# mlee03/FRE-NCtools

Measured on AMD Instinct MI355X. Metric: exchange-cells/s, higher is better.
Workload: dtype f64; 1 GPU; C384 cubed sphere (6 tiles) -> 1440x720 lat-lon, conservative_order2: exchange-grid search + centroid pass + CSR build per step; nxgrid=4160000, parallelism=1 latitude band(s) of the target, one per GPU, world_size=1

## Files before the change

### fre-nctools_amd/_lib.py

```python
import ctypes as C
import os

_HERE = os.path.dirname(os.path.abspath(__file__))
_LIB = None


class FregridHipError(RuntimeError):
    def __init__(self, code, msg):
        super().__init__(f"libfregrid_hip error {code}: {msg}")
        self.code = code


def lib_path():
    return os.environ.get("FREGRID_HIP_LIB") or os.path.join(_HERE, "libfregrid_hip.so")


EXPORTS = [
    "get_maxxgrid", "get_grid_area", "create_xgrid_2dx2d_order1", "create_xgrid_2dx2d_order2", "conserve_interp",
    "clip_2dx2d", "poly_area", "poly_ctrlon", "poly_ctrlat", "fix_lon", "pimod",
    "fg_clip_2dx2d_batch", "fg_poly_op_batch",
    "get_maxxgrid_", "get_grid_area_", "create_xgrid_2dx2d_order1_", "create_xgrid_2dx2d_order2_",
    "fg_last_error", "fg_device_count", "fg_plan_create", "fg_plan_create_dev", "fg_plan_create_empty",
    "fg_plan_destroy", "fg_plan_set_stream", "fg_pool_release", "fg_plan_nxgrid", "fg_plan_ncells_in",
    "fg_plan_cell_sums_dev", "fg_plan_copy_cell_sums", "fg_plan_accumulate_cell_sums", "fg_plan_accumulate_cell_sums_async", "fg_dev_gather_f64", "fg_dev_scatter_f64", "fg_plan_finalize", "fg_plan_get_xgrid", "fg_plan_get_polygons", "fg_plan_create_polylist", "fg_plan_get_cell_struct",
    "fg_plan_get_cell_area", "fg_plan_set_xgrid", "fg_plan_apply", "fg_plan_apply_interleaved", "fg_plan_apply_records", "fg_plan_apply_levels", "fg_plan_apply_records_levels", "fg_plan_levels_capacity", "fg_plan_apply_ex", "fg_plan_mono_begin",
    "fg_plan_mono_minmax_dev", "fg_plan_mono_copy_minmax", "fg_plan_mono_end",
    "fg_plan_create_great_circle", "fg_plan_create_great_circle_dev", "fg_latlon2xyz", "create_xgrid_great_circle",
    "create_xgrid_great_circle_", "get_grid_great_circle_area", "get_grid_great_circle_area_", "clip_2dx2d_great_circle",
    "great_circle_area", "fg_gc_clip_batch", "conserve_interp_great_circle", "fg_sincos_batch",
    "create_xgrid_1dx2d_order1", "create_xgrid_1dx2d_order2", "create_xgrid_2dx1d_order1", "create_xgrid_2dx1d_order2",
    "create_xgrid_1dx2d_order1_", "create_xgrid_1dx2d_order2_", "create_xgrid_2dx1d_order1_", "create_xgrid_2dx1d_order2_",
    "clip", "box_ctrlat", "box_ctrlon", "get_grid_area_no_adjust", "get_grid_area_no_adjust_", "fg_plan_stream", "fg_plan_sync",
    "fg_c2l_create", "fg_c2l_destroy", "fg_c2l_ncells", "fg_c2l_halo_size", "fg_c2l_set_stream", "fg_c2l_sync",
    "fg_c2l_get_centres", "fg_c2l_fill_halo", "fg_c2l_gradient", "fg_c2l_gradient_records", "fg_c2l_records", "fg_c2l_records_levels", "fg_c2l_grid_info", "fg_find_contacts", "fg_halo_map",
    "fg_gnomonic_ed_grid", "fg_tripolar_corners", "fg_remap_write", "fg_remap_write_interp", "fg_remap_read_size", "fg_remap_read", "fg_remap_last_error",
    "fg_plan_trim", "fg_plan_ncells_out", "fg_plan_order", "fg_plan_device", "fg_dev_alloc", "fg_dev_free", "fg_dev_upload", "fg_dev_download",
    "fg_nc_open", "fg_nc_create", "fg_nc_def_dim", "fg_nc_def_var", "fg_nc_put_att_text", "fg_nc_put_att_double", "fg_nc_enddef",
    "fg_nc_inq_ndims", "fg_nc_inq_nvars", "fg_nc_inq_numrecs", "fg_nc_inq_dimid", "fg_nc_inq_dim", "fg_nc_inq_varid", "fg_nc_inq_var",
    "fg_nc_get_att_double", "fg_nc_get_att_text", "fg_nc_get_vara", "fg_nc_get_vara_double", "fg_nc_put_vara", "fg_nc_put_vara_double",
    "fg_nc_close", "fg_nc_last_error", "fg_dev_widen", "fg_dev_narrow", "fg_sweep_create", "fg_sweep_run", "fg_sweep_run_levels", "fg_sweep_destroy", "fg_host_alloc", "fg_host_free",
    "fg_plan_stats", "fg_set_search_mode", "fg_set_search_cull", "fg_set_search_finalize", "fg_set_search_rect", "fg_set_search_frame", "fg_set_apply_xcd", "fg_set_apply_vec", "fg_set_apply_ep", "fg_set_gc_split", "fg_set_profiling", "fg_plan_phase_ms", "fg_gnomonic_ed_corners", "fg_latlon_corners",
    "fg_bilin_create", "fg_bilin_create_from_weights", "fg_bilin_destroy", "fg_bilin_get_index_weight", "fg_bilin_npoints_fine",
    "fg_bilin_nlon_fine", "fg_bilin_nlat_fine", "fg_bilin_nlon", "fg_bilin_nlat", "fg_bilin_ncells", "fg_bilin_set_stream",
    "fg_bilin_sync", "fg_bilin_apply_scalar", "fg_bilin_apply_vector", "fg_bilin_remap_write", "fg_bilin_remap_read",
    "fg_unit_vect_latlon", "fg_bilin_fine_grid", "fg_bilin_ambiguous_ties",
    "fg_extrap_create", "fg_extrap_destroy", "fg_extrap_set_stream", "fg_extrap_stream", "fg_extrap_run_dev", "fg_extrap_run",
    "fg_extrap_last_syncs", "fg_extrap_get_coef", "fg_extrap_coef_host", "fg_set_extrap_batch", "fg_set_extrap_coef",
    "fg_setup_vertical_interp", "fg_dev_vertical_interp",
    "fg_dev_latlon2xyz", "fg_plan_create_great_circle_lonlat", "fg_plan_create_great_circle_lonlat_dev",
    "fg_runoff_create", "fg_runoff_create_from_xgrid", "fg_runoff_destroy", "fg_runoff_nxgrid", "fg_runoff_get_xgrid",
    "fg_runoff_get_maps", "fg_runoff_get_xyz", "fg_runoff_search_stats", "fg_runoff_phase_ms", "fg_runoff_stream", "fg_runoff_apply", "fg_runoff_apply_dev",
    "fg_nearest_unmasked", "fg_set_runoff_prune", "fg_runoff_tile",
    "fg_rland_create", "fg_rland_destroy", "fg_rland_stream", "fg_rland_search", "fg_rland_search_sface", "fg_rland_stats",
    "fg_rland_phase_ms", "fg_set_rland_prune", "fg_rland_tile",
    "fg_river_create", "fg_river_destroy", "fg_river_stream", "fg_river_run", "fg_river_get", "fg_river_get_max_suba",
    "fg_river_stats", "fg_river_phase_ms", "fg_set_river_prune", "fg_river_qsort_index",
    "fg_topog_default_opts", "fg_topog_create", "fg_topog_destroy", "fg_topog_stream", "fg_topog_set_source", "fg_topog_get_source",
    "fg_topog_remap", "fg_topog_filter", "fg_topog_process", "fg_topog_run", "fg_topog_set_depth", "fg_topog_get", "fg_topog_stats",
    "fg_topog_phase_ms", "fg_plan_apply_frac_dev", "fg_set_topog_sweep",
]


class TopogOpts(C.Structure):
    _fields_ = [("scale_factor", C.c_double)] + \
        [(k, C.c_int) for k in ("tripolar_grid", "cyclic_x", "cyclic_y", "fill_first_row", "filter_topog", "num_filter_pass",
                                "smooth_topo_allow_deepening", "round_shallow", "fill_shallow", "deepen_shallow", "full_cell", "flat_bottom",
                                "adjust_topo", "fill_isolated_cells", "dont_change_landmask", "kmt_min")] + \
        [("min_thickness", C.c_double), ("open_very_this_cell", C.c_int), ("fraction_full_cell", C.c_double),
         ("use_great_circle_algorithm", C.c_int), ("on_grid", C.c_int)]


class ApplyOpts(C.Structure):
    _fields_ = [("has_missing", C.c_int), ("missing", C.c_double), ("weight", C.c_void_p),
                ("cell_methods_sum", C.c_int), ("field_area", C.c_void_p), ("area_missing", C.c_double),
                ("cell_area_in", C.c_void_p), ("cell_area_out", C.c_void_p), ("monotonic", C.c_int)]


def lib():
    global _LIB
    if _LIB is not None:
        return _LIB
    path = lib_path()
    if not os.path.exists(path):
        raise ImportError(
            f"{path} not found: build the HIP extension first (make -C fre-nctools_amd/csrc, or "
            "python -c 'import __graft_entry__ as g; g.build()').  There is no CPU fallback.")
    try:
        import torch
    except ImportError:
        pass
    L = C.CDLL(path)
    dp, ip, vp = C.POINTER(C.c_double), C.POINTER(C.c_int), C.c_void_p
    dpp = C.POINTER(dp)
    cip = C.POINTER(C.c_int)

    L.get_maxxgrid.restype = C.c_int
    L.get_grid_area.argtypes = [cip, cip, dp, dp, dp]
    L.get_grid_area.restype = None
    L.create_xgrid_2dx2d_order1.argtypes = [cip] * 4 + [dp] * 5 + [ip] * 4 + [dp]
    L.create_xgrid_2dx2d_order1.restype = C.c_int
    L.create_xgrid_2dx2d_order2.argtypes = [cip] * 4 + [dp] * 5 + [ip] * 4 + [dp] * 3
    L.create_xgrid_2dx2d_order2.restype = C.c_int
    L.conserve_interp.argtypes = [C.c_int] * 4 + [dp] * 7
    L.conserve_interp.restype = None

    L.clip_2dx2d.argtypes = [dp, dp, C.c_int, dp, dp, C.c_int, dp, dp]
    L.clip_2dx2d.restype = C.c_int
    L.poly_area.argtypes = [dp, dp, C.c_int]
    L.poly_area.restype = C.c_double
    L.poly_ctrlon.argtypes = [dp, dp, C.c_int, C.c_double]
    L.poly_ctrlon.restype = C.c_double
    L.poly_ctrlat.argtypes = [dp, dp, C.c_int]
    L.poly_ctrlat.restype = C.c_double
    L.fix_lon.argtypes = [dp, dp, C.c_int, C.c_double]
    L.fix_lon.restype = C.c_int
    L.fg_clip_2dx2d_batch.argtypes = [C.c_int, dp, dp, ip, dp, dp, ip, dp, dp, ip]
    L.fg_clip_2dx2d_batch.restype = C.c_int
    L.fg_poly_op_batch.argtypes = [C.c_int, C.c_int, dp, dp, ip, dp, dp]
    L.fg_poly_op_batch.restype = C.c_int

    L.fg_last_error.restype = C.c_char_p
    L.fg_device_count.restype = C.c_int
    L.fg_plan_create.argtypes = [C.c_int, C.c_int, ip, ip, dpp, dpp, dpp, C.c_int, C.c_int, dp, dp, C.c_int, C.POINTER(vp)]
    L.fg_plan_create.restype = C.c_long
# ... 383 lines not shown
```

### fre-nctools_amd/csrc/plan.hip

```cpp
#include <hip/hip_runtime.h>
#include <math.h>
#include <stdio.h>
#include <stdlib.h>
#include <string.h>
#include <algorithm>
#include <map>
#include <mutex>
#include <string>
#include <type_traits>
#include <vector>
#include "fg_host.h"
#include "xgrid_device.h"

static thread_local std::string g_err;
extern "C" const char *fg_last_error(void) { return g_err.c_str(); }
void fg_set_last_error(const char *msg) { g_err = msg ? msg : ""; }

extern "C" int fg_device_count(void)
{
  int n = 0;
  hipError_t e = hipGetDeviceCount(&n);
  if (e != hipSuccess) { fg_fail(FG_ERR_HIP, "hipGetDeviceCount: %s", hipGetErrorString(e)); return FG_ERR_HIP; }
  return n;
}
// ... 297 lines not shown
    hipEvent_t e = g_handles.get_event(); (void)hipEventRecord(e, st);
    spans.push_back({open_ph, {open_ev, e}}); open_ph = -1;
  }
  void collect(float *ms)
  {
    for (auto &sp : spans) {
      float t = 0; (void)hipEventElapsedTime(&t, sp.second.first, sp.second.second);
      ms[sp.first] += t;
      g_handles.put_event(sp.second.first); g_handles.put_event(sp.second.second);
    }
    spans.clear();
  }
};

struct fg_plan {
  float phase_ms[PH_COUNT] = {0};
  PhaseTimer apply_pt;
  int apply_spans = 0;
  int order = 0, device = 0;
  bool great_circle = false;
  hipStream_t stream = nullptr;
  hipStream_t stream_b = nullptr;
  bool own_stream = true;
  int ntiles = 0;
  std::vector<int> nx_in, ny_in, cell_off;
  std::vector<FgTile> tiles_host;
  int nsrc = 0;
  int nx_out = 0, ny_out = 0, ndst = 0;
  long f_stride = 0;
  bool searched = false, finalized = false, have_geom = false;
  bool fused = false;

  std::vector<void *> owned;
  FgTile *tiles_dev = nullptr;
  double *mask_dev = nullptr;
  FgCells S{}, D{};
  bool rect = false;
  FgRect rect_tab{};
  FgPolyList polys{};
  long nx = 0;
  int *x_src = nullptr, *x_dst = nullptr;
  double *x_area = nullptr, *x_c1 = nullptr, *x_c2 = nullptr;
  int *xoff = nullptr;
  FgRowEnt *perm = nullptr;
  bool rows_built = false;
  bool dist_pending = false;
  double *sums = nullptr;
  FgSrcRec *cen = nullptr;
  FgCsr csr{};
  int *src_idx_f = nullptr;
  double *row_sum = nullptr, *red_partial = nullptr, *red_result = nullptr;
  long row_sum_cap = 0;
  double *il_f = nullptr, *il_out = nullptr, *il_rs = nullptr;
  double *il_m = nullptr;
  unsigned char *lv_bits = nullptr;
  long stats[FG_NSTATS] = {0};
  double *mono_x = nullptr, *mono_b = nullptr;
  int *xerr = nullptr;
  bool mono_open = false;
  unsigned *ll_err = nullptr;

  template <typename T> T *alloc(size_t count)
  {
    void *p = g_pool.get(device, count * sizeof(T));
    if (p) owned.push_back(p);
    return (T *)p;
  }
  void release(void *p)
  {
    if (!p) return;
    for (size_t k = 0; k < owned.size(); k++) if (owned[k] == p) { owned.erase(owned.begin() + k); break; }
    g_pool.put(p);
  }
  void drop_search(size_t keep)
  {
    while (owned.size() > keep) { g_pool.put(owned.back()); owned.pop_back(); }
    tiles_dev = nullptr; mask_dev = nullptr; S = FgCells{}; D = FgCells{};
    x_src = x_dst = nullptr; x_area = x_c1 = x_c2 = nullptr; xoff = nullptr;
    perm = nullptr; csr.row_ptr = nullptr; csr.e1 = nullptr; csr.e2 = nullptr; cen = nullptr; src_idx_f = nullptr; sums = nullptr;
    have_geom = false; rect = false; rect_tab = FgRect{};
  }
};

static bool alloc_cells(fg_plan *pl, FgCells *c, size_t n)
{
  c->lat_min = pl->alloc<double>(n); c->lat_max = pl->alloc<double>(n);
  c->lon_min = pl->alloc<double>(n); c->lon_max = pl->alloc<double>(n);
  c->lon_avg = pl->alloc<double>(n); c->area = pl->alloc<double>(n);
  c->nv = pl->alloc<int>(n);
  c->verts = pl->alloc<double>(n * 16);
  return c->lat_min && c->lat_max && c->lon_min && c->lon_max && c->lon_avg && c->area && c->nv && c->verts;
}

static int plan_base(int order, int ntiles_in, const int *nx_in, const int *ny_in, int nx_out, int ny_out,
                     int device, fg_plan **out)
{
  if (order != FG_CONSERVE_ORDER1 && order != FG_CONSERVE_ORDER2) return fg_fail(FG_ERR_ARG, "order must be 1 or 2");
  if (ntiles_in < 1 || !nx_in || !ny_in || nx_out < 1 || ny_out < 1 || !out) return fg_fail(FG_ERR_ARG, "bad grid sizes");
  if (int rc = fg_use_device("fg_plan", device)) return rc;
  fg_plan *pl = new fg_plan();
  pl->order = order; pl->device = device; pl->ntiles = ntiles_in;
  long off = 0, foff = 0;
  for (int m = 0; m < ntiles_in; m++) {
    if (nx_in[m] < 1 || ny_in[m] < 1) { delete pl; return fg_fail(FG_ERR_ARG, "bad source tile size"); }
    pl->nx_in.push_back(nx_in[m]); pl->ny_in.push_back(ny_in[m]); pl->cell_off.push_back((int)off);
    off += (long)nx_in[m] * ny_in[m];
    foff += (order == 2) ? (long)(nx_in[m] + 2) * (ny_in[m] + 2) : (long)nx_in[m] * ny_in[m];
  }
  if (off > 2000000000L || (long)nx_out * ny_out > 2000000000L) { delete pl; return fg_fail(FG_ERR_ARG, "grid too large for 32-bit cell indices"); }
  pl->nsrc = (int)off; pl->f_stride = foff;
  pl->nx_out = nx_out; pl->ny_out = ny_out; pl->ndst = nx_out * ny_out;
  pl->stream = g_handles.get_stream(device);
  if (!pl->stream) { delete pl; return fg_fail(FG_ERR_HIP, "hipStreamCreate failed"); }
  *out = pl;
  return 0;
}

extern "C" void fg_plan_destroy(fg_plan *pl)
{
  if (!pl) return;
  (void)hipSetDevice(pl->device);
  if (pl->stream || !pl->own_stream) (void)hipStreamSynchronize(pl->stream);
  if (pl->stream && pl->own_stream) g_handles.put_stream(pl->device, pl->stream);
  if (pl->stream_b) { (void)hipStreamSynchronize(pl->stream_b); g_handles.put_stream(pl->device, pl->stream_b); }
  { float junk[PH_COUNT] = {0}; pl->apply_pt.collect(junk); }
  for (void *p : pl->owned) g_pool.put(p);
  delete pl;
}

static void choose_bins(const fg_plan *pl, double mean_dlat, double mean_dlon, FgBins *b)
{
  const double PI = 3.14159265358979323846;
  double h = 1.25 * mean_dlat, w = 1.25 * mean_dlon;
  int nblat = (h > 0) ? (int)ceil(PI / h) : 1;
  int nblon = (w > 0) ? (int)ceil(2.0 * PI / w) : 1;
  if (nblat < 1) nblat = 1; if (nblat > 8192) nblat = 8192;
  if (nblon < 1) nblon = 1; if (nblon > 16384) nblon = 16384;
  (void)pl;
  b->nblat = nblat; b->nblon = nblon;
  b->inv_wlat = nblat / PI;
  b->inv_wlon = nblon / (2.0 * PI);
}

static FgCounters *pinned_counters()
{
  static thread_local FgCounters *h = nullptr;
  if (!h) { if (hipHostMalloc((void **)&h, sizeof(FgCounters), hipHostMallocDefault) != hipSuccess) h = nullptr; }
  return h;
}

struct GcXyz { const double *x, *y, *z; };
struct BoxMode { FgBox box; const double *mask_quad; int no_adjust; };
struct SearchIn {
  const double *const *lon_in = nullptr, *const *lat_in = nullptr, *const *mask_in = nullptr;
  const double *lon_out = nullptr, *lat_out = nullptr;
  const GcXyz *gc_in = nullptr, *gc_out = nullptr;
  const BoxMode *boxm = nullptr;
  double mean_dlat = 0, mean_dlon = 0;
  int rect_hint = 1;
};
struct SearchOpts { bool exact, cull, finalize, rect, dst_frame; int gc_split; bool profile; };
static const char *gc_clip_error(int code)
{
  switch (code) {
    case 3: return "firstIntersect is not in the grid1List";
    case 4: return " not found the next intersection ";
    case 5: return "not return back to the first intersection";
    case 6: return "After clipping, nintersect should be 0";
    case 7: return "inserAfter: point (x,y,z) is not found in the list";
    case 8: return "Error from create_xgrid.c: temp is not in list1";
    default: return "clip_2dx2d_great_circle: more intersections than two convex quadrilaterals can have (list capacity)";
  }
}

// ... 13 lines not shown
  for (int a = 0; a < 3; a++)
    for (int b = 0; b < 3; b++) {
      const long e = (long)js[a] * nxp + is[b];
      if (memcmp(&lon[e], &lon[is[b]], sizeof(double)) || memcmp(&lat[e], &lat[(long)js[a] * nxp], sizeof(double))) return true;
    }
  return false;
}
#define FG_RETRY (-1000L)
struct Carve {
  size_t n = 0;
  size_t operator()(size_t size) { const size_t at = n; n += size; return at; }
};
struct SearchBlocks {
  fg_plan *pl;
  bool ok = true;
  std::vector<void *> scratch;
  template <typename T> T *keep(size_t count) { T *p = pl->alloc<T>(count); ok = ok && p; return p; }
  template <typename T> T *get(size_t count) { T *p = keep<T>(count); if (p) scratch.push_back(p); return p; }
  void release() { for (void *p : scratch) pl->release(p); scratch.clear(); }
};
static long plan_search_core(fg_plan *pl, const SearchIn &in, const SearchOpts &opt, SearchCaps *caps)
{
  const bool gc = in.gc_in != nullptr;
  const BoxMode *const boxm = in.boxm;
  pl->great_circle = gc;
  hipStream_t st = pl->stream;
  const int nsrc = pl->nsrc, ndst = pl->ndst, order = pl->order;
  FgCounters *hc = pinned_counters();
  if (!hc) return fg_fail(FG_ERR_HIP, "hipHostMalloc failed");

  std::vector<FgTile> &th = pl->tiles_host;
  th.resize(pl->ntiles + 1);
  for (int m = 0; m < pl->ntiles; m++) th[m] = FgTile{gc ? nullptr : in.lon_in[m], gc ? nullptr : in.lat_in[m], pl->nx_in[m], pl->ny_in[m], pl->cell_off[m]};
  th[pl->ntiles] = FgTile{in.lon_out, in.lat_out, pl->nx_out, pl->ny_out, 0};
  pl->tiles_dev = pl->alloc<FgTile>(pl->ntiles + 1);
  if (!pl->tiles_dev) return fg_fail(FG_ERR_HIP, "out of device memory");
  FgTileSet ts; ts.n = 0;
  const bool by_value = !gc && pl->ntiles + 1 <= FG_TILESET_MAX;
  if (by_value) { ts.n = pl->ntiles + 1; for (int m = 0; m <= pl->ntiles; m++) ts.t[m] = th[m]; }
  else FGCHK(hipMemcpyAsync(pl->tiles_dev, th.data(), sizeof(FgTile) * th.size(), hipMemcpyHostToDevice, st));
  FgTileXyz *gct_dev = nullptr;
  std::vector<FgTileXyz> gct;
  if (gc) {
    gct.resize(pl->ntiles + 1);
    for (int m = 0; m < pl->ntiles; m++) gct[m] = FgTileXyz{in.gc_in[m].x, in.gc_in[m].y, in.gc_in[m].z, pl->nx_in[m], pl->ny_in[m], pl->cell_off[m]};
    gct[pl->ntiles] = FgTileXyz{in.gc_out->x, in.gc_out->y, in.gc_out->z, pl->nx_out, pl->ny_out, 0};
    gct_dev = pl->alloc<FgTileXyz>(pl->ntiles + 1);
    if (!gct_dev) return fg_fail(FG_ERR_HIP, "out of device memory");
    FGCHK(hipMemcpyAsync(gct_dev, gct.data(), sizeof(FgTileXyz) * gct.size(), hipMemcpyHostToDevice, st));
  }

  bool any_mask = false;
  if (in.mask_in) for (int m = 0; m < pl->ntiles; m++) if (in.mask_in[m]) any_mask = true;
  if (any_mask) {
    pl->mask_dev = pl->alloc<double>(nsrc);
    if (!pl->mask_dev) return fg_fail(FG_ERR_HIP, "out of device memory");
    std::vector<double> ones;
    for (int m = 0; m < pl->ntiles; m++) {
      size_t nc = (size_t)pl->nx_in[m] * pl->ny_in[m];
      if (in.mask_in[m]) FGCHK(hipMemcpyAsync(pl->mask_dev + pl->cell_off[m], in.mask_in[m], nc * sizeof(double), hipMemcpyDeviceToDevice, st));
      else {
        ones.assign(nc, 1.0);
        FGCHK(hipMemcpyAsync(pl->mask_dev + pl->cell_off[m], ones.data(), nc * sizeof(double), hipMemcpyHostToDevice, st));
        FGCHK(hipStreamSynchronize(st));
      }
    }
  }

  const bool rect = caps->rect && !gc && !boxm;
  pl->rect = rect;
  const double dst_tlon = opt.dst_frame ? (double)NAN : 3.14159265358979323846;
  FgBins bins;
  choose_bins(pl, in.mean_dlat, in.mean_dlon, &bins);
  if (rect) { bins.nblat = 0; bins.nblon = 0; }
  const long nbins = (long)bins.nblat * bins.nblon;
  const long nslots = nbins + bins.nblat;
  const unsigned long long nentries = rect ? 0ull : caps->entries;
  const int ecap = (int)std::min<unsigned long long>(nentries, 2147483647ull);
  FgPairSpace ps{};
  ps.nreg = caps->nreg; ps.regcap = caps->regcap;
  const long npairs = fgd_pairs_total(ps);
  const long nx_alloc = npairs;

  if (!alloc_cells(pl, &pl->S, nsrc)) return fg_fail(FG_ERR_HIP, "out of device memory");
  SearchBlocks blk{pl};
  struct { double *hdr, *lat_ax, *lon_ax, *col, *row, *col_min, *col_max, *col_avg; } rt{};
  if (rect) {
    pl->D = FgCells{};
    pl->D.area = blk.keep<double>(ndst);
    Carve at;
    const size_t o_hdr = at(8), o_lat = at((size_t)pl->ny_out + 1), o_lon = at((size_t)pl->nx_out + 1), o_col = at(8 * (size_t)pl->nx_out),
                 o_row = at(4 * ((size_t)pl->ny_out + 1)), o_cmin = at((size_t)pl->nx_out), o_cmax = at((size_t)pl->nx_out), o_cavg = at((size_t)pl->nx_out);
    double *rect_blk = blk.keep<double>(at.n);
    if (!blk.ok) return fg_fail(FG_ERR_HIP, "out of device memory");
    rt = {rect_blk + o_hdr, rect_blk + o_lat, rect_blk + o_lon, rect_blk + o_col, rect_blk + o_row, rect_blk + o_cmin, rect_blk + o_cmax, rect_blk + o_cavg};
  } else if (!alloc_cells(pl, &pl->D, ndst)) return fg_fail(FG_ERR_HIP, "out of device memory");
  const long t_bins = fgd_scan_tiles(nslots), t_rows = fgd_scan_tiles(ndst), t_comp = fgd_scan_tiles(nsrc);
  const size_t zreg = (size_t)FG_NREG * FG_FILL_STRIDE * sizeof(unsigned);
  Carve z;
  const size_t z_dc = z((sizeof(FgCounters) + 127) / 128 * 128), z_fill = z(zreg), z_tick = z(128);
  const size_t z_lb_bins = z(t_bins * sizeof(unsigned long long)), z_lb_rows = z(t_rows * sizeof(unsigned long long)),
               z_lb_comp = z(t_comp * sizeof(unsigned long long));
  const size_t z_bin_cnt = z((size_t)(nslots + 1) * sizeof(int)), z_bin_fill = z((size_t)(nslots + 1) * sizeof(int)),
               z_row_cnt = z((size_t)(ndst + 1) * sizeof(int)), z_nacc = z((size_t)(nsrc + 1) * sizeof(int));
  z((16 - (z.n - z_bin_cnt) % 16) % 16);
  const size_t z_gc_ntask = z(gc ? zreg : 0), z_gc_ocnt = z(gc ? zreg : 0);
  const size_t zbytes = z.n;
  char *zero_blk = blk.get<char>(zbytes);
  int *bin_start = blk.get<int>(nslots + 1);
  int *heavy_list = blk.get<int>(nsrc + 1);
  int *rare_list = blk.get<int>(rect ? nsrc + 1 : 1);
  int *big_list = blk.get<int>(nsrc + 1);
  int *pair_beg = blk.get<int>(nsrc + 1), *pair_cnt = blk.get<int>(nsrc + 1);
  FgBinEntry *bin_entries = blk.get<FgBinEntry>(nentries ? nentries : 1);
  ps.src = blk.get<int>(npairs + 1); ps.dst = blk.get<int>(npairs + 1);
  double *tmp_area = blk.get<double>(npairs + 1);
  double *tmp_clon = (order == 2) ? blk.get<double>(npairs + 1) : nullptr;
  double *tmp_clat = (order == 2) ? blk.get<double>(npairs + 1) : nullptr;
  int *defer_list = blk.get<int>(npairs + 1);
  const bool early_rows = !gc && !boxm;
  int *tmp_rowpos = early_rows ? blk.get<int>(npairs + 1) : nullptr;
  const bool gc_split = gc && opt.gc_split && npairs < (1L << 28);
  const long tcap_want = (opt.gc_split == 2) ? npairs / 64 : 3 * npairs;
  const long tcap_reg = gc_split ? std::min<long>((tcap_want / FG_NREG + 255) / 256 * 256, 0x7ffffff0L / FG_NREG) : 0;
  const long tcap_all = tcap_reg * FG_NREG;
  unsigned *gc_meta = gc_split ? blk.get<unsigned>(npairs + 1) : nullptr;
  int *gc_tbase = gc_split ? blk.get<int>(npairs + 1) : nullptr;
  int *gc_order = gc_split ? blk.get<int>(npairs + 1) : nullptr;
  unsigned *gc_task = gc_split ? blk.get<unsigned>(tcap_all + 1) : nullptr;
  double *gc_res = gc_split ? blk.get<double>(2 * (size_t)tcap_all + 2) : nullptr;
  pl->xoff = blk.keep<int>(nsrc + 1);
  pl->x_src = blk.keep<int>(nx_alloc + 1); pl->x_dst = blk.keep<int>(nx_alloc + 1);
  pl->x_area = blk.keep<double>(nx_alloc + 1);
  if (order == 2) { pl->x_c1 = blk.keep<double>(nx_alloc + 1); pl->x_c2 = blk.keep<double>(nx_alloc + 1); pl->sums = blk.keep<double>(3 * (size_t)nsrc); }
  int *x_rowpos = blk.get<int>(nx_alloc + 1);
  pl->perm = blk.keep<FgRowEnt>(nx_alloc + 1);
  pl->csr.row_ptr = blk.keep<int>(ndst + 1);
  if (!pl->src_idx_f) pl->src_idx_f = blk.keep<int>(nsrc + 1);
  if (!blk.ok) return fg_fail(FG_ERR_HIP, "out of device memory");
  FgCounters *dc = (FgCounters *)(zero_blk + z_dc);
  ps.fill = (unsigned *)(zero_blk + z_fill);
  unsigned *tickets = (unsigned *)(zero_blk + z_tick);
  unsigned long long *lb_bins = (unsigned long long *)(zero_blk + z_lb_bins), *lb_rows = (unsigned long long *)(zero_blk + z_lb_rows),
                     *lb_comp = (unsigned long long *)(zero_blk + z_lb_comp);
  int *bin_cnt = (int *)(zero_blk + z_bin_cnt), *bin_fill = (int *)(zero_blk + z_bin_fill), *row_cnt = (int *)(zero_blk + z_row_cnt);
  int *nacc = (int *)(zero_blk + z_nacc);
  FGCHK(hipMemsetAsync(zero_blk, 0, zbytes, st));
  if (pl->ll_err) FGCHK(hipMemcpyAsync(&dc->err[2], pl->ll_err, sizeof(unsigned), hipMemcpyDeviceToDevice, st));

  PhaseTimer pt, ptot;
  pt.start(opt.profile, st); ptot.start(opt.profile, st);
  for (int k = 0; k < PH_COUNT; k++) pl->phase_ms[k] = 0;
  ptot.begin(PH_SEARCH_TOTAL);
  pt.begin(PH_CELL_STRUCT);
  if (gc) {
    fgd_gc_cell_struct(gct_dev + pl->ntiles, 1, ndst, pl->D, st, opt.cull ? dc->band_keys : nullptr, 1);
    fgd_gc_cell_struct(gct_dev, pl->ntiles, nsrc, pl->S, st, opt.cull ? dc->band_keys : nullptr, 2);
    fgd_src_field_index(order, pl->tiles_dev, pl->ntiles, nsrc, pl->src_idx_f, st);
  } else if (rect) {
    FgRect &R = pl->rect_tab;
    R.hdr = rt.hdr; R.lat_ax = rt.lat_ax; R.lon_ax = rt.lon_ax; R.col = rt.col; R.row = rt.row;
    R.col_min = rt.col_min; R.col_max = rt.col_max; R.col_avg = rt.col_avg;
    R.bad = &dc->rect_bad; R.nx = pl->nx_out; R.ny = pl->ny_out;
    fgd_rect_tables(in.lon_out, in.lat_out, pl->nx_out, pl->ny_out, rt.hdr, rt.lat_ax, rt.lon_ax, rt.col, rt.col_min, rt.col_max, rt.col_avg, rt.row,
                    &dc->rect_bad, dc->err, st, dst_tlon);
    if (pl->polys.npoly) fgd_polylist_records(pl->polys, pl->S, pl->src_idx_f, pl->sums, &R, heavy_list, &dc->heavy_cnt, dc->err, st);
    fgd_cell_struct2r(ts, pl->tiles_dev, pl->tiles_dev, pl->ntiles, pl->polys.npoly ? 0 : nsrc, ndst, pl->S, pl->D.area, R, pl->mask_dev, order,
                      pl->src_idx_f, pl->sums, dc->err, st, dc->band_keys, (opt.cull && !pl->polys.npoly) ? 2 : 0, heavy_list, &dc->heavy_cnt,
                      rare_list, &dc->rare_cnt, ps, pair_beg, pair_cnt, big_list, &dc->big_cnt);
  } else if (opt.cull && !boxm && !pl->polys.npoly) {
    fgd_band_keys(in.lat_out, (long)(pl->nx_out + 1) * (pl->ny_out + 1), dc->band_keys, st);
    fgd_cell_struct2(ts, pl->tiles_dev, pl->tiles_dev, pl->ntiles, nsrc, ndst, pl->S, pl->D, bins, bin_cnt, order, pl->src_idx_f, pl->sums, dc->err, st, dc->band_keys, 2, dst_tlon);
  } else if (pl->polys.npoly) {
    fgd_polylist_records(pl->polys, pl->S, pl->src_idx_f, pl->sums, nullptr, nullptr, nullptr, dc->err, st);
    fgd_cell_struct2(ts, pl->tiles_dev, pl->tiles_dev, pl->ntiles, 0, ndst, pl->S, pl->D, bins, bin_cnt, order, pl->src_idx_f, pl->sums, dc->err, st, nullptr, 0, dst_tlon);
  } else
    fgd_cell_struct2(ts, pl->tiles_dev, pl->tiles_dev, pl->ntiles, nsrc, ndst, pl->S, pl->D, bins, bin_cnt, order, pl->src_idx_f, pl->sums, dc->err, st, nullptr, 0, dst_tlon);
  if (boxm) fgd_box_cell_boxes(boxm->box, pl->S, st);
  if (boxm && boxm->no_adjust) fgd_box_area_no_adjust(boxm->box, pl->S.area, st);
  pt.end();
  pl->have_geom = true;

  if (!rect) {
    pt.begin(PH_BINS);
    if (gc) fgd_bin_count(ndst, pl->D, bins, bin_cnt, st);
    fgd_exclusive_scan1(bin_cnt, nslots, bin_start, lb_bins, &tickets[0], &dc->total[0], dc->err, st);
    fgd_bin_fill(ndst, pl->D, bins, bin_fill, bin_start, bin_entries, ecap, nsrc, pl->S, pl->mask_dev, heavy_list, &dc->heavy_cnt, st);
    pt.end();
  }

  pt.begin(PH_CANDIDATES);
  if (rect)
    fgd_candidates_rect(nsrc, pl->S, pl->mask_dev, pl->rect_tab, ps, pair_beg, pair_cnt, heavy_list, &dc->heavy_cnt, big_list, &dc->big_cnt, st,
                        pl->polys.npoly ? 0 : 1,
                        rare_list, &dc->rare_cnt, dc->err);
  else
    fgd_candidates1(nsrc, pl->S, pl->mask_dev, bins, bin_start, bin_entries, ecap, ps, pair_beg, pair_cnt, heavy_list, &dc->heavy_cnt, big_list,
                    &dc->big_cnt, st);
  pt.end();
  hipEvent_t gc_e1 = nullptr, gc_e2 = nullptr;
  struct EvReturn {
    hipEvent_t &a, &b;
    ~EvReturn() { g_handles.put_sync_event(a); g_handles.put_sync_event(b); a = b = nullptr; }
  } ev_return{gc_e1, gc_e2};
  if (boxm) {
    pt.begin(PH_CLIP_GENERAL);
    fgd_clip_box(order, ps, boxm->box, th[pl->ntiles], pl->S, pl->D, pl->mask_dev, boxm->mask_quad, tmp_area, tmp_clon, tmp_clat, nacc, dc->stats, dc->err, st);
    pt.end();
  } else if (gc) {
    pt.begin(PH_CLIP_GENERAL);
    if (gc_split) {
      if (!pl->stream_b) pl->stream_b = g_handles.get_stream(pl->device);
      gc_e1 = g_handles.get_sync_event(); gc_e2 = g_handles.get_sync_event();
      GcSplit g{gc_meta, gc_tbase, gc_task, gc_res, (unsigned)tcap_reg, (unsigned *)(zero_blk + z_gc_ntask), defer_list, &dc->defer_cnt,
                &dc->gc_list2_cnt, npairs, gc_order, (unsigned *)(zero_blk + z_gc_ocnt)};
      fgd_gc_clip_split(ps, pl->S, pl->mask_dev, pl->D, tmp_area, nacc, g, dc->stats, dc->err, st, pl->stream_b, gc_e1, gc_e2);
    } else
      fgd_gc_clip(ps, pl->S, pl->mask_dev, pl->D, tmp_area, nacc, defer_list, &dc->defer_cnt, dc->stats, dc->err, st);
    pt.end();
  } else {
    pt.begin(PH_CLIP_QUAD);
    fgd_clip_quad(order, ps, pl->S, pl->mask_dev, pl->D, tmp_area, tmp_clon, tmp_clat, nacc, defer_list, &dc->defer_cnt, dc->stats, dc->err, st,
                  rect ? &pl->rect_tab : nullptr, row_cnt, tmp_rowpos);
    pt.end();
    pt.begin(PH_CLIP_GENERAL);
    fgd_clip_general(order, ps, pl->S, pl->mask_dev, pl->D, tmp_area, tmp_clon, tmp_clat, nacc, defer_list, &dc->defer_cnt, dc->stats, dc->err, st,
                     rect ? &pl->rect_tab : nullptr, row_cnt, tmp_rowpos);
    pt.end();
  }
  pt.begin(PH_COMPACT);
  FgCompactIo io{};
  io.pair_beg = pair_beg; io.pair_cnt = pair_cnt;
  io.tmp_area = tmp_area; io.tmp_clon = tmp_clon; io.tmp_clat = tmp_clat;
  io.xoff = pl->xoff; io.x_src = pl->x_src; io.x_dst = pl->x_dst; io.x_area = pl->x_area; io.x_c1 = pl->x_c1; io.x_c2 = pl->x_c2;
  io.row_cnt = row_cnt; io.x_rowpos = x_rowpos; io.sums = pl->sums; io.big_list = big_list; io.big_cnt = &dc->big_cnt;
  io.tmp_rowpos = tmp_rowpos; io.row_ptr = pl->csr.row_ptr; io.perm = pl->perm;
  io.dc = dc; io.xcap = nx_alloc;
  if (early_rows)
    fgd_exclusive_scan2(nacc, nsrc, pl->xoff, lb_comp, &tickets[2], &dc->xtot, row_cnt, ndst, pl->csr.row_ptr, lb_rows, &tickets[1], &dc->rows_total, dc->err, st);
  else
    fgd_exclusive_scan1(nacc, nsrc, pl->xoff, lb_comp, &tickets[2], &dc->xtot, dc->err, st);
  fgd_compact(order, nsrc, ps, io, st);
  pt.end();
  if (!early_rows) {
    pt.begin(PH_ROWS);
    fgd_exclusive_scan1(row_cnt, ndst, pl->csr.row_ptr, lb_rows, &tickets[1], &dc->rows_total, dc->err, st);
    fgd_csr_fill_pos(nx_alloc, &dc->xtot, pl->x_src, pl->x_dst, pl->csr.row_ptr, x_rowpos, pl->perm, st);
    pt.end();
  }
  ptot.end();
  const bool fuse = opt.finalize && early_rows && !pl->polys.npoly;
  int *fused_tmp = nullptr;
  if (fuse) {
    pt.begin(PH_FINALIZE);
    if (order == 2) {
      pl->cen = pl->alloc<FgSrcRec>((size_t)nsrc + 1);
      if (!pl->cen) return fg_fail(FG_ERR_HIP, "out of device memory");
      fgd_centroids(nsrc, pl->S, pl->sums, pl->cen, st);
      pl->csr.e2 = pl->alloc<FgCsrEntry2>(nx_alloc + 1);
    } else pl->csr.e1 = pl->alloc<FgCsrEntry1>(nx_alloc + 1);
    if (!pl->csr.e1 && !pl->csr.e2) return fg_fail(FG_ERR_HIP, "out of device memory");
    int *sg_tmp = pl->alloc<int>(3 * (size_t)(nx_alloc + 1));
    fgd_csr_sortgather(order, ndst, (long)nsrc + ndst, pl->perm, pl->x_area, pl->x_c1, pl->x_c2, pl->src_idx_f,
                       order == 2 ? pl->cen : nullptr, pl->csr, st, sg_tmp, nx_alloc + 1);
    fused_tmp = sg_tmp;
    pt.end();
  }
  FGCHK(hipMemcpyAsync(hc, dc, sizeof(FgCounters), hipMemcpyDeviceToHost, st));
  FGCHK(hipStreamSynchronize(st));
  pt.collect(pl->phase_ms); ptot.collect(pl->phase_ms);
  FGCHK(hipGetLastError());
  if (rect && hc->rect_bad) { caps->rect = false; return FG_RETRY; }
  if (hc->total[0] > nentries) { caps->entries = hc->total[0]; return FG_RETRY; }
  if (hc->total[0] > 2000000000ull) return fg_fail(FG_ERR_ARG, "bin table too large");
  if (hc->total[3] > (unsigned long long)ps.regcap) {
    if (hc->total[3] > 2000000000ull / (unsigned long long)ps.nreg) return fg_fail(FG_ERR_CAPACITY, "candidate pair list exceeds 2^31 entries");
    caps->regcap = (int)((hc->total[3] + FG_REG_ALIGN - 1) / FG_REG_ALIGN * FG_REG_ALIGN);
    return FG_RETRY;
  }
  if (hc->err[2] & G_ERRBIT_LL2X) return fg_fail(FG_ERR_ARG, "latlon2xyz: a grid corner is not finite, or its latitude (|lat| >= 2.4262) or longitude "
                                                          "(|lon| > 1024) lies outside the range of the device trig (radians expected)");
  if (hc->err[0] & 8u) return fg_fail(FG_ERR_ARG, "a grid corner latitude lies outside [-pi/2, pi/2] (radians expected)");
  if (hc->err[0] & 1u) return fg_fail(FG_ERR_MAXV, "create_xgrid.c: n2_in is greater than MAX_V");
  if (hc->err[0] & 2u) return fg_fail(FG_ERR_PARALLEL, "the line between <x1_0,y1_0> and  <x1_1,y1_1> should not parallel to "
                                                    "the line between <x2_0,y2_0> and  <x2_1,y2_1>");
  if (hc->err[0] & 4u) return fg_fail(FG_ERR_MAXV, "clipped polygon exceeds 16 vertices");
  if (hc->err[0] & G_ERRBIT_GC_CONVEX1) return fg_fail(FG_ERR_GEOM, "create_xgrid.c(clip_2dx2d_great_circle): grid box 1 is not convex");
  if (hc->err[0] & G_ERRBIT_GC_CONVEX2) return fg_fail(FG_ERR_GEOM, "create_xgrid.c(clip_2dx2d_great_circle): grid box 2 is not convex");
  if (hc->err[0] & G_ERRBIT_GC_CLIP) return fg_fail(FG_ERR_GEOM, "%s", gc_clip_error((int)hc->err[1]));
  if (hc->err[0] & G_ERRBIT_LOOKBACK) return fg_fail(FG_ERR_HIP, "single-pass scan: a tile waited too long for its predecessor");
  pl->nx = (long)hc->xtot;
  pl->stats[FG_STAT_PAIRS] = (long)hc->total[1];
  pl->stats[FG_STAT_NONEMPTY] = (long)(hc->xtot + hc->stats[FG_STAT_BELOW]);
  pl->stats[FG_STAT_NXGRID] = pl->nx;
  pl->stats[FG_STAT_BORDERLINE] = (long)hc->stats[FG_STAT_BORDERLINE];
  pl->stats[FG_STAT_BINS] = nbins;
  pl->stats[FG_STAT_BIN_ENTRIES] = (long)hc->total[0];
  pl->stats[FG_STAT_DEFERRED] = hc->defer_cnt + hc->gc_list2_cnt;
  pl->stats[FG_STAT_HEAVY] = hc->heavy_cnt;
  pl->stats[FG_STAT_RARE] = hc->rare_cnt;
  pl->stats[FG_STAT_BELOW] = (long)hc->stats[FG_STAT_BELOW];

  pl->rect_tab.bad = nullptr;
  blk.release();
  pl->rows_built = true;
  pl->searched = true;
  if (fuse) {
    pl->release(pl->perm); pl->perm = nullptr; pl->release(fused_tmp);
    if (!pl->red_partial) { pl->red_partial = pl->alloc<double>(1024); pl->red_result = pl->alloc<double>(260); }
    if (!pl->red_partial || !pl->red_result) return fg_fail(FG_ERR_HIP, "out of device memory");
    pl->dist_pending = (order == 2);
    pl->finalized = true; pl->fused = true;
  }
  return pl->nx;
}

static int g_search_exact = 0;
extern "C" void fg_set_search_mode(int exact) { g_search_exact = exact; }
extern "C" void fg_set_search_cull(int on) { g_search_cull = on ? 1 : 0; }
extern "C" void fg_set_search_finalize(int on) { g_search_finalize = on ? 1 : 0; }
static long plan_search(fg_plan *pl, const SearchIn &in)
{
  static const bool env_exact = getenv("FREGRID_HIP_EXACT_SEARCH") && atoi(getenv("FREGRID_HIP_EXACT_SEARCH")) != 0;
  const SearchOpts opt{.exact = g_search_exact || env_exact, .cull = g_search_cull != 0, .finalize = g_search_finalize != 0,
                       .rect = g_search_rect != 0, .dst_frame = g_dst_frame != 0, .gc_split = g_gc_split, .profile = g_profiling != 0};
  const long big = std::max((long)pl->nsrc, (long)pl->ndst);
  if (big > (1L << 28)) return fg_fail(FG_ERR_CAPACITY, "grid of %ld cells: more than 2^28 cells per search are not supported", big);
  SearchCaps caps;
  caps.entries = opt.exact ? 0ull : 3ull * (unsigned long long)pl->ndst + 4096ull;
  const unsigned long long cap_pairs = std::min<unsigned long long>(8ull * (unsigned long long)big + 65536ull, 2000000000ull);
  caps.nreg = (int)std::max(1L, std::min((long)FG_NREG, ((long)pl->nsrc + 1023) / 1024));
  caps.regcap = opt.exact ? 0 : (int)((cap_pairs / caps.nreg + FG_REG_ALIGN - 1) / FG_REG_ALIGN * FG_REG_ALIGN);
  caps.rect = opt.rect && in.rect_hint && !in.gc_in && !in.boxm && pl->nx_out <= 8192 && pl->nx_out >= 2;
  const size_t keep = pl->owned.size();
  long rc = FG_RETRY;
  int attempts = 0;
  for (; attempts < 4 && rc == FG_RETRY; attempts++) {
    if (attempts) {
      (void)hipStreamSynchronize(pl->stream);
      pl->drop_search(keep);
    }
    rc = plan_search_core(pl, in, opt, &caps);
  }
  if (rc == FG_RETRY) return fg_fail(FG_ERR_CAPACITY, "exchange-grid search: capacities did not settle");
  if (rc >= 0) pl->stats[FG_STAT_EXACT] = (attempts > 1) ? 1 : 0;
  return rc;
}

struct CornerSample {
  int nsamp = 0;
  std::vector<double> q;
  const double *corners(int a, int k) const { return &q[((size_t)a * nsamp + k) * 4]; }
};
static long sample_step(int nx, int ny, int *nsamp)
{
// ... 584 lines not shown
  }
  if (area) jobs.push_back(XferJob{area, pl->x_area, (size_t)nx * sizeof(double), true});
  if (pl->order == 2) {
    if (c1) jobs.push_back(XferJob{c1, pl->x_c1, (size_t)nx * sizeof(double), true});
    if (c2) jobs.push_back(XferJob{c2, pl->x_c2, (size_t)nx * sizeof(double), true});
  }
  if (!xfer_pool().run(pl->device, jobs)) return fg_fail(FG_ERR_HIP, "fg_plan_get_xgrid: device -> host copy failed");
  return 0;
}

extern "C" int fg_plan_get_polygons(const fg_plan *pl, int maxv, int *n_out, double *v0, double *v1, double *v2)
{
  if (!pl || !n_out || !v0 || !v1) return fg_fail(FG_ERR_ARG, "null argument");
  if (!pl->searched || !pl->have_geom || !pl->x_src) return fg_fail(FG_ERR_STATE, "fg_plan_get_polygons: needs a plan from a search (cell records)");
  if (pl->great_circle && !v2) return fg_fail(FG_ERR_ARG, "fg_plan_get_polygons: a great-circle plan returns x, y, z");
  if (maxv < 3 || maxv > 64) return fg_fail(FG_ERR_ARG, "fg_plan_get_polygons: maxv must be 3..64");
  FGCHK(hipSetDevice(pl->device));
  FGCHK(hipStreamSynchronize(pl->stream));
  const long nx = pl->nx, CH = 1L << 20;
  const int dev = pl->device;
  for (long k0 = 0; k0 < nx; k0 += CH) {
    const long n = std::min(CH, nx - k0);
    const size_t nv = (size_t)n * maxv;
    int *d_n = (int *)g_pool.get(dev, n * sizeof(int));
    double *d_v = (double *)g_pool.get(dev, 3 * nv * sizeof(double));
    struct Put { void *a, *b; ~Put() { g_pool.put(a); g_pool.put(b); } } put{d_n, d_v};
    if (!d_n || !d_v) return fg_fail(FG_ERR_HIP, "out of device memory");
    std::vector<XferJob> jobs;
    if (pl->great_circle) {
      double *a = (double *)g_pool.get(dev, (size_t)n * 12 * 8), *b = (double *)g_pool.get(dev, (size_t)n * 12 * 8);
      double *o = (double *)g_pool.get(dev, (size_t)n * FG_GC_POLY_CAP * 3 * 8), *ar = (double *)g_pool.get(dev, (size_t)n * 8);
      struct Put4 { void *p[4]; ~Put4() { for (void *q : p) g_pool.put(q); } } put4{{a, b, o, ar}};
      if (!a || !b || !o || !ar) return fg_fail(FG_ERR_HIP, "out of device memory");
      fgd_xgrid_gather_gc(n, pl->x_src + k0, pl->x_dst + k0, pl->S, pl->D, a, b, pl->stream);
      fgd_gc_clip_batch((int)n, a, b, o, d_n, ar, pl->stream);
      fgd_split_xyz(n, maxv, o, d_v, d_v + nv, d_v + 2 * nv, pl->stream);
      FGCHK(hipStreamSynchronize(pl->stream));
      jobs.push_back(XferJob{v2 + (size_t)k0 * maxv, d_v + 2 * nv, nv * sizeof(double), true});
    } else {
      fgd_xgrid_polygons(n, pl->x_src + k0, pl->x_dst + k0, pl->S, pl->D, pl->rect ? &pl->rect_tab : nullptr, maxv, d_n, d_v, d_v + nv, pl->stream);
      FGCHK(hipStreamSynchronize(pl->stream));
    }
    FGCHK(hipGetLastError());
    jobs.push_back(XferJob{n_out + k0, d_n, (size_t)n * sizeof(int), true});
    jobs.push_back(XferJob{v0 + (size_t)k0 * maxv, d_v, nv * sizeof(double), true});
    jobs.push_back(XferJob{v1 + (size_t)k0 * maxv, d_v + nv, nv * sizeof(double), true});
    if (!xfer_pool().run(dev, jobs)) return fg_fail(FG_ERR_HIP, "fg_plan_get_polygons: device -> host copy failed");
  }
  return 0;
}

extern "C" int fg_plan_get_cell_area(const fg_plan *pl, double *area_in, double *area_out)
{
  if (!pl) return fg_fail(FG_ERR_ARG, "null plan");
  if (!pl->have_geom) return fg_fail(FG_ERR_STATE, "plan holds no cell records");
  FGCHK(hipSetDevice(pl->device));
  FGCHK(hipStreamSynchronize(pl->stream));
  if (area_in) FGCHK(hipMemcpy(area_in, pl->S.area, (size_t)pl->nsrc * sizeof(double), hipMemcpyDeviceToHost));
  if (area_out) FGCHK(hipMemcpy(area_out, pl->D.area, (size_t)pl->ndst * sizeof(double), hipMemcpyDeviceToHost));
  return 0;
}

extern "C" int fg_plan_get_cell_struct(const fg_plan *pl, int which, double *lat_min, double *lat_max, double *lon_min,
                                       double *lon_max, double *lon_avg, int *nvert, double *vlon, double *vlat)
{
  if (!pl) return fg_fail(FG_ERR_ARG, "null plan");
  if (!pl->have_geom) return fg_fail(FG_ERR_STATE, "plan holds no cell records");
  FGCHK(hipSetDevice(pl->device));
  FGCHK(hipStreamSynchronize(pl->stream));
  FgCells tmp{};
  std::vector<void *> tmp_blocks;
  struct Free { std::vector<void *> &v; ~Free() { for (void *p : v) g_pool.put(p); } } free_tmp{tmp_blocks};
  if (which && pl->rect) {
    const size_t nd = (size_t)pl->ndst;
    auto get = [&](size_t bytes) { void *p = g_pool.get(pl->device, bytes); if (p) tmp_blocks.push_back(p); return p; };
    tmp.lat_min = (double *)get(nd * 8); tmp.lat_max = (double *)get(nd * 8); tmp.lon_min = (double *)get(nd * 8);
    tmp.lon_max = (double *)get(nd * 8); tmp.lon_avg = (double *)get(nd * 8); tmp.nv = (int *)get(nd * 4); tmp.verts = (double *)get(nd * 128);
    tmp.area = pl->D.area;
    if (tmp_blocks.size() != 7) return fg_fail(FG_ERR_HIP, "out of device memory");
    FgRect R = pl->rect_tab;
    fgd_rect_materialize(pl->ndst, R, tmp, pl->stream);
    FGCHK(hipStreamSynchronize(pl->stream));
  }
  const FgCells &c = which ? (pl->rect ? tmp : pl->D) : pl->S;
  size_t n = which ? pl->ndst : pl->nsrc;
  if (lat_min) FGCHK(hipMemcpy(lat_min, c.lat_min, n * sizeof(double), hipMemcpyDeviceToHost));
  if (lat_max) FGCHK(hipMemcpy(lat_max, c.lat_max, n * sizeof(double), hipMemcpyDeviceToHost));
  if (lon_min) FGCHK(hipMemcpy(lon_min, c.lon_min, n * sizeof(double), hipMemcpyDeviceToHost));
  if (lon_max) FGCHK(hipMemcpy(lon_max, c.lon_max, n * sizeof(double), hipMemcpyDeviceToHost));
  if (lon_avg) FGCHK(hipMemcpy(lon_avg, c.lon_avg, n * sizeof(double), hipMemcpyDeviceToHost));
  if (nvert) FGCHK(hipMemcpy(nvert, c.nv, n * sizeof(int), hipMemcpyDeviceToHost));
  if (vlon || vlat) {
    std::vector<double> v(n * 16);
    FGCHK(hipMemcpy(v.data(), c.verts, n * 16 * sizeof(double), hipMemcpyDeviceToHost));
    for (size_t k = 0; k < n; k++)
      for (int l = 0; l < 8; l++) {
        if (vlon) vlon[k * 8 + l] = v[k * 16 + l];
        if (vlat) vlat[k * 8 + l] = v[k * 16 + 8 + l];
      }
  }
  return 0;
}

extern "C" int fg_plan_set_xgrid(fg_plan *pl, long nxgrid, const int *t_in, const int *i_in, const int *j_in,
                                 const int *i_out, const int *j_out, const double *area,
                                 const double *di_in, const double *dj_in)
{
  if (!pl) return fg_fail(FG_ERR_ARG, "null plan");
  if (nxgrid < 0 || (nxgrid > 0 && (!t_in || !i_in || !j_in || !i_out || !j_out || !area))) return fg_fail(FG_ERR_ARG, "null exchange-cell array");
  if (pl->order == 2 && nxgrid > 0 && (!di_in || !dj_in)) return fg_fail(FG_ERR_ARG, "order 2 needs di_in/dj_in");
  if (pl->finalized || pl->searched) return fg_fail(FG_ERR_STATE, "fg_plan_set_xgrid needs a plan from fg_plan_create_empty");
  FGCHK(hipSetDevice(pl->device));
  std::vector<int> s(nxgrid), d(nxgrid);
  for (long k = 0; k < nxgrid; k++) {
    int m = t_in[k];
    if (m < 0 || m >= pl->ntiles || i_in[k] < 0 || i_in[k] >= pl->nx_in[m] || j_in[k] < 0 || j_in[k] >= pl->ny_in[m] ||
        i_out[k] < 0 || i_out[k] >= pl->nx_out || j_out[k] < 0 || j_out[k] >= pl->ny_out)
      return fg_fail(FG_ERR_ARG, "exchange cell %ld has an index outside its grid", k);
    s[k] = pl->cell_off[m] + j_in[k] * pl->nx_in[m] + i_in[k];
    d[k] = j_out[k] * pl->nx_out + i_out[k];
  }
  pl->nx = nxgrid;
  pl->x_src = pl->alloc<int>(nxgrid + 1); pl->x_dst = pl->alloc<int>(nxgrid + 1);
  pl->x_area = pl->alloc<double>(nxgrid + 1);
  if (pl->order == 2) { pl->x_c1 = pl->alloc<double>(nxgrid + 1); pl->x_c2 = pl->alloc<double>(nxgrid + 1); }
  if (!pl->x_src || !pl->x_dst || !pl->x_area || (pl->order == 2 && (!pl->x_c1 || !pl->x_c2))) return fg_fail(FG_ERR_HIP, "out of device memory");
  if (nxgrid > 0) {
    FGCHK(hipMemcpy(pl->x_src, s.data(), nxgrid * sizeof(int), hipMemcpyHostToDevice));
    FGCHK(hipMemcpy(pl->x_dst, d.data(), nxgrid * sizeof(int), hipMemcpyHostToDevice));
    FGCHK(hipMemcpy(pl->x_area, area, nxgrid * sizeof(double), hipMemcpyHostToDevice));
    if (pl->order == 2) {
      FGCHK(hipMemcpy(pl->x_c1, di_in, nxgrid * sizeof(double), hipMemcpyHostToDevice));
      FGCHK(hipMemcpy(pl->x_c2, dj_in, nxgrid * sizeof(double), hipMemcpyHostToDevice));
    }
  }
  pl->searched = true;
  int rc = build_csr(pl, nullptr);
  if (rc) return rc;
  pl->finalized = true;
  return 0;
}

extern int g_apply_vec, g_apply_ep;
extern "C" void fg_set_apply_ep(int on) { g_apply_ep = on ? 1 : 0; }

extern int g_apply_xcd;
extern "C" void fg_set_apply_xcd(int on) { g_apply_xcd = on < 0 ? 0 : on; }
extern "C" void fg_set_apply_vec(int v) { g_apply_vec = (v >= 4) ? 4 : (v >= 2 ? 2 : (v == 1 ? 1 : 0)); }

static void apply_span_begin(fg_plan *pl, hipStream_t st)
{
  pl->apply_pt.start(g_profiling != 0 && pl->apply_spans < 256, st);
  pl->apply_pt.begin(PH_APPLY);
}
static void apply_span_end(fg_plan *pl)
{
  pl->apply_pt.end();
  if (pl->apply_pt.on) pl->apply_spans++;
}

static int levels_pad(int nz) { return nz > 4 ? 8 : (nz > 2 ? 4 : 2); }

static int ensure_il_rs(fg_plan *pl)
{
  if (!pl->il_rs) {
    pl->il_rs = pl->alloc<double>((size_t)pl->ndst * 16);
    if (!pl->il_rs) return fg_fail(FG_ERR_HIP, "out of device memory");
// ... 1042 lines not shown
```

### fre-nctools_amd/csrc/poly_kernels.hip

```cpp
#include "xgrid_device.h"
#include "geom.hip.h"

#define PB_IN   12
#define PB_CAP  24

__device__ inline int d_clip_private(const double *lon1, const double *lat1, int n1,
                                     const double *lon2, const double *lat2, int n2,
                                     double *lon_out, double *lat_out)
{
  double cx[PB_CAP], cy[PB_CAP], ex[PB_IN], ey[PB_IN];
  bool wrap = false;
  for (int k = 0; k < n1; k++) { cx[k] = lon1[k]; cy[k] = lat1[k]; if (cx[k] > G_TPI || cx[k] < 0.0) wrap = true; }
  for (int k = 0; k < n2; k++) { ex[k] = lon2[k]; ey[k] = lat2[k]; }
  if (wrap) {
    for (int k = 0; k < n1; k++) cx[k] = d_pimod1(cx[k]);
    for (int k = 0; k < n2; k++) ex[k] = d_pimod1(ex[k]);
  }
  int n_cur = n1;
  double x2_0 = ex[n2 - 1], y2_0 = ey[n2 - 1];
  for (int e = 0; e < n2; e++) {
    double x2_1 = ex[e], y2_1 = ey[e];
    double x1_0 = cx[n_cur - 1], y1_0 = cy[n_cur - 1];
    int inside_last = d_inside_edge(x2_0, y2_0, x2_1, y2_1, x1_0, y1_0);
    int n_new = 0;
// ... 22 lines not shown
    n_cur = n_new;
    if (!n_cur) return 0;
    for (int k = 0; k < n_cur; k++) { cx[k] = lon_out[k]; cy[k] = lat_out[k]; }
    x2_0 = x2_1; y2_0 = y2_1;
  }
  return n_cur;
}

__global__ __launch_bounds__(64) void k_poly_clip(int npoly, const double *lon1, const double *lat1, const int *n1,
                                                   const double *lon2, const double *lat2, const int *n2,
                                                   double *lon_out, double *lat_out, int *n_out)
{
  int p = blockIdx.x * blockDim.x + threadIdx.x;
  if (p >= npoly) return;
  double a[PB_IN], b[PB_IN], c[PB_IN], d[PB_IN], xo[PB_CAP], yo[PB_CAP];
  int m1 = n1[p], m2 = n2[p];
  if (m1 < 1 || m1 > PB_IN || m2 < 1 || m2 > PB_IN) { n_out[p] = -2; return; }
  for (int k = 0; k < m1; k++) { a[k] = lon1[(size_t)p * PB_CAP + k]; b[k] = lat1[(size_t)p * PB_CAP + k]; }
  for (int k = 0; k < m2; k++) { c[k] = lon2[(size_t)p * PB_CAP + k]; d[k] = lat2[(size_t)p * PB_CAP + k]; }
  int n = d_clip_private(a, b, m1, c, d, m2, xo, yo);
  n_out[p] = n;
  for (int k = 0; k < PB_CAP; k++) {
    lon_out[(size_t)p * PB_CAP + k] = (k < n) ? xo[k] : 0.0;
    lat_out[(size_t)p * PB_CAP + k] = (k < n) ? yo[k] : 0.0;
  }
}

__global__ __launch_bounds__(64) void k_poly_op(int op, int npoly, double *lon, double *lat, int *n, const double *clon,
                                                 double *result)
{
  int p = blockIdx.x * blockDim.x + threadIdx.x;
  if (p >= npoly) return;
  double x[PB_CAP], y[PB_CAP];
  int m = n[p];
  if (m < 1 || m > PB_CAP || (op == 3 && m > G_FIXCAP - 4)) { if (result) result[p] = 0; if (op == 3) n[p] = -2; return; }
  for (int k = 0; k < m; k++) { x[k] = lon[(size_t)p * PB_CAP + k]; y[k] = lat[(size_t)p * PB_CAP + k]; }
  if (op == 0) result[p] = d_poly_area<1>(x, y, m);
  else if (op == 1) result[p] = d_poly_ctrlon<1>(x, y, m, clon[p]);
  else if (op == 2) result[p] = d_poly_ctrlat<1>(x, y, m);
  else if (op >= 4) {
    double pa, pclon, pclat;
    d_poly_area_ctr<1>(x, y, m, op == 5 ? clon[p] : 0.0, &pa, &pclon, &pclat);
    result[p] = (op == 4) ? pa : (op == 5) ? pclon : pclat;
  } else {
    int mm = d_fix_lon(x, y, m, clon[p]);
    n[p] = mm;
    for (int k = 0; k < PB_CAP; k++) {
      lon[(size_t)p * PB_CAP + k] = (k < mm) ? x[k] : 0.0;
      lat[(size_t)p * PB_CAP + k] = (k < mm) ? y[k] : 0.0;
    }
  }
}

void fgd_poly_clip(int npoly, const double *lon1, const double *lat1, const int *n1, const double *lon2, const double *lat2,
                   const int *n2, double *lon_out, double *lat_out, int *n_out, hipStream_t st)
{
  if (npoly > 0) k_poly_clip<<<(npoly + 63) / 64, 64, 0, st>>>(npoly, lon1, lat1, n1, lon2, lat2, n2, lon_out, lat_out, n_out);
}
void fgd_poly_op(int op, int npoly, double *lon, double *lat, int *n, const double *clon, double *result, hipStream_t st)
{
  if (npoly > 0) k_poly_op<<<(npoly + 63) / 64, 64, 0, st>>>(op, npoly, lon, lat, n, clon, result);
}

__global__ __launch_bounds__(256) void k_sincos_probe(long n, const double *x, double *s, double *c)
{
  long i = (long)blockIdx.x * blockDim.x + threadIdx.x;
  if (i >= n) return;
  s[i] = d_sin_lat(x[i]); c[i] = d_cos_lat(x[i]);
}
void fgd_sincos_probe(long n, const double *x, double *s, double *c, hipStream_t st)
{
  if (n > 0) k_sincos_probe<<<(int)((n + 255) / 256), 256, 0, st>>>(n, x, s, c);
}

__global__ __launch_bounds__(64) void k_xgrid_polygons(long n, const int *x_src, const int *x_dst, FgCells S, FgCells D, FgRect R, int rect,
                                                        int maxv, int *n_out, double *lon_out, double *lat_out)
{
  const long k = (long)blockIdx.x * blockDim.x + threadIdx.x;
  if (k >= n) return;
  const int s = x_src[k], d = x_dst[k];
  double a[PB_IN], b[PB_IN], c[PB_IN], e[PB_IN], xo[PB_CAP], yo[PB_CAP];
  const int n1 = S.nv[s];
  int n2;
  const double *sv = S.verts + (size_t)s * 16;
  for (int q = 0; q < 8; q++) { a[q] = sv[q]; b[q] = sv[8 + q]; }
  double lon_out_avg;
  if (rect) {
    const int j = d / R.nx, i = d - j * R.nx;
    const double *cr = R.col + (size_t)i * RECT_COLW;
    const double ya = R.lat_ax[j], yb = R.lat_ax[j + 1];
    c[0] = cr[0]; c[1] = cr[1]; c[2] = cr[2]; c[3] = cr[3]; lon_out_avg = cr[6];
    e[0] = ya; e[1] = ya; e[2] = yb; e[3] = yb;
    n2 = 4;
  } else {
    const double *dv = D.verts + (size_t)d * 16;
    for (int q = 0; q < 8; q++) { c[q] = dv[q]; e[q] = dv[8 + q]; }
    lon_out_avg = D.lon_avg[d];
    n2 = D.nv[d];
  }
  const double dx = lon_out_avg - S.lon_avg[s];
  const double shift = (dx < -G_PI) ? G_TPI : ((dx > G_PI) ? -G_TPI : 0.0);
  if (shift != 0.0) for (int q = 0; q < n2; q++) c[q] += shift;
  int m = (n1 < 1 || n2 < 1) ? 0 : d_clip_private(a, b, n1, c, e, n2, xo, yo);
  n_out[k] = m;
  for (int q = 0; q < maxv; q++) {
    lon_out[(size_t)k * maxv + q] = (q < m && q < PB_CAP) ? xo[q] : 0.0;
    lat_out[(size_t)k * maxv + q] = (q < m && q < PB_CAP) ? yo[q] : 0.0;
  }
}
void fgd_xgrid_polygons(long n, const int *x_src, const int *x_dst, FgCells S, FgCells D, const FgRect *rect, int maxv,
                        int *n_out, double *lon_out, double *lat_out, hipStream_t st)
{
  if (n > 0) k_xgrid_polygons<<<(unsigned)((n + 63) / 64), 64, 0, st>>>(n, x_src, x_dst, S, D, rect ? *rect : FgRect{}, rect ? 1 : 0, maxv,
                                                                      n_out, lon_out, lat_out);
}
__global__ __launch_bounds__(256) void k_xgrid_gather_gc(long n, const int *x_src, const int *x_dst, FgCells S, FgCells D, double *a, double *b)
{
  const long t = (long)blockIdx.x * blockDim.x + threadIdx.x;
  if (t >= n * 12) return;
  const long k = t / 12; const int q = (int)(t - k * 12);
  a[t] = S.verts[(size_t)x_src[k] * 16 + q];
  b[t] = D.verts[(size_t)x_dst[k] * 16 + q];
}
void fgd_xgrid_gather_gc(long n, const int *x_src, const int *x_dst, FgCells S, FgCells D, double *a, double *b, hipStream_t st)
{
  if (n > 0) k_xgrid_gather_gc<<<(unsigned)((n * 12 + 255) / 256), 256, 0, st>>>(n, x_src, x_dst, S, D, a, b);
}
__global__ __launch_bounds__(256) void k_split_xyz(long n, int maxv, const double *xyz, double *x, double *y, double *z)
{
  const long t = (long)blockIdx.x * blockDim.x + threadIdx.x;
  if (t >= n * maxv) return;
  const long k = t / maxv; const int q = (int)(t - k * maxv);
  const bool in = q < FG_GC_POLY_CAP;
  x[t] = in ? xyz[((size_t)k * FG_GC_POLY_CAP + q) * 3] : 0.0;
  y[t] = in ? xyz[((size_t)k * FG_GC_POLY_CAP + q) * 3 + 1] : 0.0;
  z[t] = in ? xyz[((size_t)k * FG_GC_POLY_CAP + q) * 3 + 2] : 0.0;
}
void fgd_split_xyz(long n, int maxv, const double *xyz, double *x, double *y, double *z, hipStream_t st)
{
  if (n > 0) k_split_xyz<<<(unsigned)((n * maxv + 255) / 256), 256, 0, st>>>(n, maxv, xyz, x, y, z);
}
```

### fre-nctools_amd/csrc/xgrid_device.h

```cpp
#pragma once
#include <hip/hip_runtime.h>

struct FgTile {
  const double *lon;
  const double *lat;
  int nx, ny;
  int cell_off;
};

struct FgTileXyz {
  const double *x, *y, *z;
  int nx, ny;
  int cell_off;
};
#define G_ERRBIT_GC_CONVEX1 16u
#define G_ERRBIT_GC_CONVEX2 32u
#define G_ERRBIT_GC_CLIP    64u

struct FgCells {
  double *lat_min, *lat_max, *lon_min, *lon_max, *lon_avg, *area;
  int *nv;
  double *verts;
};

struct FgBins {
  int nblat, nblon;
  double inv_wlat, inv_wlon;
};

struct FgBinEntry {
  double lat_min, lat_max, lon_min, lon_max, lon_avg;
  int d;
  int row0;
};

enum {
  FG_STAT_PAIRS = 0,
  FG_STAT_NONEMPTY = 1,
  FG_STAT_NXGRID = 2,
  FG_STAT_BORDERLINE = 3,
  FG_STAT_BINS = 4,
  FG_STAT_BIN_ENTRIES = 5,
  FG_STAT_DEFERRED = 6,
  FG_STAT_HEAVY = 7,
  FG_STAT_BELOW = 8,
  FG_STAT_EXACT = 9,
  FG_STAT_RARE = 10,
  FG_NSTATS = 11
};

#define FG_REG_ALIGN 512
#define FG_NREG 64
#define FG_FILL_STRIDE 32
struct FgPairSpace {
  int *src, *dst;
  unsigned *fill;
  int regcap, nreg;
};
#ifdef __HIPCC__
__device__ __forceinline__ bool d_pair_live(const FgPairSpace &ps, int p)
{
  const unsigned first = blockIdx.x * blockDim.x;
  const unsigned r = first / (unsigned)ps.regcap;
  const unsigned f = ps.fill[r * FG_FILL_STRIDE];
  return (unsigned)p - r * (unsigned)ps.regcap < (f < (unsigned)ps.regcap ? f : (unsigned)ps.regcap);
}
#endif
static inline long fgd_pairs_total(const FgPairSpace &ps) { return (long)ps.regcap * ps.nreg; }
#ifdef __HIPCC__
__device__ __forceinline__ unsigned long long d_ord_key(double v)
{
  const unsigned long long b = (unsigned long long)__double_as_longlong(v);
  return (b >> 63) ? ~b : (b | 0x8000000000000000ull);
}
__device__ __forceinline__ double d_ord_val(unsigned long long k)
{
  const unsigned long long b = (k >> 63) ? (k & 0x7fffffffffffffffull) : ~k;
  return __longlong_as_double((long long)b);
}
#endif

#define FG_TILESET_MAX 8
struct FgTileSet { FgTile t[FG_TILESET_MAX]; int n; };

struct FgLl2xGrid { const double *lon, *lat; double *x, *y, *z; long n; };
struct FgLl2xSet { FgLl2xGrid g[FG_TILESET_MAX]; int n; };
#define G_ERRBIT_LL2X 256u
void fgd_latlon2xyz(const FgLl2xGrid *grids, int ngrids, unsigned *err, hipStream_t st);

struct FgCounters {
  unsigned long long total[4];
  unsigned long long rows_total;
  unsigned long long band_keys[2];
  unsigned long long xtot;
  unsigned err[4];
  int heavy_cnt;
  unsigned rect_bad;
  int defer_cnt, big_cnt;
  int gc_list2_cnt;
  int rare_cnt;
  unsigned long long stats[FG_NSTATS];
};
#define G_ERRBIT_LOOKBACK 128u

long fgd_scan_tiles(long n);
void fgd_exclusive_scan1(const int *in, long n, int *out, unsigned long long *status, unsigned *ticket,
                         unsigned long long *total_dev, unsigned *err, hipStream_t st);

void fgd_exclusive_scan2(const int *in_a, long n_a, int *out_a, unsigned long long *status_a, unsigned *ticket_a, unsigned long long *total_a,
                         const int *in_b, long n_b, int *out_b, unsigned long long *status_b, unsigned *ticket_b, unsigned long long *total_b,
                         unsigned *err, hipStream_t st);

void fgd_cell_struct2(const FgTileSet &ts, const FgTile *tiles_in, FgTile *tiles_out, int ntiles, int nsrc, int ndst, FgCells S, FgCells D,
                      FgBins b, int *slot_cnt, int order, int *src_idx_f, double *sums, unsigned *err, hipStream_t st,
                      unsigned long long *band_keys = nullptr, int cull = 0, double dst_tlon = 3.14159265358979323846);
void fgd_cell_struct(const FgTile *tiles_dev, int ntiles, int ncells, FgCells c, unsigned *err, hipStream_t st);
void fgd_band_keys(const double *lat, long n, unsigned long long *band_keys, hipStream_t st);
void fgd_bin_count(int ncells, FgCells c, FgBins b, int *slot_cnt, hipStream_t st);
void fgd_bin_fill(int ndst, FgCells D, FgBins b, int *slot_fill, const int *slot_start, FgBinEntry *entries, int cap,
                  int nsrc, FgCells S, const double *mask, int *heavy_list, int *heavy_cnt, hipStream_t st);
void fgd_candidates1(int nsrc, FgCells S, const double *mask, FgBins b, const int *slot_start, const FgBinEntry *entries, int ecap,
                     FgPairSpace ps, int *pair_beg, int *pair_cnt, const int *heavy_list, const int *heavy_cnt, int *big_list, int *big_cnt,
                     hipStream_t st);
#define RECT_COLW 8
struct FgRect {
  const double *lon_ax;
  const double *lat_ax;
  const double *col;
  const double *col_min, *col_max, *col_avg;
  const double *hdr;
  const double *row;
  const unsigned *bad;
  int nx, ny;
};
void fgd_rect_tables(const double *lon, const double *lat, int nx, int ny, double *hdr, double *lat_ax, double *lon_ax, double *col,
                     double *col_min, double *col_max, double *col_avg, double *row, unsigned *bad, unsigned *err, hipStream_t st,
                     double dst_tlon = 3.14159265358979323846);
void fgd_cell_struct2r(const FgTileSet &ts, const FgTile *tiles_in, FgTile *tiles_out, int ntiles, int nsrc, int ndst, FgCells S, double *area_out,
                       FgRect R, const double *mask, int order, int *src_idx_f, double *sums, unsigned *err, hipStream_t st,
                       unsigned long long *band_keys, int cull, int *heavy_list, int *heavy_cnt, int *rare_list, int *rare_cnt, FgPairSpace ps,
                       int *pair_beg, int *pair_cnt, int *big_list, int *big_cnt);
void fgd_rect_materialize(int ndst, FgRect R, FgCells D, hipStream_t st);
struct FgPolyList { const int *n; const double *lon, *lat; const double *lon_avg, *area; int npoly; };
void fgd_polylist_records(FgPolyList P, FgCells S, int *src_idx_f, double *sums, const FgRect *rect, int *heavy_list, int *heavy_cnt,
                          unsigned *err, hipStream_t st);
void fgd_candidates_rect(int nsrc, FgCells S, const double *mask, FgRect R, FgPairSpace ps, int *pair_beg, int *pair_cnt,
                         const int *heavy_list, const int *heavy_cnt, int *big_list, int *big_cnt, hipStream_t st, int listed_only,
                         const int *rare_list = nullptr, const int *rare_cnt = nullptr, unsigned *err = nullptr);
void fgd_clip_general(int order, FgPairSpace ps, FgCells S, const double *mask, FgCells D,
              double *tmp_area, double *tmp_clon, double *tmp_clat, int *nacc, int *defer_list, int *defer_cnt,
              unsigned long long *stats, unsigned *err, hipStream_t st, const FgRect *rect = nullptr, int *row_cnt = nullptr,
              int *tmp_rowpos = nullptr);
void fgd_clip_quad(int order, FgPairSpace ps, FgCells S, const double *mask, FgCells D,
              double *tmp_area, double *tmp_clon, double *tmp_clat, int *nacc, int *defer_list, int *defer_cnt,
              unsigned long long *stats, unsigned *err, hipStream_t st, const FgRect *rect = nullptr, int *row_cnt = nullptr,
              int *tmp_rowpos = nullptr);
struct alignas(8) FgRowEnt { int n, s; };
struct alignas(16) FgSrcRec { double cen_lon, cen_lat; };
struct FgCompactIo {
  const int *pair_beg, *pair_cnt;
  const double *tmp_area, *tmp_clon, *tmp_clat;
  const int *xoff;
  int *x_src, *x_dst;
  double *x_area, *x_c1, *x_c2;
  int *row_cnt, *x_rowpos;
  const int *tmp_rowpos;
  const int *row_ptr; FgRowEnt *perm;
  double *sums;
  const int *big_list;
  const int *big_cnt;
  FgCounters *dc;
  long xcap;
};
void fgd_compact(int order, int nsrc, FgPairSpace ps, const FgCompactIo &io, hipStream_t st);
void fgd_centroids(int nsrc, FgCells S, const double *sums, FgSrcRec *cen, hipStream_t st);
void fgd_distances(long nx, const int *x_src, const double *x_area, const FgSrcRec *cen, double *x_c1, double *x_c2, hipStream_t st);

struct FgCsrEntry1 { int idx_f; int pad; double area; };
struct FgCsrEntry2 { int idx_f; int idx_g; double area, di, dj; };
struct FgCsr {
  int *row_ptr;
  FgCsrEntry1 *e1;
  FgCsrEntry2 *e2;
};
void fgd_csr_count(long nx, const int *x_dst, int *row_cnt, hipStream_t st);
void fgd_csr_fill(long nx, const int *x_src, const int *x_dst, const int *row_ptr, int *row_fill, FgRowEnt *perm, hipStream_t st);
void fgd_csr_fill_pos(long nx_cap, const unsigned long long *nx_dev, const int *x_src, const int *x_dst, const int *row_ptr, const int *x_rowpos,
                      FgRowEnt *perm, hipStream_t st);
void fgd_csr_sortgather(int order, int ndst, long nx, const FgRowEnt *perm, const double *x_area, const double *x_c1, const double *x_c2,
                        const int *src_idx_f, const FgSrcRec *cen, FgCsr csr, hipStream_t st, int *tmp = nullptr, long ntmp = 0,
                        int long_rows = 0);
void fgd_src_field_index(int order, const FgTile *tiles_dev, int ntiles, int nsrc, int *src_idx_f, hipStream_t st);
void fgd_apply1(int order, int ndst, FgCsr csr, const double *f, const double *gx, const double *gy, const int *gmask,
                int has_missing, double missing, double *out, double *row_sum, hipStream_t st, long nx = -1);
void fgd_apply_il(int order, int nb, int ndst, FgCsr csr, const double *f, const double *gx, const double *gy, double missing,
                  double *out, double *row_sum, long out_ld, int nb_valid, hipStream_t st, long nx = -1);
void fgd_interleave(int nb_pad, long n, const double *in, long ld, int nb_valid, double *out, hipStream_t st);
void fgd_apply_il_merged(int nb, int ndst, long nx, FgCsr csr, const double *rec, double missing, double *out, double *row_sum, long out_ld,
                         int nb_valid, hipStream_t st);
void fgd_merge3(int nb_pad, long n, const int *src_idx_f, const double *f, long ld_f, const double *gx, const double *gy, long ld_g,
                int nb_valid, double *out, hipStream_t st);
void fgd_interleave3(int nb_pad, int narr, const double *const *in, const long *ld, const long *n, double *const *out, int nb_valid,
                     hipStream_t st);
void fgd_deinterleave(int nb_pad, long n, const double *in, long ld, int nb_valid, double *out, hipStream_t st);
#define FG_LEVELS_CAP 256
void fgd_apply_levels8(int order, int ndst, long nx, FgCsr csr, const double *rec, const unsigned char *gbits, double missing, double *out,
                       double *row_sum, long ld, int nb_valid, hipStream_t st);
void fgd_gmask_bits(long n, const int *gmask, long ld, int nb, unsigned char *bits, hipStream_t st);
void fgd_apply_frac(int ndst, FgCsr csr, const double *data, double *out, hipStream_t st);
void fgd_reduce_sum(const double *v, long n, double *partial, double *result, hipStream_t st);
void fgd_xgrid_indices(long nx, const int *x_src, const int *x_dst, const FgTile *tiles_dev, int ntiles, int nx_out,
                       int *t_in, int *i_in, int *j_in, int *i_out, int *j_out, hipStream_t st);

struct FgApplyEx {
  const double *weight;
  const double *cell_area;
  const double *field_area;
  const double *cell_area_out;
  const int *gmask;
  const double *xdata;
  double area_missing, missing;
  int has_missing, sum;
};
#define FG_XERR_AREA_MISSING 1
#define FG_XERR_ABOVE 2
#define FG_XERR_BELOW 4
void fgd_apply_ex(int order, int ndst, FgCsr csr, const double *f, const double *gx, const double *gy, FgApplyEx o,
                  double *out, double *row_sum, int *err, hipStream_t st, long nx = -1);
void fgd_mono_bounds(const FgTile *tiles_dev, int ntiles, int nsrc, const int *src_idx_f, const double *f, double missing,
                     double *fbmax, double *fbmin, double *fmax, double *fmin, hipStream_t st);
void fgd_mono_xdata(long nx, FgCsr csr, const double *f, const double *gx, const double *gy, const int *gmask, double missing,
// ... 65 lines not shown
```

### fre-nctools_amd/csrc/xgrid_kernels.hip

```cpp
#include <algorithm>
#include "xgrid_device.h"
#ifndef FG_EXP
#define FG_EXP 0
#endif
static __shared__ double fgs_lds_tab[112 * 4];
#define FGS_TAB(k, j) fgs_lds_tab[(k) * 4 + (j)]
#include "geom.hip.h"
__device__ __forceinline__ void d_load_trig_table()
{
  for (int i = threadIdx.x; i < 112 * 4; i += blockDim.x) fgs_lds_tab[i] = FG_SINCOS_TAB[i >> 2][i & 3];
  __syncthreads();
}

#define SCAN_THREADS 256
#define SCAN_ITEMS   8
#define SCAN_CHUNK   (SCAN_THREADS * SCAN_ITEMS)
#define LB_AGG   (1ull << 62)
#define LB_INC   (2ull << 62)
#define LB_MASK  ((1ull << 62) - 1ull)
#define LB_SPIN_LIMIT (1u << 22)

__device__ __forceinline__ unsigned wave_incl_scan(unsigned v, int lane)
{
#pragma unroll
// ... 134 lines not shown
  unsigned run = (unsigned)excl + inc - s;
#pragma unroll
  for (int k = 0; k < SCAN_ITEMS; k++) { tile[threadIdx.x * SCAN_ITEMS + k] = run; run += loc[k]; }
  __syncthreads();
#pragma unroll
  for (int k = 0; k < SCAN_ITEMS; k++) {
    const int li = k * SCAN_THREADS + threadIdx.x;
    const long idx = base + li;
    if (idx <= j.n) j.out[idx] = (int)tile[li];
  }
  if (threadIdx.x == 0 && j.n >= base && j.n < base + SCAN_CHUNK) *j.total = excl + tot;
}

long fgd_scan_tiles(long n) { if (n < 0) n = 0; return (n + 1 + SCAN_CHUNK - 1) / SCAN_CHUNK; }
void fgd_exclusive_scan2(const int *in_a, long n_a, int *out_a, unsigned long long *status_a, unsigned *ticket_a, unsigned long long *total_a,
                         const int *in_b, long n_b, int *out_b, unsigned long long *status_b, unsigned *ticket_b, unsigned long long *total_b,
                         unsigned *err, hipStream_t st)
{
  if (n_a < 0) n_a = 0;
  if (n_b < 0) n_b = 0;
  const long nt = std::max(fgd_scan_tiles(n_a), fgd_scan_tiles(n_b));
  k_scan2<<<dim3((unsigned)nt, 2), SCAN_THREADS, 0, st>>>(FgScanJob{in_a, n_a, out_a, status_a, ticket_a, total_a},
                                                         FgScanJob{in_b, n_b, out_b, status_b, ticket_b, total_b}, err, 2 * nt > 1024 ? 1 : 0);
}

void fgd_exclusive_scan1(const int *in, long n, int *out, unsigned long long *status, unsigned *ticket,
                         unsigned long long *total_dev, unsigned *err, hipStream_t st)
{
  if (n < 0) n = 0;
  const int nt = (int)fgd_scan_tiles(n);
  k_scan1<<<nt, SCAN_THREADS, 0, st>>>(in, n, out, status, nt <= 1024 ? nullptr : ticket, total_dev, err);
}


template <bool QUADS_ONLY = false>
__device__ __forceinline__ int d_cell_record(const FgTile *tiles, int ntiles, int ncells, const FgCells &c, unsigned *err, int s0,
                                             double *vtile, double *box , int *tile_of,
                                             const unsigned long long *cull = nullptr, double tlon = G_PI, bool *rare = nullptr)
{
  constexpr int VS = QUADS_ONLY ? 9 : 17, NLIVE = QUADS_ONLY ? 8 : 16, CAP = QUADS_ONLY ? 4 : G_FIXCAP;
  const int s = s0 + threadIdx.x;
  double *row = vtile + threadIdx.x * VS;
#pragma unroll
  for (int k = 0; k < NLIVE; k++) row[k] = 0.0;
  int nvert = 0;
  bool listed = false;
  if (s < ncells) {
    int t = 0;
    while (t + 1 < ntiles && s >= tiles[t + 1].cell_off) t++;
    *tile_of = t;
    const FgTile T = tiles[t];
    int loc = s - T.cell_off;
    int i = loc % T.nx, j = loc / T.nx;
    int nxp = T.nx + 1;
    int n0 = j * nxp + i, n1 = n0 + 1, n3 = n0 + nxp, n2 = n3 + 1;
    double x[CAP], y[CAP];
    x[0] = T.lon[n0]; y[0] = T.lat[n0];
    x[1] = T.lon[n1]; y[1] = T.lat[n1];
    x[2] = T.lon[n2]; y[2] = T.lat[n2];
    x[3] = T.lon[n3]; y[3] = T.lat[n3];
    double lmin = y[0], lmax = y[0];
#pragma unroll
    for (int k = 1; k < 4; k++) { if (y[k] < lmin) lmin = y[k]; if (y[k] > lmax) lmax = y[k]; }
    c.lat_min[s] = lmin; c.lat_max[s] = lmax;
    box[0] = lmin; box[1] = lmax;
    if (!(lmin >= -G_HPI - 1.e-6) || !(lmax <= G_HPI + 1.e-6)) atomicOr(err, G_ERRBIT_BADLAT);
    bool out_of_band = false;
    if (cull && cull[0]) {
      const double bmax = d_ord_val(cull[0]), bmin = d_ord_val(~cull[1]);
      out_of_band = (lmax <= bmin) || (lmin >= bmax);
    }
    int n = out_of_band ? 0 : d_fix_lon_quad_fast(x, y, tlon);
    if constexpr (!QUADS_ONLY) {
      if (n < 0) n = d_fix_lon(x, y, 4, tlon);
    }
    if (out_of_band) { c.nv[s] = 0; c.area[s] = 0; }
    else if (QUADS_ONLY && n < 0) {
      listed = true;
#pragma unroll
      for (int k = 0; k < 4; k++) { row[k] = x[k]; row[4 + k] = y[k]; }
    }
    else if (n < 0 || n > G_MAXV) {
      atomicOr(err, G_ERRBIT_MAXV);
      c.nv[s] = 0; c.lon_min[s] = 0; c.lon_max[s] = 0; c.lon_avg[s] = 0; c.area[s] = 0;
    } else if constexpr (QUADS_ONLY) {
      double xmin = x[0], xmax = x[0], xs = 0;
#pragma unroll
      for (int k = 1; k < 4; k++) { if (x[k] < xmin) xmin = x[k]; if (x[k] > xmax) xmax = x[k]; }
#pragma unroll
      for (int k = 0; k < 4; k++) xs += x[k];
      xs /= 4;
      c.lon_min[s] = xmin; c.lon_max[s] = xmax; c.lon_avg[s] = xs;
      box[2] = xmin; box[3] = xmax; box[4] = xs;
      c.nv[s] = 4;
      nvert = 4;
#pragma unroll
      for (int k = 0; k < 4; k++) { row[k] = x[k]; row[4 + k] = y[k]; }
      c.area[s] = d_poly_area<1>(x, y, 4);
    } else {
      double xmin = x[0], xmax = x[0], xs = 0;
      for (int k = 1; k < n; k++) { if (x[k] < xmin) xmin = x[k]; if (x[k] > xmax) xmax = x[k]; }
      for (int k = 0; k < n; k++) xs += x[k];
      xs /= n;
      c.lon_min[s] = xmin; c.lon_max[s] = xmax; c.lon_avg[s] = xs;
      box[2] = xmin; box[3] = xmax; box[4] = xs;
      c.nv[s] = n;
      nvert = n;
      for (int k = 0; k < G_MAXV; k++) {
        row[k] = (k < n) ? x[k] : 0.0;
        row[8 + k] = (k < n) ? y[k] : 0.0;
      }
      c.area[s] = d_poly_area<1>(x, y, n);
    }
  }
  if (QUADS_ONLY) *rare = listed;
  if (!__syncthreads_or(nvert != 0 || listed) && cull) return 0;
  const long cnt = (long)min(256, ncells - s0) * 16;
  double *out = c.verts + (size_t)s0 * 16;
#pragma unroll
  for (int q = 0; q < 16; q++) {
    const long e = (long)q * 256 + threadIdx.x;
    if constexpr (QUADS_ONLY) {
      const int k = (int)e & 15;
      if (e < cnt) out[e] = (k & 4) ? 0.0 : vtile[(e >> 4) * VS + ((k >> 3) << 2) + (k & 3)];
    } else if (e < cnt) out[e] = vtile[(e >> 4) * VS + (e & 15)];
  }
  return nvert;
}

__device__ __forceinline__ int d_finish_rare_cell(const FgCells &c, unsigned *err, int s, int lane, double *box)
{
  double *v = c.verts + (size_t)s * 16;
  double x[G_FIXCAP], y[G_FIXCAP];
#pragma unroll
  for (int k = 0; k < 4; k++) { x[k] = v[k]; y[k] = v[8 + k]; }
  double lmin = y[0], lmax = y[0];
#pragma unroll
  for (int k = 1; k < 4; k++) { if (y[k] < lmin) lmin = y[k]; if (y[k] > lmax) lmax = y[k]; }
  box[0] = lmin; box[1] = lmax;
  const int n = d_fix_lon(x, y, 4, G_PI);
  if (n < 0 || n > G_MAXV) {
    if (lane == 0) {
      atomicOr(err, G_ERRBIT_MAXV);
      c.nv[s] = 0; c.lon_min[s] = 0; c.lon_max[s] = 0; c.lon_avg[s] = 0; c.area[s] = 0;
      for (int k = 0; k < 16; k++) v[k] = 0.0;
    }
    return 0;
  }
  double xmin = x[0], xmax = x[0], xs = 0;
  for (int k = 1; k < n; k++) { if (x[k] < xmin) xmin = x[k]; if (x[k] > xmax) xmax = x[k]; }
  for (int k = 0; k < n; k++) xs += x[k];
  xs /= n;
  box[2] = xmin; box[3] = xmax; box[4] = xs;
  const double area = d_poly_area<1>(x, y, n);
  if (lane == 0) {
    c.lon_min[s] = xmin; c.lon_max[s] = xmax; c.lon_avg[s] = xs;
    c.nv[s] = n;
    for (int k = 0; k < G_MAXV; k++) {
      v[k] = (k < n) ? x[k] : 0.0;
      v[8 + k] = (k < n) ? y[k] : 0.0;
    }
    c.area[s] = area;
  }
  return n;
}

__global__ __launch_bounds__(256) void k_cell_struct(const FgTile *tiles, int ntiles, int ncells, FgCells c, unsigned *err)
{
  __shared__ double vtile[256 * 17];
  d_load_trig_table();
  double box[5]; int tl = 0;
  (void)d_cell_record(tiles, ntiles, ncells, c, err, blockIdx.x * 256, vtile, box, &tl);
}

__device__ __forceinline__ void d_cell_box(double lat_min, double lat_max, double lon_min, double lon_max, FgBins b,
                                           int *r0, int *r1, long long *l0, long long *l1)
{
  const double eps = 1.e-9;
  int a0 = (int)floor((lat_min - eps + G_HPI) * b.inv_wlat);
  int a1 = (int)floor((lat_max + eps + G_HPI) * b.inv_wlat);
  *r0 = max(0, min(b.nblat - 1, a0));
  *r1 = max(0, min(b.nblat - 1, a1));
  *l0 = (long long)floor((lon_min - eps) * b.inv_wlon);
  *l1 = (long long)floor((lon_max + eps) * b.inv_wlon);
}
__device__ __forceinline__ int d_colmod(long long l, int nb) { return (int)(((l % nb) + nb) % nb); }

__device__ __forceinline__ int d_slot_position(int *slot_cnt, int key)
{
  const int lane = threadIdx.x & 63;
  const int prev = __shfl_up(key, 1);
  const bool head = (lane == 0) || (key != prev);
  const unsigned long long heads = __ballot(head);
  const int start = 63 - __clzll((long long)(heads & ((2ull << lane) - 1ull)));
  const unsigned long long above = (start == 63) ? 0ull : (heads & ~((2ull << start) - 1ull));
  const int end = above ? (__ffsll((long long)above) - 1) : 64;
  int base = 0;
  if (lane == start && key >= 0) base = atomicAdd(&slot_cnt[key], end - start);
  base = __shfl(base, start);
  return base + (lane - start);
}

#define BIN_COPIES 16
#define BIN_ROW_COPIES 4
static_assert(BIN_COPIES >= 1 && BIN_COPIES <= 16, "a bin record keeps the copy number and copies - 1 in four bits each");

__device__ __forceinline__ bool d_copy_first(int word, int c_start, int nblon, bool first_row)
{
  const int col = word & 0xffff, o = (word >> 16) & 15, flen = ((word >> 20) & 15) + 1;
  if (((word >> 24) & 1) && !first_row) return false;
  int p = col - c_start;
  if (p < 0) p += nblon;
  return p == 0 || (o == 0 && p + flen <= nblon);
}

template <bool FILL>
__device__ __forceinline__ void d_bin_insert(bool live, int d, double lat_min, double lat_max, double lon_min, double lon_max, double lon_avg,
                                             FgBins b, int *slot_cnt, const int *slot_start, FgBinEntry *entries, int cap)
{
  FgBinEntry E;
  int r0 = 0, r1 = 0; long long l0 = 0, l1 = 0;
  if (live) {
    E.lat_min = lat_min; E.lat_max = lat_max; E.lon_min = lon_min; E.lon_max = lon_max; E.lon_avg = lon_avg;
    E.d = d;
    d_cell_box(lat_min, lat_max, lon_min, lon_max, b, &r0, &r1, &l0, &l1);
    E.row0 = r0;
  }
  const int nbins = b.nblat * b.nblon;
  const int maxcopies = (b.nblon <= 0xffff) ? min(BIN_COPIES, b.nblon) : 1, maxrows_c = (b.nblon <= 0xffff) ? BIN_ROW_COPIES : 1;
  const bool regular = live && r1 - r0 <= maxrows_c && l1 - l0 <= maxcopies;
  const int ccopies = regular ? max(1, (int)(l1 - l0)) : 0, rcopies = regular ? max(1, r1 - r0) : 0;
  const int ncopies = ccopies * rcopies;
  int maxc = ncopies;
#pragma unroll
  for (int o = 32; o; o >>= 1) maxc = max(maxc, __shfl_xor(maxc, o));
  for (int k = 0; k < maxc; k++) {
    const bool on = k < ncopies;
    const int kr = on ? k / ccopies : 0, kc = on ? k - kr * ccopies : 0;
    const int col = on ? d_colmod(l0 + kc, b.nblon) : 0;
    const int slot = on ? (r0 + kr) * b.nblon + col : -1;
    if (FILL) {
      const int pos = d_slot_position(slot_cnt, slot);
      if (on) {
        const int at = slot_start[slot] + pos;
// ... 289 lines not shown
{
  const int lane = threadIdx.x;
  if ((int)blockIdx.x < H) {
    const int nheavy = *heavy_cnt;
    for (int h = blockIdx.x; h < nheavy; h += H) {
      const int s = heavy_list[h];
      const double lat_in_min = S.lat_min[s], lat_in_max = S.lat_max[s];
      const double lon_in_min = S.lon_min[s], lon_in_max = S.lon_max[s], lon_in_avg = S.lon_avg[s];
      const SrcQuery q = d_src_query(lat_in_min, lat_in_max, lon_in_min, lon_in_max, b);
      const int cnt = d_heavy_scan<false>(q, b, slot_start, entries, ecap, lat_in_min, lat_in_max, lon_in_min, lon_in_max, lon_in_avg,
                                          s, nullptr, nullptr, 0, 0);
      const int r = (int)(((unsigned)s * 2654435761u >> 12) % (unsigned)ps.nreg);
      unsigned base = 0;
      if (lane == 0 && cnt) base = atomicAdd(&ps.fill[r * FG_FILL_STRIDE], (unsigned)cnt);
      base = __shfl(base, 0);
      const int loc0 = (int)min(base, (unsigned)ps.regcap), n_ok = min(cnt, ps.regcap - loc0);
      const int wbase = r * ps.regcap + loc0;
      if (n_ok > 0)
        (void)d_heavy_scan<true>(q, b, slot_start, entries, ecap, lat_in_min, lat_in_max, lon_in_min, lon_in_max, lon_in_avg,
                                 s, ps.src, ps.dst, wbase, n_ok);
      if (lane == 0) { pair_beg[s] = wbase; pair_cnt[s] = n_ok; if (n_ok > CP_SMALL) big_list[atomicAdd(big_cnt, 1)] = s; }
    }
    return;
  }
  const int bR = (int)blockIdx.x - H;
  const long t = (long)bR * 64 + lane;
  const int s = (int)(t / CAND_G), sub = (int)(t % CAND_G);
  int cnt = 0;
  int ids[4] = {-1, -1, -1, -1};
  bool heavy = false;
  double lat_in_min = 0, lat_in_max = 0, lon_in_min = 0, lon_in_max = 0, lon_in_avg = 0;
  SrcQuery q{};
  if (s < nsrc && d_src_active(S, mask, s)) {
    lat_in_min = S.lat_min[s]; lat_in_max = S.lat_max[s];
    lon_in_min = S.lon_min[s]; lon_in_max = S.lon_max[s]; lon_in_avg = S.lon_avg[s];
    q = d_src_query(lat_in_min, lat_in_max, lon_in_min, lon_in_max, b);
    heavy = d_query_size(q, b, slot_start) > HEAVY_ENTRIES;
    if (!heavy)
      cnt = d_lane_scan<false>(q, sub, b, slot_start, entries, ecap, lat_in_min, lat_in_max, lon_in_min, lon_in_max, lon_in_avg,
                               ids, s, nullptr, nullptr, 0u, 0u);
  }
  const unsigned incl = wave_incl_scan((unsigned)cnt, lane);
  const unsigned total = __shfl(incl, 63);
  const unsigned excl = incl - (unsigned)cnt;
  const int r = (int)((((unsigned)(bR / CAND_CHUNK)) * 2654435761u >> 12) % (unsigned)ps.nreg);
  unsigned base = 0;
  if (lane == 0 && total) base = atomicAdd(&ps.fill[r * FG_FILL_STRIDE], total);
  base = __shfl(base, 0);
  int c4 = cnt;
  c4 += __shfl_xor(c4, 1); c4 += __shfl_xor(c4, 2);
  const unsigned excl0 = __shfl(excl, lane & ~(CAND_G - 1));
  if (sub == 0 && s < nsrc && !heavy) {
    const unsigned first = base + excl0;
    const int loc0 = (int)min(first, (unsigned)ps.regcap);
    pair_beg[s] = r * ps.regcap + loc0;
    pair_cnt[s] = min(c4, ps.regcap - loc0);
  }
  {
    const bool bigc = sub == 0 && s < nsrc && !heavy && min(c4, ps.regcap - (int)min(base + excl0, (unsigned)ps.regcap)) > CP_SMALL;
    const unsigned long long bm = __ballot(bigc);
    if (bm) {
      int q = 0;
      if (lane == 0) q = atomicAdd(big_cnt, __popcll(bm));
      q = __shfl(q, 0);
      if (bigc) big_list[q + __popcll(bm & ((1ull << lane) - 1ull))] = s;
    }
  }
  if (cnt == 0) return;
  const unsigned wloc = base + excl;
  int *psrc = ps.src + (size_t)r * ps.regcap, *pdst = ps.dst + (size_t)r * ps.regcap;
  if (cnt <= 4) {
#pragma unroll
    for (int k = 0; k < 4; k++)
      if (k < cnt && wloc + k < (unsigned)ps.regcap) { psrc[wloc + k] = s; pdst[wloc + k] = ids[k]; }
    return;
  }
  (void)d_lane_scan<true>(q, sub, b, slot_start, entries, ecap, lat_in_min, lat_in_max, lon_in_min, lon_in_max, lon_in_avg,
                          ids, s, psrc, pdst, wloc, (unsigned)ps.regcap);
}


#define RECT_HDR 8
#define RECT_EPS 1.e-9
#define RECT_HEAVY 48

__global__ __launch_bounds__(256) void k_rect_tables(const double *lon, const double *lat, int nx, int ny, double *hdr, double *lat_ax,
                                                      double *lon_ax, double *col, double *col_min, double *col_max, double *col_avg, double *row,
                                                      unsigned *bad, unsigned *err, double dst_tlon)
{
  d_load_trig_table();
  const long np = (long)(nx + 1) * (ny + 1);
  const long gid = (long)blockIdx.x * 256 + threadIdx.x, gsz = (long)gridDim.x * 256;
  bool b = false;
  for (long e = gid; e < np; e += gsz) {
    const long j = e / (nx + 1); const int i = (int)(e - j * (nx + 1));
    if (__double_as_longlong(lon[e]) != __double_as_longlong(lon[i]) ||
        __double_as_longlong(lat[e]) != __double_as_longlong(lat[j * (nx + 1)])) b = true;
  }
  if (gid <= ny) {
    const double y = lat[gid * (nx + 1)];
    lat_ax[gid] = y;
    if (!(y >= -G_HPI - 1.e-6) || !(y <= G_HPI + 1.e-6)) atomicOr(err, G_ERRBIT_BADLAT);
    if (gid < ny && !(lat[(gid + 1) * (nx + 1)] > y)) b = true;
    if (gid > 0 && gid < ny && d_is_pole(y)) b = true;
    double *r = row + (size_t)gid * 4;
    r[0] = d_sin_lat(0.5 * (y + y));
    if (gid < ny) {
      const double yb = lat[(gid + 1) * (nx + 1)];
      const bool flat = fabs(yb - y) < G_SMALL;
      const double dy = 0.5 * (yb - y);
      r[1] = d_sin_lat(0.5 * (yb + y)); r[2] = flat ? 1.0 : d_sin_lat(dy) / dy; r[3] = flat ? 1.0 : 0.0;
    } else { r[1] = 0.0; r[2] = 1.0; r[3] = 1.0; }
  }
  if (gid <= nx) lon_ax[gid] = lon[gid];
  if (gid < nx) {
    const double x0 = lon[gid], x1 = lon[gid + 1];
    if (!(x1 > x0) || !(x1 - x0 < G_PI - 1.e-6)) b = true;
    double x[G_FIXCAP], y[G_FIXCAP];
    x[0] = x0; x[1] = x1; x[2] = x1; x[3] = x0;
    y[0] = 0.0; y[1] = 0.0; y[2] = 0.1; y[3] = 0.1;
    const int n = d_fix_lon(x, y, 4, dst_tlon);
    double *c = col + (size_t)gid * RECT_COLW;
    if (n != 4) { b = true; for (int k = 0; k < RECT_COLW; k++) c[k] = 0.0; col_min[gid] = 0.0; col_max[gid] = 0.0; col_avg[gid] = 0.0; }
    else {
      double xmin = x[0], xmax = x[0], xs = 0;
      for (int k = 1; k < 4; k++) { if (x[k] < xmin) xmin = x[k]; if (x[k] > xmax) xmax = x[k]; }
      for (int k = 0; k < 4; k++) xs += x[k];
      xs /= 4;
      c[0] = x[0]; c[1] = x[1]; c[2] = x[2]; c[3] = x[3]; c[4] = xmin; c[5] = xmax; c[6] = xs; c[7] = x1 - x0;
      col_min[gid] = xmin; col_max[gid] = xmax; col_avg[gid] = xs;
    }
  }
  if (gid == 0) {
    if (!(lon[nx] - lon[0] <= G_TPI + 1.e-9)) b = true;
    hdr[0] = lon[0]; hdr[1] = nx / (lon[nx] - lon[0]); hdr[2] = lat[0]; hdr[3] = ny / (lat[(long)ny * (nx + 1)] - lat[0]);
  }
  if (__ballot(b) && (threadIdx.x & 63) == 0) atomicOr(bad, 1u);
}

template <bool STRICT>
__device__ __forceinline__ int d_axis_first(const double *ax, int n, double v, double x0, double inv)
{
  const double t = fmin(fmax(floor((v - x0) * inv), -1.0), (double)(n - 1));
  const int g = (int)t;
  auto above = [&](double a) { return STRICT ? a > v : a >= v; };
  const bool lo_ok = (g < 0) || !above(ax[g]);
  const bool hi_ok = (g + 1 >= n) || above(ax[g + 1]);
  if (lo_ok && hi_ok) return g + 1;
  int lo = 0, hi = n;
  while (lo < hi) { const int mid = (lo + hi) >> 1; if (above(ax[mid])) hi = mid; else lo = mid + 1; }
  return lo;
}

struct RectQuery { int j0, j1; int nw; int wa[3], wb[3]; };

__device__ __forceinline__ RectQuery d_rect_query(const FgRect &R, double lat_in_min, double lat_in_max, double lon_in_min, double lon_in_max)
{
  RectQuery q{};
  const double lon0 = R.hdr[0], inv_lon = R.hdr[1], lat0 = R.hdr[2], inv_lat = R.hdr[3];
  q.j0 = max(d_axis_first<true>(R.lat_ax, R.ny + 1, lat_in_min, lat0, inv_lat) - 1, 0);
  q.j1 = min(d_axis_first<false>(R.lat_ax, R.ny + 1, lat_in_max, lat0, inv_lat) - 1, R.ny - 1);
  q.nw = 0;
  if (lon_in_max - lon_in_min > G_PI) { q.nw = 1; q.wa[0] = 0; q.wb[0] = R.nx - 1; return q; }
  const double axl = R.lon_ax[0], axh = R.lon_ax[R.nx];
#pragma unroll
  for (int t = 2; t >= -2; t--) {
    const double T = t * G_TPI;
    const double lo = lon_in_min - RECT_EPS - T, hi = lon_in_max + RECT_EPS - T;
    if (!(axh > lo) || !(axl < hi)) continue;
    const int a = max(d_axis_first<true>(R.lon_ax, R.nx + 1, lo, lon0, inv_lon) - 1, 0);
    const int b = min(d_axis_first<false>(R.lon_ax, R.nx + 1, hi, lon0, inv_lon) - 1, R.nx - 1);
    if (a <= b && q.nw < 3) {
      if (q.nw == 0) { q.wa[0] = a; q.wb[0] = b; } else if (q.nw == 1) { q.wa[1] = a; q.wb[1] = b; } else { q.wa[2] = a; q.wb[2] = b; }
      q.nw++;
    }
  }
  return q;
}
__device__ __forceinline__ int d_rect_ncols(const RectQuery &q)
{
  int n = 0;
#pragma unroll
  for (int w = 0; w < 3; w++) if (w < q.nw) n += q.wb[w] - q.wa[w] + 1;
  return n;
}
__device__ __forceinline__ bool d_rect_heavy(const FgRect &R, double lat_in_min, double lat_in_max, double lon_in_min, double lon_in_max)
{
  const double nr = (lat_in_max - lat_in_min) * R.hdr[3] + 2.0;
  const double nc = (lon_in_max - lon_in_min > G_PI) ? (double)R.nx : (lon_in_max - lon_in_min) * R.hdr[1] + 2.0;
  return nr * nc > (double)RECT_HEAVY;
}
__device__ __forceinline__ int d_rect_col(const RectQuery &q, int k)
{
  int i = q.wa[0] + k;
  const int l0 = q.wb[0] - q.wa[0] + 1;
  if (q.nw > 1 && k >= l0) { i = q.wa[1] + (k - l0); const int l1 = q.wb[1] - q.wa[1] + 1; if (q.nw > 2 && k - l0 >= l1) i = q.wa[2] + (k - l0 - l1); }
  return i;
}
__device__ __forceinline__ bool d_rect_col_pass(const FgRect &R, int i, double lon_in_min, double lon_in_max, double lon_in_avg)
{
  double lon_out_min = R.col_min[i], lon_out_max = R.col_max[i];
  const double dx = R.col_avg[i] - lon_in_avg;
  if (dx < -G_PI)     { lon_out_min += G_TPI; lon_out_max += G_TPI; }
  else if (dx > G_PI) { lon_out_min -= G_TPI; lon_out_max -= G_TPI; }
  return !(lon_out_min >= lon_in_max || lon_out_max <= lon_in_min);
}

__device__ __forceinline__ double d_rect_area(const double *c, const double *r)
{
  const double s_lo = r[0], s_hi = r[4], s_mid = r[1], dat = r[2];
  const bool flat_m = r[3] != 0.0;
  double area = 0.0;
#pragma unroll
  for (int k = 0; k < 4; k++) {
    double dx = c[(k + 1) & 3] - c[k];
    if (dx > G_PI)  dx = dx - 2.0 * G_PI;
    if (dx < -G_PI) dx = dx + 2.0 * G_PI;
    if (fabs(dx + G_PI) < G_SMALL || fabs(dx - G_PI) < G_SMALL) { area += G_PI; continue; }
    if (k == 0) area -= dx * s_lo;
    else if (k == 2) area -= dx * s_hi;
    else if (flat_m) area -= dx * s_mid;
    else area -= dx * s_mid * dat;
  }
  if (area < 0) return -area * G_RADIUS * G_RADIUS;
  return area * G_RADIUS * G_RADIUS;
}

__device__ __forceinline__ int d_kth_set_bit(unsigned long long m, unsigned k)
{
  int pos = 0;
#pragma unroll
  for (int w = 32; w; w >>= 1) {
    const unsigned c = (unsigned)__popcll(m & ((1ull << w) - 1ull));
    if (k >= c) { k -= c; m >>= w; pos += w; }
  }
  return pos;
}

#define RECT_WL_WORDS 10
template <bool ONE = false>
__device__ __forceinline__ bool d_rect_wave_candidates(const FgRect &R, const FgPairSpace &ps, bool active, int s, int nsrc, unsigned wave_no,
                                                       double lat_in_min, double lat_in_max, double lon_in_min, double lon_in_max,
                                                       double lon_in_avg, int *pair_beg, int *pair_cnt, int *big_list, int *big_cnt,
                                                       unsigned *wl )
{
  const int lane = threadIdx.x & 63;
  int cnt = 0, nr = 0, nwc = 0, nc = 0;
  unsigned long long cmask = 0ull;
  RectQuery q{};
  bool heavy = false;
  if (active) {
    heavy = d_rect_heavy(R, lat_in_min, lat_in_max, lon_in_min, lon_in_max);
    if (!heavy) {
      q = d_rect_query(R, lat_in_min, lat_in_max, lon_in_min, lon_in_max);
      nr = max(q.j1 - q.j0 + 1, 0);
      nwc = d_rect_ncols(q);
      if (nr > 0) {
        for (int k = 0; k < nwc; k++)
          if (d_rect_col_pass(R, d_rect_col(q, k), lon_in_min, lon_in_max, lon_in_avg)) { nc++; if (k < 64) cmask |= 1ull << k; }
      }
      cnt = (int)min((long)nr * nc, 0x3fffffffL);
    }
  }
  const unsigned incl = wave_incl_scan((unsigned)cnt, lane);
  const unsigned total = __shfl(incl, 63);
  const unsigned excl = incl - (unsigned)cnt;
  const int r = (int)((wave_no * 2654435761u >> 12) % (unsigned)ps.nreg);
  unsigned base = 0;
  if (lane == 0 && total) base = atomicAdd(&ps.fill[r * FG_FILL_STRIDE], total);
  base = __shfl(base, 0);
  int n_ok = 0;
  const unsigned first = base + excl;
  if (s < nsrc && !heavy && (!ONE || lane == 0)) {
    const int loc0 = (int)min(first, (unsigned)ps.regcap);
    n_ok = min(cnt, ps.regcap - loc0);
    pair_beg[s] = r * ps.regcap + loc0;
    pair_cnt[s] = n_ok;
  }
  {
    const bool bigc = n_ok > CP_SMALL;
    const unsigned long long bm = __ballot(bigc);
    if (bm) {
      int qq = 0;
      if (lane == 0) qq = atomicAdd(big_cnt, __popcll(bm));
      qq = __shfl(qq, 0);
      if (bigc) big_list[qq + __popcll(bm & ((1ull << lane) - 1ull))] = s;
    }
  }
  const bool wide = nwc > 64;
  const int l0 = q.nw > 1 ? q.wb[0] - q.wa[0] + 1 : 64, l1 = q.nw > 2 ? q.wb[1] - q.wa[1] + 1 : 64;
  __syncthreads();
  wl[lane] = excl;
  wl[64 + lane] = wide ? 0u : (unsigned)nc;
  wl[2 * 64 + lane] = (unsigned)cmask; wl[3 * 64 + lane] = (unsigned)(cmask >> 32);
  wl[4 * 64 + lane] = (unsigned)q.j0;
  wl[5 * 64 + lane] = (unsigned)q.wa[0]; wl[6 * 64 + lane] = (unsigned)l0;
  wl[7 * 64 + lane] = (unsigned)(q.wa[1] - l0); wl[8 * 64 + lane] = (unsigned)(l0 + l1);
  wl[9 * 64 + lane] = (unsigned)(q.wa[2] - l0 - l1);
  __syncthreads();
  const unsigned lim = min(total, (unsigned)ps.regcap - min(base, (unsigned)ps.regcap));
  int *wsrc = ps.src + (size_t)r * ps.regcap + base, *wdst = ps.dst + (size_t)r * ps.regcap + base;
  const int s_first = ONE ? s : s - lane;
  for (unsigned ob = 0; ob < lim; ob += 64) {
    const unsigned o = ob + lane;
    if (o >= lim || base + o >= (unsigned)ps.regcap) continue;
    int L = 0;
#pragma unroll
    for (int st = 32; st; st >>= 1) if (wl[L + st] <= o) L += st;
    const unsigned ncL = wl[64 + L];
    if (!ncL) continue;
    const unsigned t = o - wl[L], jr = t / ncL, kc = t - jr * ncL;
    const int k = d_kth_set_bit((unsigned long long)wl[2 * 64 + L] | ((unsigned long long)wl[3 * 64 + L] << 32), kc);
    const int i = k + (k < (int)wl[6 * 64 + L] ? (int)wl[5 * 64 + L] : k < (int)wl[8 * 64 + L] ? (int)wl[7 * 64 + L] : (int)wl[9 * 64 + L]);
    wsrc[o] = s_first + L;
    wdst[o] = ((int)wl[4 * 64 + L] + (int)jr) * R.nx + i;
  }
  if (wide && n_ok > 0) {
    int *psrc = ps.src + (size_t)r * ps.regcap + first, *pdst = ps.dst + (size_t)r * ps.regcap + first;
    int w = 0;
    for (int j = q.j0; j <= q.j1 && w < n_ok; j++)
      for (int k = 0; k < nwc && w < n_ok; k++) {
        const int i = d_rect_col(q, k);
        if (d_rect_col_pass(R, i, lon_in_min, lon_in_max, lon_in_avg)) { psrc[w] = s; pdst[w] = j * R.nx + i; w++; }
      }
  }
  return heavy;
}

#define RECORD_WAVES 7
__global__ __launch_bounds__(256, RECORD_WAVES) void k_cell_struct2r(FgTileSet ts, const FgTile *tiles_in, FgTile *tiles_out, int ntiles, int nsrc, int ndst,
                                                        int nbS, FgCells S, double *area_out, FgRect R, const double *mask, int order, int *src_idx_f,
                                                        double *sums, unsigned *err, unsigned long long *band_keys, int cull,
                                                        int *heavy_list, int *heavy_cnt, int *rare_list, int *rare_cnt, FgPairSpace ps,
                                                        int *pair_beg, int *pair_cnt, int *big_list, int *big_cnt)
{
  __shared__ double vtile[256 * 9];
  __shared__ FgTile sh_tiles[FG_TILESET_MAX];
  static_assert(64 * RECT_WL_WORDS * sizeof(unsigned) <= 64 * 9 * sizeof(double), "a wave's share of vtile holds its candidate words");
  if (*R.bad) return;
  if (ts.n && (int)threadIdx.x < ts.n) sh_tiles[threadIdx.x] = ts.t[threadIdx.x];
  const bool isD = (int)blockIdx.x >= nbS;
  __shared__ unsigned long long sh_band[2];
  if (cull) {
    if (threadIdx.x == 0) { sh_band[0] = d_ord_key(R.lat_ax[R.ny]); sh_band[1] = ~d_ord_key(R.lat_ax[0]); }
    __syncthreads();
    band_keys = sh_band;
  }
  if (cull && !isD && band_keys[0]) {
    __syncthreads();
    const FgTile *tl0 = ts.n ? sh_tiles : tiles_in;
    const int s = blockIdx.x * 256 + threadIdx.x;
    bool keep = false;
    int idx_f = s;
    if (s < nsrc) {
      int t = 0;
      while (t + 1 < ntiles && s >= tl0[t + 1].cell_off) t++;
      const int loc = s - tl0[t].cell_off, i = loc % tl0[t].nx, j = loc / tl0[t].nx, nxp = tl0[t].nx + 1;
      if (order == 2) {
        int foff = 0;
        for (int m = 0; m < t; m++) foff += (tl0[m].nx + 2) * (tl0[m].ny + 2);
        idx_f = foff + (j + 1) * (tl0[t].nx + 2) + i + 1;
      }
      const int n0 = j * nxp + i;
      const double y0 = tl0[t].lat[n0], y1 = tl0[t].lat[n0 + 1], y2 = tl0[t].lat[n0 + nxp + 1], y3 = tl0[t].lat[n0 + nxp];
      const double lmin = fmin(fmin(y0, y1), fmin(y2, y3)), lmax = fmax(fmax(y0, y1), fmax(y2, y3));
      const double bmax = d_ord_val(band_keys[0]), bmin = d_ord_val(~band_keys[1]);
      keep = !((lmax <= bmin) || (lmin >= bmax)) || !(lmin == lmin);
    }
    if (!__syncthreads_or(keep)) {
      if (s < nsrc) {
        S.nv[s] = 0; S.area[s] = 0;
        pair_beg[s] = 0; pair_cnt[s] = 0;
        if (src_idx_f) src_idx_f[s] = idx_f;
        if (sums) { sums[s] = 0.0; sums[nsrc + s] = 0.0; sums[2 * (size_t)nsrc + s] = 0.0; }
      }
      if (ts.n && blockIdx.x == 0 && (int)threadIdx.x < ts.n) tiles_out[threadIdx.x] = sh_tiles[threadIdx.x];
      return;
    }
  }
  d_load_trig_table();
  const FgTile *tiles = ts.n ? sh_tiles : tiles_in;
  if (ts.n && blockIdx.x == 0 && (int)threadIdx.x < ts.n) tiles_out[threadIdx.x] = sh_tiles[threadIdx.x];
  if (!isD) {
    double box[5] = {0, 0, 0, 0, 0};
    int tl = 0;
    const int s0 = blockIdx.x * 256, s = s0 + threadIdx.x, lane = threadIdx.x & 63;
    bool rare = false;
    const int nv = d_cell_record<true>(tiles, ntiles, nsrc, S, err, s0, vtile, box, &tl, cull ? band_keys : nullptr, G_PI, &rare);
    {
      const unsigned long long m = __ballot(rare);
      if (m) {
        int base = 0;
        if (lane == 0) base = atomicAdd(rare_cnt, __popcll(m));
        base = __shfl(base, 0);
        if (rare) rare_list[base + __popcll(m & ((1ull << lane) - 1ull))] = s;
      }
    }
    if (s < nsrc && sums) { sums[s] = 0.0; sums[nsrc + s] = 0.0; sums[2 * (size_t)nsrc + s] = 0.0; }
    if (s < nsrc && src_idx_f) {
      if (order != 2) src_idx_f[s] = s;
      else {
        int foff = 0;
        for (int t = 0; t < tl; t++) foff += (tiles[t].nx + 2) * (tiles[t].ny + 2);
        const int loc = s - tiles[tl].cell_off, i = loc % tiles[tl].nx, j = loc / tiles[tl].nx;
        src_idx_f[s] = foff + (j + 1) * (tiles[tl].nx + 2) + i + 1;
      }
    }
    const bool active = s < nsrc && nv > 0 && (!mask || mask[s] > 0.5);
    const bool heavy = d_rect_wave_candidates(R, ps, active, s, nsrc, (unsigned)(s >> 6), box[0], box[1], box[2], box[3], box[4], pair_beg, pair_cnt,
                                              big_list, big_cnt, (unsigned *)(vtile + (threadIdx.x >> 6) * (64 * 9)));
    const unsigned long long m = __ballot(heavy);
    if (m) {
      int base = 0;
      if (lane == 0) base = atomicAdd(heavy_cnt, __popcll(m));
      base = __shfl(base, 0);
      if (heavy) heavy_list[base + __popcll(m & ((1ull << lane) - 1ull))] = s;
    }
  } else {
    const int d = ((int)blockIdx.x - nbS) * 256 + threadIdx.x;
    if (d < ndst) {
      const int j = d / R.nx, i = d - j * R.nx;
      area_out[d] = d_rect_area(R.col + (size_t)i * RECT_COLW, R.row + (size_t)j * 4);
    }
  }
}

__global__ __launch_bounds__(256) void k_polylist_records(FgPolyList P, FgCells S, int *src_idx_f, double *sums, FgRect R, int rect,
                                                           int *heavy_list, int *heavy_cnt, unsigned *err)
{
  if (rect && *R.bad) return;
  const int s = blockIdx.x * 256 + threadIdx.x, lane = threadIdx.x & 63;
  bool heavy = false;
  if (s < P.npoly) {
    const int n = P.n[s];
    double *v = S.verts + (size_t)s * 16;
    if (n < 3 || n > G_MAXV) {
      if (n > G_MAXV) atomicOr(err, G_ERRBIT_MAXV);
      S.nv[s] = 0; S.area[s] = 0; S.lat_min[s] = 0; S.lat_max[s] = 0; S.lon_min[s] = 0; S.lon_max[s] = 0; S.lon_avg[s] = 0;
      for (int k = 0; k < 16; k++) v[k] = 0.0;
    } else {
      double xmin = 0, xmax = 0, ymin = 0, ymax = 0;
      for (int k = 0; k < G_MAXV; k++) {
        const double x = (k < n) ? P.lon[(size_t)s * G_MAXV + k] : 0.0, y = (k < n) ? P.lat[(size_t)s * G_MAXV + k] : 0.0;
        v[k] = x; v[8 + k] = y;
        if (k == 0) { xmin = xmax = x; ymin = ymax = y; }
        else if (k < n) { xmin = fmin(xmin, x); xmax = fmax(xmax, x); ymin = fmin(ymin, y); ymax = fmax(ymax, y); }
      }
      if (!(ymin >= -G_HPI - 1.e-6) || !(ymax <= G_HPI + 1.e-6)) atomicOr(err, G_ERRBIT_BADLAT);
      S.nv[s] = n; S.area[s] = P.area[s]; S.lon_avg[s] = P.lon_avg[s];
      S.lat_min[s] = ymin; S.lat_max[s] = ymax; S.lon_min[s] = xmin; S.lon_max[s] = xmax;
      if (rect) heavy = d_rect_heavy(R, ymin, ymax, xmin, xmax);
    }
    if (src_idx_f) src_idx_f[s] = s;
    if (sums) { sums[s] = 0.0; sums[P.npoly + s] = 0.0; sums[2 * (size_t)P.npoly + s] = 0.0; }
  }
  if (rect) {
    const unsigned long long m = __ballot(heavy);
    if (m) {
      int base = 0;
      if (lane == 0) base = atomicAdd(heavy_cnt, __popcll(m));
      base = __shfl(base, 0);
      if (heavy) heavy_list[base + __popcll(m & ((1ull << lane) - 1ull))] = s;
    }
  }
}

__global__ __launch_bounds__(256) void k_rect_materialize(int ndst, FgRect R, FgCells D)
{
  const int d = blockIdx.x * 256 + threadIdx.x;
  if (d >= ndst) return;
  const int j = d / R.nx, i = d - j * R.nx;
  const double *c = R.col + (size_t)i * RECT_COLW;
  const double ya = R.lat_ax[j], yb = R.lat_ax[j + 1];
  D.lat_min[d] = ya; D.lat_max[d] = yb; D.lon_min[d] = c[4]; D.lon_max[d] = c[5]; D.lon_avg[d] = c[6]; D.nv[d] = 4;
  double *v = D.verts + (size_t)d * 16;
  for (int k = 0; k < 16; k++) v[k] = 0.0;
  v[0] = c[0]; v[1] = c[1]; v[2] = c[2]; v[3] = c[3];
  v[8] = ya; v[9] = ya; v[10] = yb; v[11] = yb;
}

__device__ __forceinline__ void d_rect_cell_candidates(const FgRect &R, const FgPairSpace &ps, int s, int lane, double lat_in_min, double lat_in_max,
                                                       double lon_in_min, double lon_in_max, double lon_in_avg, int *pair_beg, int *pair_cnt,
                                                       int *big_list, int *big_cnt)
{
  const RectQuery q = d_rect_query(R, lat_in_min, lat_in_max, lon_in_min, lon_in_max);
  const int nwc = d_rect_ncols(q), nr = q.j1 - q.j0 + 1;
  int nc = 0;
  for (int kb = 0; kb < nwc; kb += 64) {
    const int k = kb + lane;
    const bool pass = k < nwc && d_rect_col_pass(R, d_rect_col(q, k), lon_in_min, lon_in_max, lon_in_avg);
    nc += __popcll(__ballot(pass));
  }
  const long cnt_l = (long)nr * nc;
  const int cnt = (int)min(cnt_l, 0x7fffffffL);
  const int r = (int)(((unsigned)s * 2654435761u >> 12) % (unsigned)ps.nreg);
  unsigned base = 0;
  if (lane == 0 && cnt) base = atomicAdd(&ps.fill[r * FG_FILL_STRIDE], (unsigned)cnt);
  base = __shfl(base, 0);
  const int loc0 = (int)min(base, (unsigned)ps.regcap), n_ok = min(cnt, ps.regcap - loc0);
  const int wbase = r * ps.regcap + loc0;
  int cbase = 0;
  for (int kb = 0; kb < nwc && n_ok > 0; kb += 64) {
    const int k = kb + lane;
    int i = 0; bool pass = false;
    if (k < nwc) { i = d_rect_col(q, k); pass = d_rect_col_pass(R, i, lon_in_min, lon_in_max, lon_in_avg); }
    const unsigned long long m = __ballot(pass);
    const int at = cbase + __popcll(m & ((1ull << lane) - 1ull));
    if (pass)
      for (int jr = 0; jr < nr; jr++) {
        const long kk = (long)jr * nc + at;
        if (kk < n_ok) { ps.src[wbase + kk] = s; ps.dst[wbase + kk] = (q.j0 + jr) * R.nx + i; }
      }
    cbase += __popcll(m);
  }
  if (lane == 0) { pair_beg[s] = wbase; pair_cnt[s] = n_ok; if (n_ok > CP_SMALL) big_list[atomicAdd(big_cnt, 1)] = s; }
}

#define RARE_BLOCKS 64
template <bool FINISH>
__global__ __launch_bounds__(64) void k_candidates_rect(int nsrc, int H, FgCells S, const double *mask, FgRect R, FgPairSpace ps,
                                                         int *pair_beg, int *pair_cnt, const int *heavy_list, const int *heavy_cnt,
                                                         int *big_list, int *big_cnt, const int *rare_list, const int *rare_cnt, unsigned *err)
{
  const int lane = threadIdx.x;
  __shared__ unsigned wl[64 * RECT_WL_WORDS];
  if (FINISH && (int)blockIdx.x < RARE_BLOCKS) d_load_trig_table();
  const unsigned bad = *R.bad;
  const int nrare = FINISH ? *rare_cnt : 0;
  if (bad) return;
  const int hb = FINISH ? (int)blockIdx.x - RARE_BLOCKS : (int)blockIdx.x;
  if (hb >= 0 && hb < H) {
    const int nheavy = *heavy_cnt;
    for (int h = hb; h < nheavy; h += H) {
      const int s = heavy_list[h];
      d_rect_cell_candidates(R, ps, s, lane, S.lat_min[s], S.lat_max[s], S.lon_min[s], S.lon_max[s], S.lon_avg[s], pair_beg, pair_cnt, big_list, big_cnt);
    }
    return;
  }
  if constexpr (FINISH) {
    for (int h = blockIdx.x; h < nrare; h += RARE_BLOCKS) {
      const int s = rare_list[h];
      const double mk = mask ? mask[s] : 1.0;
      double b[5] = {0, 0, 0, 0, 0};
      const int nv = d_finish_rare_cell(S, err, s, lane, b);
      if (!(nv > 0 && mk > 0.5)) continue;
      if (d_rect_heavy(R, b[0], b[1], b[2], b[3])) d_rect_cell_candidates(R, ps, s, lane, b[0], b[1], b[2], b[3], b[4], pair_beg, pair_cnt, big_list, big_cnt);
      else (void)d_rect_wave_candidates<true>(R, ps, lane == 0, s, nsrc, (unsigned)(s >> 6), b[0], b[1], b[2], b[3], b[4], pair_beg, pair_cnt, big_list, big_cnt, wl);
    }
  } else {
    const int bR = (int)blockIdx.x - H;
    const int s = bR * 64 + lane;
    const bool active = s < nsrc && d_src_active(S, mask, s);
    double b[5] = {0, 0, 0, 0, 0};
    if (active) { b[0] = S.lat_min[s]; b[1] = S.lat_max[s]; b[2] = S.lon_min[s]; b[3] = S.lon_max[s]; b[4] = S.lon_avg[s]; }
    (void)d_rect_wave_candidates(R, ps, active, s, nsrc, (unsigned)bR, b[0], b[1], b[2], b[3], b[4], pair_beg, pair_cnt, big_list, big_cnt, wl);
  }
}

struct ClipOut { double area, clon, clat; };

template <int ORDER, int S>
__device__ __forceinline__ void d_finish_pair(const double *px, const double *py, int n_out, double maskv,
                                              double area_in, double area_out, double lon_in_avg,
                                              ClipOut *o, unsigned long long *stats)
{
  double pa, clon = 0, clat = 0;
  if (ORDER == 2) d_poly_area_ctr<S>(px, py, n_out, lon_in_avg, &pa, &clon, &clat);
  else pa = d_poly_area<S>(px, py, n_out);
  double xarea = pa * maskv;
  double min_area = (area_in < area_out) ? area_in : area_out;
  double ratio = xarea / min_area;
  if (fabs(ratio - 1.e-6) < 1.e-15) atomicAdd(&stats[FG_STAT_BORDERLINE], 1ull);
  if (ratio > 1.e-6) { o->area = xarea; o->clon = clon; o->clat = clat; }
  else o->area = -2.0;
}

#ifndef CLIP_THREADS
#define CLIP_THREADS 256
#endif
#ifndef CLIP_SLOTS
#define CLIP_SLOTS 8
#endif
#ifndef CLIP_WAVES
#define CLIP_WAVES 4
#endif
#ifndef CLIP_PAD_LDS
#define CLIP_PAD_LDS 0
#endif

template <bool RECT, int T>
__device__ __forceinline__ int d_clip_quad_sh(double2 (*sh_poly)[T], const int tid, const int s, const int d,
                                              const FgCells &S, const FgCells &D, const FgRect &R, unsigned *err)
{
  constexpr int NV1 = RECT ? CLIP_SLOTS : 4;
  const double *sv = S.verts + (size_t)s * 16;
  double x1[NV1], y1[NV1], x2[4], y2[4];
  double lon_out_avg;
  int n1 = S.nv[s], n2 = RECT ? 4 : D.nv[d];
  double lon_in_avg = S.lon_avg[s];
#pragma unroll
  for (int k = 0; k < NV1; k++) { x1[k] = sv[k]; y1[k] = sv[8 + k]; }
  if (RECT) {
    const int j = d / R.nx, i = d - j * R.nx;
    const double *c = R.col + (size_t)i * RECT_COLW;
    double ya = R.lat_ax[j], yb = R.lat_ax[j + 1];
    x2[0] = c[0]; x2[1] = c[1]; x2[2] = c[2]; x2[3] = c[3]; lon_out_avg = c[6];
    asm volatile("" : "+v"(ya), "+v"(yb));
    y2[0] = ya; y2[1] = ya; y2[2] = yb; y2[3] = yb;
  } else {
    const double *dv = D.verts + (size_t)d * 16;
#pragma unroll
    for (int k = 0; k < 4; k++) { x2[k] = dv[k]; y2[k] = dv[8 + k]; }
    lon_out_avg = D.lon_avg[d];
#pragma unroll
    for (int k = 0; k < 4; k++) asm volatile("" : "+v"(y2[k]));
    asm volatile("" : "+v"(n2));
  }
#pragma unroll
  for (int k = 0; k < NV1; k++) asm volatile("" : "+v"(x1[k]), "+v"(y1[k]));
#pragma unroll
  for (int k = 0; k < 4; k++) asm volatile("" : "+v"(x2[k]));
  asm volatile("" : "+v"(n1), "+v"(lon_in_avg), "+v"(lon_out_avg));
  if (n1 > NV1 || n2 > 4) return -1;
  double shift = 0.0;
  {
    double dx = lon_out_avg - lon_in_avg;
    if (dx < -G_PI) shift = G_TPI; else if (dx > G_PI) shift = -G_TPI;
  }
  bool wrap = false;
#pragma unroll
  for (int k = 0; k < NV1; k++) {
    if (!(k < 4 || k < n1)) { x1[k] = 0.0; y1[k] = 0.0; }
    if (k < n1 && (x1[k] > G_TPI || x1[k] < 0.0)) wrap = true;
  }
#pragma unroll
  for (int k = 0; k < 4; k++) if (shift != 0.0) x2[k] += shift;
  if (wrap) {
#pragma unroll
    for (int k = 0; k < NV1; k++) x1[k] = d_pimod1(x1[k]);
#pragma unroll
    for (int k = 0; k < 4; k++) x2[k] = d_pimod1(x2[k]);
  }
#pragma unroll
  for (int k = 0; k < NV1; k++) if (k < 4 || k < n1) sh_poly[k][tid] = make_double2(x1[k], y1[k]);
  const long long b0x = __double_as_longlong(x2[0]), b1x = __double_as_longlong(x2[1]);
  const long long b2x = __double_as_longlong(x2[2]), b3x = __double_as_longlong(x2[3]);
  const long long b0y = __double_as_longlong(y2[0]), b1y = __double_as_longlong(y2[1]);
  const long long b2y = __double_as_longlong(y2[2]), b3y = __double_as_longlong(y2[3]);
  auto cut = [=](int e) -> double2 {
    const long long m0 = -(long long)(e == 0), m1 = -(long long)(e == 1), m2 = -(long long)(e == 2), m3 = -(long long)(e == 3);
    return make_double2(__longlong_as_double((b0x & m0) | (b1x & m1) | (b2x & m2) | (b3x & m3)),
                        __longlong_as_double((b0y & m0) | (b1y & m1) | (b2y & m2) | (b3y & m3)));
  };
  int n_cur = n1;
  bool overflow = false, parallel = false;
  double2 e0 = cut(n2 - 1);
#if FG_EXP == 2
  for (int e = 0; e < 0; e++) {
#else
#pragma unroll
  for (int e = 0; e < 4; e++) {
    if ((!RECT && e >= n2) || n_cur <= 0) break;
#endif
    double2 e1 = cut(e);
    const double x2_0 = e0.x, y2_0 = e0.y, x2_1 = e1.x, y2_1 = e1.y;
    double2 c[CLIP_SLOTS];
    unsigned inmask = 0u;
#pragma unroll
    for (int k = 0; k < CLIP_SLOTS; k++) c[k] = sh_poly[k][tid];
#pragma unroll
    for (int k = 0; k < CLIP_SLOTS; k++)
      if (k < n_cur) inmask |= (unsigned)d_inside_edge(x2_0, y2_0, x2_1, y2_1, c[k].x, c[k].y) << k;
    const unsigned full = (1u << n_cur) - 1u;
    const unsigned prevmask = ((inmask << 1) | (inmask >> (n_cur - 1))) & full;
    const unsigned tmask = inmask ^ prevmask;
    const int ncross = __popc(tmask);
    if (ncross > 2 || ncross + __popc(inmask) > CLIP_SLOTS) { overflow = true; break; }
    if (tmask) {
      const int ka = __ffs((int)tmask) - 1, kb = 31 - __clz((int)tmask);
      double2 I[2];
#pragma unroll
      for (int j = 0; j < 2; j++) {
        const int k = j ? kb : ka;
        const double2 p0 = sh_poly[k ? k - 1 : n_cur - 1][tid], p1 = sh_poly[k][tid];
        const double x1_0 = p0.x, y1_0 = p0.y, x1_1 = p1.x, y1_1 = p1.y;
        double dy1 = y1_1 - y1_0;
        double dy2 = y2_1 - y2_0;
        double dx1 = x1_1 - x1_0;
        double dx2 = x2_1 - x2_0;
        double ds1 = y1_0 * x1_1 - y1_1 * x1_0;
        double ds2 = y2_0 * x2_1 - y2_1 * x2_0;
        double determ = dy2 * dx1 - dy1 * dx2;
        if (fabs(determ) < 1.0e-30) parallel = true;
        I[j] = make_double2((dx2 * ds1 - dx1 * ds2) / determ, (dy2 * ds1 - dy1 * ds2) / determ);
      }
#pragma unroll
      for (int k = 0; k < CLIP_SLOTS; k++)
        if (k < n_cur && ((inmask >> k) & 1u))
          sh_poly[__popc(inmask & ((1u << k) - 1u)) + __popc(tmask & ((2u << k) - 1u))][tid] = c[k];
      sh_poly[__popc(inmask & ((1u << ka) - 1u))][tid] = I[0];
      sh_poly[__popc(inmask & ((1u << kb) - 1u)) + 1][tid] = I[1];
    }
    n_cur = ncross + __popc(inmask);
    e0 = e1;
  }
  if (overflow) return -1;
  if (parallel) atomicOr(err, G_ERRBIT_PARALLEL);
  return n_cur;
}

#ifndef CLIP_COMPACT
#define CLIP_COMPACT 0
#endif
__device__ __forceinline__ int d_row_slot(int *row_cnt, bool take, int d, int lane);
template <int ORDER, bool RECT>
__global__ __launch_bounds__(CLIP_THREADS) __attribute__((amdgpu_waves_per_eu(CLIP_WAVES, CLIP_WAVES))) void k_clip_quad(FgPairSpace ps, FgCells S, const double *mask, FgCells D, FgRect R,
                                                 double *tmp_area, double *tmp_clon, double *tmp_clat, int *nacc,
                                                 int *defer_list, int *defer_cnt,
                                                 unsigned long long *stats, unsigned *err, int *row_cnt, int *tmp_rowpos)
{
  constexpr int T = CLIP_THREADS;
  __shared__ double2 sh_poly[CLIP_SLOTS][T];
#if CLIP_PAD_LDS
  __shared__ char sh_pad[CLIP_PAD_LDS];
  if (nacc == (int *)16) sh_pad[threadIdx.x * 7 % CLIP_PAD_LDS] = 1;
#endif
#if CLIP_COMPACT
  __shared__ unsigned short sh_perm[T];
  __shared__ unsigned char sh_n[T];
  __shared__ int sh_wtot[T / 64];
#endif
  const int tid = threadIdx.x, lane = tid & 63;
  const int p0 = blockIdx.x * T;
  const unsigned first = blockIdx.x * T, reg = first / (unsigned)ps.regcap;
  const unsigned fill = ps.fill[reg * FG_FILL_STRIDE];
  const unsigned bad = RECT ? *R.bad : 0u;
  if ((RECT && bad != 0u) | (first - reg * (unsigned)ps.regcap >= fill)) return;
  static_assert(2 * T >= 112 * 4, "at most two table values per lane");
  const int t0 = min(tid, 112 * 4 - 1), t1 = min(tid + T, 112 * 4 - 1);
  int s_in = ps.src[p0 + tid], d_in = ps.dst[p0 + tid];
  double tab0 = FG_SINCOS_TAB[t0 >> 2][t0 & 3], tab1 = FG_SINCOS_TAB[t1 >> 2][t1 & 3];
  asm volatile("" : "+v"(s_in), "+v"(d_in), "+v"(tab0), "+v"(tab1));
  fgs_lds_tab[t0] = tab0; fgs_lds_tab[t1] = tab1;
  __syncthreads();
  bool defer = false;
  int n_cur = 0;
  if ((unsigned)(p0 + tid) - reg * (unsigned)ps.regcap < min(fill, (unsigned)ps.regcap)) {
    n_cur = d_clip_quad_sh<RECT, T>(sh_poly, tid, s_in, d_in, S, D, R, err);
    if (n_cur < 0) { defer = true; n_cur = 0; }
    else if (n_cur == 0) ps.dst[p0 + tid] = -1;
  }
  int src = tid;
#if CLIP_COMPACT
  {
    const int wave = tid >> 6;
    const unsigned long long hm = __ballot(n_cur > 0);
    if (lane == 0) sh_wtot[wave] = __popcll(hm);
    sh_n[tid] = (unsigned char)n_cur;
    __syncthreads();
    int base = 0, total = 0;
#pragma unroll
    for (int w = 0; w < T / 64; w++) { const int c = sh_wtot[w]; if (w < wave) base += c; total += c; }
    if (n_cur > 0) sh_perm[base + __popcll(hm & ((1ull << lane) - 1ull))] = (unsigned short)tid;
    __syncthreads();
    if (tid < total) { src = sh_perm[tid]; n_cur = sh_n[src]; } else n_cur = 0;
  }
#endif
  bool below = false, acc = false;
  int s = -1, d_acc = -1;
  if (n_cur > 0) {
    const int p = p0 + src;
    s = CLIP_COMPACT ? ps.src[p] : s_in;
    const int d = CLIP_COMPACT ? ps.dst[p] : d_in;
    ClipOut o; o.area = -1.0; o.clon = 0; o.clat = 0;
    const double *px = (const double *)&sh_poly[0][src];
#if FG_EXP == 1
    o.area = n_cur + px[0] + px[1];
#else
    d_finish_pair<ORDER, 2 * T>(px, px + 1, n_cur, mask ? mask[s] : 1.0, S.area[s], D.area[d], S.lon_avg[s], &o, stats);
#endif
    if (o.area >= 0) {
      acc = true;
      tmp_area[p] = o.area;
      if (ORDER == 2) { tmp_clon[p] = o.clon; tmp_clat[p] = o.clat; }
      d_acc = d;
    } else {
      ps.dst[p] = -1;
      below = (o.area == -2.0);
    }
  }
  if (row_cnt) {
    const int slot = d_row_slot(row_cnt, acc, d_acc, lane);
    if (acc) tmp_rowpos[p0 + src] = slot;
  }
  if (__ballot(s >= 0)) {
    const int s_prev = __shfl_up(s, 1, 64);
    const bool head = (lane == 0) || (s != s_prev);
    const unsigned long long hm = __ballot(head), am = __ballot(acc);
    if (head && s >= 0) {
      const unsigned long long above = (lane == 63) ? 0ull : (hm >> (lane + 1)) << (lane + 1);
      const int end = above ? (__ffsll((long long)above) - 1) : 64;
      const unsigned long long upto = (end == 64) ? ~0ull : ((1ull << end) - 1ull);
      const int cnt = __popcll(am & upto & ~((1ull << lane) - 1ull));
      if (cnt) atomicAdd(&nacc[s], cnt);
    }
  }
  const unsigned long long dm = __ballot(defer), bm = __ballot(below);
  if (dm) {
    int q = 0;
    if (lane == 0) q = atomicAdd(defer_cnt, __popcll(dm));
    q = __shfl(q, 0);
    if (defer) defer_list[q + __popcll(dm & ((1ull << lane) - 1ull))] = p0 + tid;
  }
  if (bm && lane == 0) atomicAdd(&stats[FG_STAT_BELOW], (unsigned long long)__popcll(bm));
}

#define GEN_THREADS 64
#define GEN_CAP 16
template <int ORDER, bool RECT>
__global__ __launch_bounds__(GEN_THREADS) void k_clip_general(const int *defer_list, const int *defer_cnt,
                                                              const int *pair_src, int *pair_dst,
                                                              FgCells S, const double *mask, FgCells D, FgRect R,
                                                              double *tmp_area, double *tmp_clon, double *tmp_clat, int *nacc,
                                                              unsigned long long *stats, unsigned *err, int *row_cnt, int *tmp_rowpos)
{
  __shared__ double2 sh_a[GEN_CAP][GEN_THREADS];
  __shared__ double2 sh_b[GEN_CAP][GEN_THREADS];
  __shared__ double2 sh_cut[G_MAXV][GEN_THREADS];
  if (RECT && *R.bad) return;
  d_load_trig_table();
  const int tid = threadIdx.x;
  const int ndefer = *defer_cnt;
  for (int q = blockIdx.x * GEN_THREADS + tid; q < ndefer; q += gridDim.x * GEN_THREADS) {
    const int p = defer_list[q];
    const int s = pair_src[p], d = pair_dst[p];
    const int n1 = S.nv[s], n2 = RECT ? 4 : D.nv[d];
    const double *sv = S.verts + (size_t)s * 16;
    const double lon_in_avg = S.lon_avg[s];
    double dvx[G_MAXV], dvy[G_MAXV], lon_out_avg;
    if (RECT) {
      const int j = d / R.nx, i = d - j * R.nx;
      const double *c = R.col + (size_t)i * RECT_COLW;
      const double ya = R.lat_ax[j], yb = R.lat_ax[j + 1];
      dvx[0] = c[0]; dvx[1] = c[1]; dvx[2] = c[2]; dvx[3] = c[3]; lon_out_avg = c[6];
      dvy[0] = ya; dvy[1] = ya; dvy[2] = yb; dvy[3] = yb;
#pragma unroll
      for (int k = 4; k < G_MAXV; k++) { dvx[k] = 0.0; dvy[k] = 0.0; }
    } else {
      const double *dv = D.verts + (size_t)d * 16;
#pragma unroll
      for (int k = 0; k < G_MAXV; k++) { dvx[k] = dv[k]; dvy[k] = dv[8 + k]; }
      lon_out_avg = D.lon_avg[d];
    }
    double shift = 0.0;
    {
      double dx = lon_out_avg - lon_in_avg;
      if (dx < -G_PI) shift = G_TPI; else if (dx > G_PI) shift = -G_TPI;
    }
    bool wrap = false;
    for (int k = 0; k < n1; k++) { double xv = sv[k]; if (xv > G_TPI || xv < 0.0) wrap = true; }
    for (int k = 0; k < n1; k++) {
      double xv = sv[k]; if (wrap) xv = d_pimod1(xv);
      sh_a[k][tid] = make_double2(xv, sv[8 + k]);
    }
#pragma unroll
    for (int k = 0; k < G_MAXV; k++)
      if (k < n2) {
        double xv = dvx[k]; if (shift != 0.0) xv += shift; if (wrap) xv = d_pimod1(xv);
        sh_cut[k][tid] = make_double2(xv, dvy[k]);
      }
    double2 (*cur)[GEN_THREADS] = sh_a;
    double2 (*nxt)[GEN_THREADS] = sh_b;
    int n_cur = n1;
    bool overflow = false, parallel = false;
    double2 e0 = sh_cut[n2 - 1][tid];
    for (int e = 0; e < n2 && n_cur > 0 && !overflow; e++) {
      double2 e1 = sh_cut[e][tid];
      const double x2_0 = e0.x, y2_0 = e0.y, x2_1 = e1.x, y2_1 = e1.y;
      double2 lastv = cur[n_cur - 1][tid];
      double x1_0 = lastv.x, y1_0 = lastv.y;
      int inside_last = d_inside_edge(x2_0, y2_0, x2_1, y2_1, x1_0, y1_0);
      int n_new = 0;
      for (int k = 0; k < n_cur; k++) {
        double2 cv = cur[k][tid];
        double x1_1 = cv.x, y1_1 = cv.y;
        int inside = d_inside_edge(x2_0, y2_0, x2_1, y2_1, x1_1, y1_1);
        if (inside != inside_last) {
          double dy1 = y1_1 - y1_0;
          double dy2 = y2_1 - y2_0;
          double dx1 = x1_1 - x1_0;
          double dx2 = x2_1 - x2_0;
          double ds1 = y1_0 * x1_1 - y1_1 * x1_0;
          double ds2 = y2_0 * x2_1 - y2_1 * x2_0;
          double determ = dy2 * dx1 - dy1 * dx2;
          if (fabs(determ) < 1.0e-30) parallel = true;
          if (n_new < GEN_CAP) nxt[n_new][tid] = make_double2((dx2 * ds1 - dx1 * ds2) / determ,
                                                              (dy2 * ds1 - dy1 * ds2) / determ);
          else overflow = true;
          n_new++;
        }
        if (inside) {
          if (n_new < GEN_CAP) nxt[n_new][tid] = make_double2(x1_1, y1_1);
          else overflow = true;
          n_new++;
        }
        x1_0 = x1_1; y1_0 = y1_1; inside_last = inside;
      }
      n_cur = n_new;
      double2 (*t)[GEN_THREADS] = cur; cur = nxt; nxt = t;
      e0 = e1;
    }
    if (overflow) { atomicOr(err, G_ERRBIT_OVERFLOW); pair_dst[p] = -1; continue; }
    if (parallel) atomicOr(err, G_ERRBIT_PARALLEL);
    ClipOut o; o.area = -1.0; o.clon = 0; o.clat = 0;
    if (n_cur > 0) {
      const double *px = (const double *)&cur[0][tid];
      d_finish_pair<ORDER, 2 * GEN_THREADS>(px, px + 1, n_cur, mask ? mask[s] : 1.0, S.area[s], D.area[d],
                                            lon_in_avg, &o, stats);
    }
    if (o.area >= 0) {
      tmp_area[p] = o.area;
      if (ORDER == 2) { tmp_clon[p] = o.clon; tmp_clat[p] = o.clat; }
      atomicAdd(&nacc[s], 1);
      if (row_cnt) tmp_rowpos[p] = atomicAdd(&row_cnt[d], 1);
    } else {
      pair_dst[p] = -1;
      if (o.area == -2.0) atomicAdd(&stats[FG_STAT_BELOW], 1ull);
    }
  }
}

#define CP_SPAN (256 + CP_SMALL)
static_assert(CP_SMALL % 64 == 0 && CP_SMALL <= 256, "the halo lanes of k_compact are whole waves of its 256-lane block");

struct CpPair { int s, d, beg, cnt, row; long x0; int na; double a, l, t; bool mine; };

__device__ __forceinline__ int d_row_slot(int *row_cnt, bool take, int d, int lane)
{
  const int key = take ? d : -1 - lane;
  const int prev = __shfl_up(key, 1, 64);
  const bool head = (lane == 0) || (key != prev);
  const unsigned long long hm = __ballot(head), am = __ballot(take);
  int slot = 0;
  if (!am) return 0;
  if (4 * __popcll(hm & am) > 3 * __popcll(am)) {
    if (take) slot = atomicAdd(&row_cnt[d], 1);
// ... 149 lines not shown
          sval[rank - c0] = a; sval[stage + rank - c0] = l; sval[2 * stage + rank - c0] = t;
        }
        if (io.tmp_rowpos) io.perm[row] = FgRowEnt{(int)pos, s};
        else io.x_rowpos[pos] = atomicAdd(&io.row_cnt[d], 1);
      }
      __syncthreads();
      if (ORDER == 2 && threadIdx.x < 3 && x0 + na <= io.xcap) {
        const double *v = sval + threadIdx.x * stage;
        const int n = min(stage, na - c0);
        int k = 0;
        for (; k + 8 <= n; k += 8) {
          double t[8];
#pragma unroll
          for (int u = 0; u < 8; u++) t[u] = v[k + u];
#pragma unroll
          for (int u = 0; u < 8; u++) acc += t[u];
        }
        for (; k < n; k++) acc += v[k];
      }
      __syncthreads();
    }
    if (ORDER == 2 && io.sums && threadIdx.x < 3) io.sums[(size_t)threadIdx.x * nsrc + s] = acc;
  }
}

template <int ORDER>
__global__ __launch_bounds__(256, 8) void k_compact(int nsrc, FgPairSpace ps, FgCompactIo io)
{
  __shared__ double lds[CP_LDS_DOUBLES];
  if ((int)blockIdx.x < BIG_BLOCKS) { d_compact_big<ORDER>(nsrc, ps, io, lds); return; }
  int *sh_d = (int *)lds;
  double (*sh_v)[CP_SPAN] = (double (*)[CP_SPAN])(lds + CP_SPAN / 2 + 8);
  const int tid = threadIdx.x;
  const int p0 = ((int)blockIdx.x - BIG_BLOCKS) * 256;
  const unsigned r = (unsigned)p0 / (unsigned)ps.regcap;
  const unsigned rfill = ps.fill[r * FG_FILL_STRIDE];
  const unsigned live_end = r * (unsigned)ps.regcap + (rfill < (unsigned)ps.regcap ? rfill : (unsigned)ps.regcap);
  if ((unsigned)p0 >= live_end) return;
  CpPair c, h; h.mine = false; h.d = -1;
  if (tid < CP_SMALL) { d_cp_load<ORDER, true>(ps, io, p0, tid, live_end, c, h); sh_d[256 + tid] = h.d; }
  else d_cp_load<ORDER, false>(ps, io, p0, tid, live_end, c, h);
  sh_d[tid] = c.d;
  __syncthreads();
  const bool first = (unsigned)(p0 + tid) < live_end && p0 + tid == c.beg;
  {
    const long pos = d_cp_place<ORDER>(io, c, p0, sh_d, sh_v);
    if (!io.tmp_rowpos) { const int slot = d_row_slot(io.row_cnt, pos >= 0, c.d, tid & 63); if (pos >= 0) io.x_rowpos[pos] = slot; }
  }
  if (tid < CP_SMALL) {
    const long pos = d_cp_place<ORDER>(io, h, p0, sh_d, sh_v);
    if (!io.tmp_rowpos) { const int slot = d_row_slot(io.row_cnt, pos >= 0, h.d, tid & 63); if (pos >= 0) io.x_rowpos[pos] = slot; }
  }
  if (ORDER != 2 || !io.sums) return;
  __syncthreads();
  if (!first || !c.mine || c.x0 + c.na > io.xcap) return;
  double sa = 0, sl = 0, st = 0;
  const int lb = c.beg - p0;
  for (int k = 0; k < c.na; k++) { sa += sh_v[0][lb + k]; sl += sh_v[1][lb + k]; st += sh_v[2][lb + k]; }
  io.sums[c.s] = sa; io.sums[nsrc + c.s] = sl; io.sums[2 * (size_t)nsrc + c.s] = st;
}

__global__ __launch_bounds__(256) void k_centroids(int nsrc, FgCells S, const double *sums, FgSrcRec *cen)
{
  const int s = blockIdx.x * blockDim.x + threadIdx.x;
  double a = 0, ca = 1, cl = 0, ct = 0;
  int nv = 0;
  bool whole = false;
  if (s < nsrc && (a = sums[s]) > 0) {
    const double sl = sums[nsrc + s], st = sums[2 * (size_t)nsrc + s], sa = S.area[s];
    nv = S.nv[s];
    if (nv > 0) {
      ca = sa;
      if (fabs(a - ca) / ca < 1.e-3) {
        cl = sl / a;
        ct = st / a;
      } else whole = true;
    }
  }
  if (__syncthreads_or(whole)) {
    d_load_trig_table();
    if (whole) {
      double x[G_MAXV], y[G_MAXV];
      int n = nv;
      const double *vp = S.verts + (size_t)s * 16;
      for (int k = 0; k < G_MAXV; k++) { x[k] = vp[k]; y[k] = vp[8 + k]; }
      cl = d_poly_ctrlon<1>(x, y, n, S.lon_avg[s]) / ca;
      ct = d_poly_ctrlat<1>(x, y, n) / ca;
    }
  }
  if (s < nsrc) cen[s] = FgSrcRec{cl, ct};
}

__global__ __launch_bounds__(256) void k_distances(long nx, const int *x_src, const double *x_area, const FgSrcRec *cen, double *x_c1,
                                                    double *x_c2)
{
  long n = (long)blockIdx.x * blockDim.x + threadIdx.x;
  if (n >= nx) return;
  int s = x_src[n];
  double a = x_area[n];
  double di = x_c1[n] / a, dj = x_c2[n] / a;
  di -= cen[s].cen_lon; dj -= cen[s].cen_lat;
  x_c1[n] = di; x_c2[n] = dj;
}

static inline int nblk(long n, int t) { return (int)((n + t - 1) / t); }

void fgd_cell_struct(const FgTile *tiles_dev, int ntiles, int ncells, FgCells c, unsigned *err, hipStream_t st)
{
  if (ncells > 0) k_cell_struct<<<nblk(ncells, 256), 256, 0, st>>>(tiles_dev, ntiles, ncells, c, err);
}

void fgd_cell_struct2(const FgTileSet &ts, const FgTile *tiles_in, FgTile *tiles_out, int ntiles, int nsrc, int ndst, FgCells S, FgCells D,
                      FgBins b, int *slot_cnt, int order, int *src_idx_f, double *sums, unsigned *err, hipStream_t st,
                      unsigned long long *band_keys, int cull, double dst_tlon)
{
  const int nbS = nblk(nsrc, 256), nbD = nblk(ndst, 256);
  if (nbS + nbD > 0)
    k_cell_struct2<<<nbS + nbD, 256, 0, st>>>(ts, tiles_in, tiles_out, ntiles, nsrc, ndst, nbS, S, D, b, slot_cnt, order, src_idx_f, sums, err,
                                              band_keys, cull, dst_tlon);
}

void fgd_bin_count(int ncells, FgCells c, FgBins b, int *slot_cnt, hipStream_t st)
{
  if (ncells > 0) k_bin_count<<<nblk(ncells, 256), 256, 0, st>>>(ncells, c, b, slot_cnt);
}

void fgd_bin_fill(int ndst, FgCells D, FgBins b, int *slot_fill, const int *slot_start, FgBinEntry *entries, int cap,
                  int nsrc, FgCells S, const double *mask, int *heavy_list, int *heavy_cnt, hipStream_t st)
{
  const int nbD = nblk(ndst, 256), nbS = nblk(nsrc, 256);
  if (nbD + nbS > 0)
    k_bin_fill<<<nbD + nbS, 256, 0, st>>>(ndst, nbD, D, b, slot_fill, slot_start, entries, cap, nsrc, S, mask, heavy_list, heavy_cnt);
}

void fgd_candidates1(int nsrc, FgCells S, const double *mask, FgBins b, const int *slot_start, const FgBinEntry *entries, int ecap,
                     FgPairSpace ps, int *pair_beg, int *pair_cnt, const int *heavy_list, const int *heavy_cnt, int *big_list, int *big_cnt,
                     hipStream_t st)
{
  if (nsrc <= 0) return;
  const int nbR = nblk((long)nsrc * CAND_G, 64);
  const int H = min(8 * HEAVY_BLOCKS, max(64, nblk(nsrc, 8)));
  k_candidates1<<<nbR + H, 64, 0, st>>>(nsrc, H, S, mask, b, slot_start, entries, ecap, ps, pair_beg, pair_cnt, heavy_list, heavy_cnt, big_list, big_cnt);
}

void fgd_clip_quad(int order, FgPairSpace ps, FgCells S, const double *mask, FgCells D,
                   double *tmp_area, double *tmp_clon, double *tmp_clat, int *nacc, int *defer_list, int *defer_cnt,
                   unsigned long long *stats, unsigned *err, hipStream_t st, const FgRect *rect, int *row_cnt, int *tmp_rowpos)
{
  const long np = fgd_pairs_total(ps);
  if (np <= 0) return;
  const FgRect R = rect ? *rect : FgRect{};
  const int g = nblk(np, CLIP_THREADS);
#define FG_LAUNCH_QUAD(O, RC) k_clip_quad<O, RC><<<g, CLIP_THREADS, 0, st>>>(ps, S, mask, D, R, tmp_area, tmp_clon, tmp_clat, nacc, defer_list, defer_cnt, stats, err, row_cnt, tmp_rowpos)
  if (order == 2) { if (rect) FG_LAUNCH_QUAD(2, true); else FG_LAUNCH_QUAD(2, false); }
  else            { if (rect) FG_LAUNCH_QUAD(1, true); else FG_LAUNCH_QUAD(1, false); }
#undef FG_LAUNCH_QUAD
}

void fgd_clip_general(int order, FgPairSpace ps, FgCells S, const double *mask, FgCells D,
                      double *tmp_area, double *tmp_clon, double *tmp_clat, int *nacc, int *defer_list, int *defer_cnt,
                      unsigned long long *stats, unsigned *err, hipStream_t st, const FgRect *rect, int *row_cnt, int *tmp_rowpos)
{
  const long np = fgd_pairs_total(ps);
  if (np <= 0) return;
  int grid = nblk(np, GEN_THREADS); if (grid > 1024) grid = 1024;
  const FgRect R = rect ? *rect : FgRect{};
#define FG_LAUNCH_GEN(O, RC) k_clip_general<O, RC><<<grid, GEN_THREADS, 0, st>>>(defer_list, defer_cnt, ps.src, ps.dst, S, mask, D, R, tmp_area, tmp_clon, tmp_clat, nacc, stats, err, row_cnt, tmp_rowpos)
  if (order == 2) { if (rect) FG_LAUNCH_GEN(2, true); else FG_LAUNCH_GEN(2, false); }
  else            { if (rect) FG_LAUNCH_GEN(1, true); else FG_LAUNCH_GEN(1, false); }
#undef FG_LAUNCH_GEN
}

void fgd_rect_tables(const double *lon, const double *lat, int nx, int ny, double *hdr, double *lat_ax, double *lon_ax, double *col,
                     double *col_min, double *col_max, double *col_avg, double *row, unsigned *bad, unsigned *err, hipStream_t st, double dst_tlon)
{
  const long np = (long)(nx + 1) * (ny + 1);
  const int g = (int)std::min<long>(1024, std::max<long>((np + 255) / 256, (std::max(nx, ny) + 1 + 255) / 256));
  k_rect_tables<<<std::max(g, 1), 256, 0, st>>>(lon, lat, nx, ny, hdr, lat_ax, lon_ax, col, col_min, col_max, col_avg, row, bad, err, dst_tlon);
}
void fgd_cell_struct2r(const FgTileSet &ts, const FgTile *tiles_in, FgTile *tiles_out, int ntiles, int nsrc, int ndst, FgCells S, double *area_out,
                       FgRect R, const double *mask, int order, int *src_idx_f, double *sums, unsigned *err, hipStream_t st,
                       unsigned long long *band_keys, int cull, int *heavy_list, int *heavy_cnt, int *rare_list, int *rare_cnt, FgPairSpace ps,
                       int *pair_beg, int *pair_cnt, int *big_list, int *big_cnt)
{
  const int nbS = nblk(nsrc, 256), nbD = nblk(ndst, 256);
  if (nbS + nbD > 0)
    k_cell_struct2r<<<nbS + nbD, 256, 0, st>>>(ts, tiles_in, tiles_out, ntiles, nsrc, ndst, nbS, S, area_out, R, mask, order, src_idx_f, sums, err,
                                               band_keys, cull, heavy_list, heavy_cnt, rare_list, rare_cnt, ps, pair_beg, pair_cnt, big_list, big_cnt);
}
void fgd_polylist_records(FgPolyList P, FgCells S, int *src_idx_f, double *sums, const FgRect *rect, int *heavy_list, int *heavy_cnt,
                          unsigned *err, hipStream_t st)
{
  if (P.npoly > 0)
    k_polylist_records<<<nblk(P.npoly, 256), 256, 0, st>>>(P, S, src_idx_f, sums, rect ? *rect : FgRect{}, rect ? 1 : 0, heavy_list, heavy_cnt, err);
}
void fgd_rect_materialize(int ndst, FgRect R, FgCells D, hipStream_t st)
{
  if (ndst > 0) k_rect_materialize<<<nblk(ndst, 256), 256, 0, st>>>(ndst, R, D);
}
void fgd_candidates_rect(int nsrc, FgCells S, const double *mask, FgRect R, FgPairSpace ps, int *pair_beg, int *pair_cnt,
                         const int *heavy_list, const int *heavy_cnt, int *big_list, int *big_cnt, hipStream_t st, int listed_only,
                         const int *rare_list, const int *rare_cnt, unsigned *err)
{
  if (nsrc <= 0) return;
  const int nbR = listed_only ? 0 : nblk(nsrc, 64);
  const int H = min(HEAVY_BLOCKS, max(64, nblk(nsrc, 8)));
  const int Hf = max(H - RARE_BLOCKS, RARE_BLOCKS);
  if (listed_only) k_candidates_rect<true><<<Hf + RARE_BLOCKS, 64, 0, st>>>(nsrc, Hf, S, mask, R, ps, pair_beg, pair_cnt, heavy_list, heavy_cnt, big_list, big_cnt,
                                                          rare_list, rare_cnt, err);
  else k_candidates_rect<false><<<nbR + H, 64, 0, st>>>(nsrc, H, S, mask, R, ps, pair_beg, pair_cnt, heavy_list, heavy_cnt, big_list, big_cnt,
                                                       nullptr, nullptr, nullptr);
}

void fgd_compact(int order, int nsrc, FgPairSpace ps, const FgCompactIo &io, hipStream_t st)
{
  if (nsrc <= 0) return;
  const long np = fgd_pairs_total(ps);
  if (order == 2) k_compact<2><<<BIG_BLOCKS + nblk(np, 256), 256, 0, st>>>(nsrc, ps, io);
  else            k_compact<1><<<BIG_BLOCKS + nblk(np, 256), 256, 0, st>>>(nsrc, ps, io);
}

void fgd_centroids(int nsrc, FgCells S, const double *sums, FgSrcRec *cen, hipStream_t st)
{
  if (nsrc > 0) k_centroids<<<nblk(nsrc, 256), 256, 0, st>>>(nsrc, S, sums, cen);
}

void fgd_distances(long nx, const int *x_src, const double *x_area, const FgSrcRec *cen, double *x_c1, double *x_c2, hipStream_t st)
{
  if (nx > 0) k_distances<<<nblk(nx, 256), 256, 0, st>>>(nx, x_src, x_area, cen, x_c1, x_c2);
}

__global__ __launch_bounds__(256) void k_accumulate_cell_sums(int n, const int *cells, int nsrc, const int *xoff, const double *xa,
                                                               const double *c1, const double *c2, double *total)
{
  const int i = blockIdx.x * blockDim.x + threadIdx.x;
  if (i >= n) return;
  const int s = cells ? cells[i] : i;
  if (s < 0 || s >= nsrc) return;
  const int b = xoff[s], e = xoff[s + 1];
  if (b >= e) return;
  double a0 = total[s], a1 = total[(size_t)nsrc + s], a2 = total[2 * (size_t)nsrc + s];
  for (int q = b; q < e; q++) { a0 += xa[q]; a1 += c1[q]; a2 += c2[q]; }
  total[s] = a0; total[(size_t)nsrc + s] = a1; total[2 * (size_t)nsrc + s] = a2;
}
void fgd_accumulate_cell_sums(int n, const int *cells, int nsrc, const int *xoff, const double *xa, const double *c1, const double *c2,
                              double *total, hipStream_t st)
{
  if (n > 0) k_accumulate_cell_sums<<<(n + 255) / 256, 256, 0, st>>>(n, cells, nsrc, xoff, xa, c1, c2, total);
}
```

### include/fregrid_hip.h

```cpp
#ifndef FREGRID_HIP_H_
#define FREGRID_HIP_H_

#include <stddef.h>

#ifdef __cplusplus
extern "C" {
#endif

#define FG_ERR_ARG        (-1)
#define FG_ERR_HIP        (-2)
#define FG_ERR_MAXV       (-3)
#define FG_ERR_PARALLEL   (-4)
#define FG_ERR_CAPACITY   (-5)
#define FG_ERR_STATE      (-6)
#define FG_ERR_GEOM       (-8)
#define FG_ERR_IO         (-9)
#define FG_ERR_NOTFOUND   (-10)
#define FG_ERR_BILIN_NOTFOUND (-11)
#define FG_ERR_DATA       (-7)

#define FG_CONSERVE_ORDER1 1
#define FG_CONSERVE_ORDER2 2

int  get_maxxgrid(void);
// ... 47 lines not shown
void fg_pool_release(void);
void *fg_dev_alloc(size_t bytes, int device);
void fg_dev_free(void *p);
int  fg_dev_upload(void *dst_dev, const void *src_host, size_t bytes);
int  fg_dev_download(void *dst_host, const void *src_dev, size_t bytes);
int  fg_dev_gather_f64(double *dst_dev, const double *src_dev, const int *idx_dev, long n);
int  fg_dev_scatter_f64(double *dst_dev, const double *src_dev, const int *idx_dev, long n);

int  fg_plan_trim(fg_plan *plan);
long fg_plan_nxgrid(const fg_plan *plan);
long fg_plan_ncells_in(const fg_plan *plan);
long fg_plan_ncells_out(const fg_plan *plan);
int  fg_plan_order(const fg_plan *plan);
int  fg_plan_device(const fg_plan *plan);

double *fg_plan_cell_sums_dev(fg_plan *plan);
int fg_plan_copy_cell_sums(fg_plan *plan, double *dst_dev);
int fg_plan_accumulate_cell_sums(fg_plan *plan, double *total_dev, const int *cells_dev, int ncells);
int fg_plan_accumulate_cell_sums_async(fg_plan *plan, double *total_dev, const int *cells_dev, int ncells);

int fg_plan_finalize(fg_plan *plan, const double *total_cell_sums_dev);

int fg_plan_get_xgrid(const fg_plan *plan, int *t_in, int *i_in, int *j_in, int *i_out, int *j_out,
                      double *area, double *c1, double *c2);

int fg_plan_get_cell_struct(const fg_plan *plan, int which, double *lat_min, double *lat_max, double *lon_min,
                            double *lon_max, double *lon_avg, int *nvert, double *vlon, double *vlat);

int fg_plan_get_polygons(const fg_plan *plan, int maxv, int *n_out, double *v0, double *v1, double *v2);
long fg_plan_create_polylist(int order, int npoly, const int *n, const double *lon, const double *lat, const double *lon_avg,
                             const double *area_ref, int nx_out, int ny_out, const double *lon_out, const double *lat_out,
                             int device, fg_plan **plan_out);
int fg_plan_get_cell_area(const fg_plan *plan, double *area_in, double *area_out);

int fg_plan_set_xgrid(fg_plan *plan, long nxgrid, const int *t_in, const int *i_in, const int *j_in,
                      const int *i_out, const int *j_out, const double *area,
                      const double *di_in, const double *dj_in);

int fg_plan_apply(fg_plan *plan, const double *data, const double *grad_x, const double *grad_y,
                  const int *grad_mask, int has_missing, double missing, int nz,
                  double *out, double *gsum_out);

int fg_plan_apply_interleaved(fg_plan *plan, int nb, const double *data_il, const double *grad_x_il,
                              const double *grad_y_il, double *out_il, double *gsum_out);

int fg_plan_apply_records(fg_plan *plan, int nz, const double *rec, double *out, double *gsum_out);

int fg_plan_apply_levels(fg_plan *plan, const double *data, const double *grad_x, const double *grad_y,
                         const int *grad_mask, double missing, int nlev, double *out, double *gsum_out);
int fg_plan_apply_records_levels(fg_plan *plan, int nz, const double *rec, const unsigned char *maskbits, double missing,
                                 double *out, double *gsum_out);
int fg_plan_levels_capacity(void);

typedef struct fg_apply_opts {
  int has_missing;
  double missing;
  const double *weight;
  int cell_methods_sum;
  const double *field_area;
  double area_missing;
  const double *cell_area_in;
  const double *cell_area_out;
  int monotonic;
} fg_apply_opts;
int fg_plan_apply_ex(fg_plan *plan, const fg_apply_opts *opts, const double *data, const double *grad_x,
                     const double *grad_y, const int *grad_mask, int nz, double *out, double *gsum_out);
int fg_plan_mono_begin(fg_plan *plan, const fg_apply_opts *opts, const double *data, const double *grad_x,
                       const double *grad_y, const int *grad_mask);
int fg_plan_mono_minmax_dev(fg_plan *plan, double **f_min, double **f_max);
int fg_plan_mono_copy_minmax(fg_plan *plan, int to_plan, double *f_min, double *f_max);
int fg_plan_mono_end(fg_plan *plan, const fg_apply_opts *opts, const double *data, double *out, double *gsum_out);

void *fg_plan_stream(fg_plan *plan);
int fg_plan_sync(fg_plan *plan);

void fg_set_profiling(int on);
int  fg_plan_phase_ms(fg_plan *plan, float *ms, int n);

int fg_plan_stats(const fg_plan *plan, long *stats, int n);
void fg_set_search_mode(int exact);
void fg_set_search_cull(int on);
void fg_set_search_finalize(int on);
void fg_set_search_rect(int on);
void fg_set_search_frame(int coupler);
void fg_set_apply_ep(int on);
void fg_set_apply_vec(int v);
void fg_set_gc_split(int on);
void fg_set_apply_xcd(int on);

int fg_clip_2dx2d_batch(int npoly, const double *lon1, const double *lat1, const int *n1,
                        const double *lon2, const double *lat2, const int *n2,
                        double *lon_out, double *lat_out, int *n_out);
int fg_poly_op_batch(int op, int npoly, double *lon, double *lat, int *n, const double *clon, double *result);

typedef struct fg_c2l fg_c2l;

int  fg_c2l_create(int ntiles, const int *nx, const int *ny, const double *const *lonc, const double *const *latc,
                   const double *const *lont, const double *const *latt,
                   int ncontacts, const int *tile1, const int *tile2,
                   const int *istart1, const int *iend1, const int *jstart1, const int *jend1,
                   const int *istart2, const int *iend2, const int *jstart2, const int *jend2,
                   int device, fg_c2l **out);
void fg_c2l_destroy(fg_c2l *h);
long fg_c2l_ncells(const fg_c2l *h);
long fg_c2l_halo_size(const fg_c2l *h);
int  fg_c2l_set_stream(fg_c2l *h, void *stream);
int  fg_c2l_sync(fg_c2l *h);
int  fg_c2l_get_centres(const fg_c2l *h, double *lont_halo, double *latt_halo);
int  fg_c2l_fill_halo(fg_c2l *h, const double *src, double *halo_data, int nz);
int  fg_c2l_gradient(fg_c2l *h, const double *halo_data, int nz, int has_missing, double missing,
                     double *grad_x, double *grad_y, int *grad_mask);
int  fg_c2l_gradient_records(fg_c2l *h, const double *halo_data, int nz, double *rec);
int  fg_c2l_records(fg_c2l *h, const double *src, int nz, double *rec);
int  fg_c2l_records_levels(fg_c2l *h, const double *src, int nz, double missing, double *rec, unsigned char *maskbits);

int fg_c2l_grid_info(int nx, int ny, const double *xt, const double *yt, const double *xc, const double *yc,
                     double *dx, double *dy, double *area, double *edge_w, double *edge_e, double *edge_s,
                     double *edge_n, double *en_n, double *en_e, double *vlon, double *vlat);
int fg_find_contacts(int ntiles, const int *nx, const int *ny, const double *const *lonc, const double *const *latc,
                     int max_contacts, int *tile1, int *tile2, int *istart1, int *iend1, int *jstart1, int *jend1,
                     int *istart2, int *iend2, int *jstart2, int *jend2);
int fg_halo_map(int ntiles, const int *nx, const int *ny, int ncontacts, const int *tile1, const int *tile2,
                const int *istart1, const int *iend1, const int *jstart1, const int *jend1,
                const int *istart2, const int *iend2, const int *jstart2, const int *jend2,
                long *map_off, int *map);

int  fg_remap_write(const char *path, int order, long ncells, const int *tile1, const int *tile1_cell,
                    const int *tile2_cell, const double *xgrid_area, const double *tile1_distance);
int  fg_remap_write_interp(const char *path, int order, long n, const int *t_in, const int *i_in, const int *j_in,
                           const int *i_out, const int *j_out, const double *area, const double *di_in,
                           const double *dj_in, int isc, int jsc);
long fg_remap_read_size(const char *path);
int  fg_remap_read(const char *path, int order, long ncells, int *t_in, int *i_in, int *j_in, int *i_out, int *j_out,
                   double *area, double *di_in, double *dj_in);
const char *fg_remap_last_error(void);

#define FG_NC_BYTE 1
#define FG_NC_CHAR 2
#define FG_NC_SHORT 3
#define FG_NC_INT 4
#define FG_NC_FLOAT 5
#define FG_NC_DOUBLE 6
typedef struct fg_ncfile fg_ncfile;
int  fg_nc_open(const char *path, fg_ncfile **out);
int  fg_nc_create(const char *path, int version , fg_ncfile **out);
int  fg_nc_def_dim(fg_ncfile *f, const char *name, long len );
int  fg_nc_def_var(fg_ncfile *f, const char *name, int type, int ndims, const int *dimids);
int  fg_nc_put_att_text(fg_ncfile *f, int varid , const char *name, const char *val);
int  fg_nc_put_att_double(fg_ncfile *f, int varid, const char *name, int type, int n, const double *vals);
int  fg_nc_enddef(fg_ncfile *f);
int  fg_nc_inq_ndims(const fg_ncfile *f);
int  fg_nc_inq_nvars(const fg_ncfile *f);
long fg_nc_inq_numrecs(const fg_ncfile *f);
int  fg_nc_inq_dimid(const fg_ncfile *f, const char *name);
int  fg_nc_inq_dim(const fg_ncfile *f, int dimid, char *name, int cap, long *len);
int  fg_nc_inq_varid(const fg_ncfile *f, const char *name);
int  fg_nc_inq_var(const fg_ncfile *f, int varid, char *name, int cap, int *type, int *ndims, int *dimids, long *shape);
int  fg_nc_get_att_double(const fg_ncfile *f, int varid, const char *name, double *val, int cap);
int  fg_nc_get_att_text(const fg_ncfile *f, int varid, const char *name, char *buf, int cap);
int  fg_nc_get_vara(fg_ncfile *f, int varid, const long *start, const long *count, void *out);
int  fg_nc_get_vara_double(fg_ncfile *f, int varid, const long *start, const long *count, double *out);
int  fg_nc_put_vara(fg_ncfile *f, int varid, const long *start, const long *count, const void *data);
int  fg_nc_put_vara_double(fg_ncfile *f, int varid, const long *start, const long *count, const double *data);
int  fg_nc_close(fg_ncfile *f);
const char *fg_nc_last_error(void);

// ... 223 lines not shown
```

Measured before the change: 5.645 billion exchange-cells/s.

## Store source quads compactly with side table for wide cells in rect search

For rect-destination searches without polygon lists, source cells now keep 8 doubles per cell (4 lon, 4 lat) rather than 16, drop the lon_min/lon_max arrays, and place the rare cells with more than 4 vertices in a capped side table reached through an index. This cuts memory traffic in cell-structure writes and in clip and candidate reads. A wide-cap overflow error sets a retry flag that falls back to the non-rect path. The rect table verification is also split into separate blocks with incremental index math, a fast quad lon-fix is tried before the general one, and the sums zeroing appears to move into the candidates kernel.

```diff
diff --git a/fre-nctools_amd/_lib.py b/fre-nctools_amd/_lib.py
--- a/fre-nctools_amd/_lib.py
+++ b/fre-nctools_amd/_lib.py
@@ -39,7 +39,7 @@
     "fg_nc_inq_ndims", "fg_nc_inq_nvars", "fg_nc_inq_numrecs", "fg_nc_inq_dimid", "fg_nc_inq_dim", "fg_nc_inq_varid", "fg_nc_inq_var",
     "fg_nc_get_att_double", "fg_nc_get_att_text", "fg_nc_get_vara", "fg_nc_get_vara_double", "fg_nc_put_vara", "fg_nc_put_vara_double",
     "fg_nc_close", "fg_nc_last_error", "fg_dev_widen", "fg_dev_narrow", "fg_sweep_create", "fg_sweep_run", "fg_sweep_run_levels", "fg_sweep_destroy", "fg_host_alloc", "fg_host_free",
-    "fg_plan_stats", "fg_set_search_mode", "fg_set_search_cull", "fg_set_search_finalize", "fg_set_search_rect", "fg_set_search_frame", "fg_set_apply_xcd", "fg_set_apply_vec", "fg_set_apply_ep", "fg_set_gc_split", "fg_set_profiling", "fg_plan_phase_ms", "fg_gnomonic_ed_corners", "fg_latlon_corners",
+    "fg_plan_stats", "fg_set_search_mode", "fg_set_search_cull", "fg_set_search_finalize", "fg_set_search_rect", "fg_set_search_wide_cap", "fg_set_search_frame", "fg_set_apply_xcd", "fg_set_apply_vec", "fg_set_apply_ep", "fg_set_gc_split", "fg_set_profiling", "fg_plan_phase_ms", "fg_gnomonic_ed_corners", "fg_latlon_corners",
     "fg_bilin_create", "fg_bilin_create_from_weights", "fg_bilin_destroy", "fg_bilin_get_index_weight", "fg_bilin_npoints_fine",
     "fg_bilin_nlon_fine", "fg_bilin_nlat_fine", "fg_bilin_nlon", "fg_bilin_nlat", "fg_bilin_ncells", "fg_bilin_set_stream",
     "fg_bilin_sync", "fg_bilin_apply_scalar", "fg_bilin_apply_vector", "fg_bilin_remap_write", "fg_bilin_remap_read",
diff --git a/fre-nctools_amd/csrc/plan.hip b/fre-nctools_amd/csrc/plan.hip
--- a/fre-nctools_amd/csrc/plan.hip
+++ b/fre-nctools_amd/csrc/plan.hip
@@ -403,14 +403,24 @@
   }
 };
 
-static bool alloc_cells(fg_plan *pl, FgCells *c, size_t n)
-{
+static int g_wide_cap = -1;
+extern "C" void fg_set_search_wide_cap(int n) { g_wide_cap = n < 0 ? -1 : n; }
+static bool alloc_cells(fg_plan *pl, FgCells *c, size_t n, bool compact = false)
+{
+  *c = FgCells{};
   c->lat_min = pl->alloc<double>(n); c->lat_max = pl->alloc<double>(n);
-  c->lon_min = pl->alloc<double>(n); c->lon_max = pl->alloc<double>(n);
+  if (!compact) { c->lon_min = pl->alloc<double>(n); c->lon_max = pl->alloc<double>(n); }
   c->lon_avg = pl->alloc<double>(n); c->area = pl->alloc<double>(n);
   c->nv = pl->alloc<int>(n);
-  c->verts = pl->alloc<double>(n * 16);
-  return c->lat_min && c->lat_max && c->lon_min && c->lon_max && c->lon_avg && c->area && c->nv && c->verts;
+  c->verts = pl->alloc<double>(n * (compact ? FG_VSTRIDE_QUAD : 16));
+  if (compact) {
+    const size_t cap = n / 16 + 64;
+    c->vstride = FG_VSTRIDE_QUAD;
+    c->wide_cap = (int)(g_wide_cap >= 0 ? std::min<size_t>((size_t)g_wide_cap, cap) : cap);
+    c->wide = pl->alloc<double>(16 * (size_t)std::max(c->wide_cap, 1));
+    if (!c->wide) return false;
+  }
+  return c->lat_min && c->lat_max && (compact || (c->lon_min && c->lon_max)) && c->lon_avg && c->area && c->nv && c->verts;
 }
 
 static int plan_base(int order, int ntiles_in, const int *nx_in, const int *ny_in, int nx_out, int ny_out,
@@ -590,7 +600,7 @@
   const long npairs = fgd_pairs_total(ps);
   const long nx_alloc = npairs;
 
-  if (!alloc_cells(pl, &pl->S, nsrc)) return fg_fail(FG_ERR_HIP, "out of device memory");
+  if (!alloc_cells(pl, &pl->S, nsrc, rect && !pl->polys.npoly)) return fg_fail(FG_ERR_HIP, "out of device memory");
   SearchBlocks blk{pl};
   struct { double *hdr, *lat_ax, *lon_ax, *col, *row, *col_min, *col_max, *col_avg; } rt{};
   if (rect) {
@@ -701,7 +711,7 @@
   if (rect)
     fgd_candidates_rect(nsrc, pl->S, pl->mask_dev, pl->rect_tab, ps, pair_beg, pair_cnt, heavy_list, &dc->heavy_cnt, big_list, &dc->big_cnt, st,
                         pl->polys.npoly ? 0 : 1,
-                        rare_list, &dc->rare_cnt, dc->err);
+                        rare_list, &dc->rare_cnt, dc->err, pl->polys.npoly ? nullptr : pl->sums);
   else
     fgd_candidates1(nsrc, pl->S, pl->mask_dev, bins, bin_start, bin_entries, ecap, ps, pair_beg, pair_cnt, heavy_list, &dc->heavy_cnt, big_list,
                     &dc->big_cnt, st);
@@ -779,6 +789,7 @@
   pt.collect(pl->phase_ms); ptot.collect(pl->phase_ms);
   FGCHK(hipGetLastError());
   if (rect && hc->rect_bad) { caps->rect = false; return FG_RETRY; }
+  if (rect && (hc->err[0] & G_ERRBIT_WIDECAP)) { caps->rect = false; return FG_RETRY; }
   if (hc->total[0] > nentries) { caps->entries = hc->total[0]; return FG_RETRY; }
   if (hc->total[0] > 2000000000ull) return fg_fail(FG_ERR_ARG, "bin table too large");
   if (hc->total[3] > (unsigned long long)ps.regcap) {
@@ -1529,7 +1540,17 @@
     fgd_rect_materialize(pl->ndst, R, tmp, pl->stream);
     FGCHK(hipStreamSynchronize(pl->stream));
   }
-  const FgCells &c = which ? (pl->rect ? tmp : pl->D) : pl->S;
+  if (!which && pl->S.vstride == FG_VSTRIDE_QUAD) {
+    const size_t ns = (size_t)pl->nsrc;
+    auto get = [&](size_t bytes) { void *p = g_pool.get(pl->device, bytes); if (p) tmp_blocks.push_back(p); return p; };
+    tmp = pl->S;
+    tmp.lon_min = (double *)get(ns * 8); tmp.lon_max = (double *)get(ns * 8); tmp.verts = (double *)get(ns * 128);
+    tmp.vstride = 16; tmp.wide = nullptr; tmp.wide_cap = 0;
+    if (tmp_blocks.size() != 3) return fg_fail(FG_ERR_HIP, "out of device memory");
+    fgd_quad_materialize(pl->nsrc, pl->S, tmp.lon_min, tmp.lon_max, tmp.verts, pl->stream);
+    FGCHK(hipStreamSynchronize(pl->stream));
+  }
+  const FgCells &c = which ? (pl->rect ? tmp : pl->D) : (pl->S.vstride == FG_VSTRIDE_QUAD ? tmp : pl->S);
   size_t n = which ? pl->ndst : pl->nsrc;
   if (lat_min) FGCHK(hipMemcpy(lat_min, c.lat_min, n * sizeof(double), hipMemcpyDeviceToHost));
   if (lat_max) FGCHK(hipMemcpy(lat_max, c.lat_max, n * sizeof(double), hipMemcpyDeviceToHost));
diff --git a/fre-nctools_amd/csrc/poly_kernels.hip b/fre-nctools_amd/csrc/poly_kernels.hip
--- a/fre-nctools_amd/csrc/poly_kernels.hip
+++ b/fre-nctools_amd/csrc/poly_kernels.hip
@@ -128,8 +128,8 @@
   double a[PB_IN], b[PB_IN], c[PB_IN], e[PB_IN], xo[PB_CAP], yo[PB_CAP];
   const int n1 = S.nv[s];
   int n2;
-  const double *sv = S.verts + (size_t)s * 16;
-  for (int q = 0; q < 8; q++) { a[q] = sv[q]; b[q] = sv[8 + q]; }
+  const FgVerts sv = d_cell_verts(S, s, n1);
+  for (int q = 0; q < 8; q++) { a[q] = q < n1 ? sv.x[q] : 0.0; b[q] = q < n1 ? sv.y[q] : 0.0; }
   double lon_out_avg;
   if (rect) {
     const int j = d / R.nx, i = d - j * R.nx;
@@ -139,8 +139,8 @@
     e[0] = ya; e[1] = ya; e[2] = yb; e[3] = yb;
     n2 = 4;
   } else {
-    const double *dv = D.verts + (size_t)d * 16;
-    for (int q = 0; q < 8; q++) { c[q] = dv[q]; e[q] = dv[8 + q]; }
+    const FgVerts dv = d_cell_verts(D, d, 0);
+    for (int q = 0; q < 8; q++) { c[q] = dv.x[q]; e[q] = dv.y[q]; }
     lon_out_avg = D.lon_avg[d];
     n2 = D.nv[d];
   }
diff --git a/fre-nctools_amd/csrc/xgrid_device.h b/fre-nctools_amd/csrc/xgrid_device.h
--- a/fre-nctools_amd/csrc/xgrid_device.h
+++ b/fre-nctools_amd/csrc/xgrid_device.h
@@ -17,11 +17,33 @@
 #define G_ERRBIT_GC_CONVEX2 32u
 #define G_ERRBIT_GC_CLIP    64u
 
+#define FG_VSTRIDE_QUAD 8
 struct FgCells {
   double *lat_min, *lat_max, *lon_min, *lon_max, *lon_avg, *area;
   int *nv;
   double *verts;
-};
+  int vstride;
+  int wide_cap;
+  double *wide;
+};
+#ifdef __HIPCC__
+struct FgVerts { const double *x, *y; };
+__device__ __forceinline__ FgVerts d_cell_verts(const FgCells &c, int s, int n)
+{
+  if (c.vstride == FG_VSTRIDE_QUAD) {
+    const double *v = c.verts + (size_t)s * FG_VSTRIDE_QUAD;
+    if (n > 4) {
+      const int k = *(const int *)v;
+      const double *w = c.wide + (size_t)((unsigned)k < (unsigned)c.wide_cap ? k : 0) * 16;
+      return FgVerts{w, w + 8};
+    }
+    return FgVerts{v, v + 4};
+  }
+  const double *v = c.verts + (size_t)s * 16;
+  return FgVerts{v, v + 8};
+}
+__device__ __forceinline__ double *d_cell_quad(const FgCells &c, int s) { return c.verts + (size_t)s * FG_VSTRIDE_QUAD; }
+#endif
 
 struct FgBins {
   int nblat, nblon;
@@ -86,6 +108,7 @@
 struct FgLl2xGrid { const double *lon, *lat; double *x, *y, *z; long n; };
 struct FgLl2xSet { FgLl2xGrid g[FG_TILESET_MAX]; int n; };
 #define G_ERRBIT_LL2X 256u
+#define G_ERRBIT_WIDECAP 512u
 void fgd_latlon2xyz(const FgLl2xGrid *grids, int ngrids, unsigned *err, hipStream_t st);
 
 struct FgCounters {
@@ -141,12 +164,14 @@
                        unsigned long long *band_keys, int cull, int *heavy_list, int *heavy_cnt, int *rare_list, int *rare_cnt, FgPairSpace ps,
                        int *pair_beg, int *pair_cnt, int *big_list, int *big_cnt);
 void fgd_rect_materialize(int ndst, FgRect R, FgCells D, hipStream_t st);
+void fgd_quad_materialize(int nsrc, FgCells S, double *lon_min, double *lon_max, double *verts, hipStream_t st);
 struct FgPolyList { const int *n; const double *lon, *lat; const double *lon_avg, *area; int npoly; };
 void fgd_polylist_records(FgPolyList P, FgCells S, int *src_idx_f, double *sums, const FgRect *rect, int *heavy_list, int *heavy_cnt,
                           unsigned *err, hipStream_t st);
 void fgd_candidates_rect(int nsrc, FgCells S, const double *mask, FgRect R, FgPairSpace ps, int *pair_beg, int *pair_cnt,
                          const int *heavy_list, const int *heavy_cnt, int *big_list, int *big_cnt, hipStream_t st, int listed_only,
-                         const int *rare_list = nullptr, const int *rare_cnt = nullptr, unsigned *err = nullptr);
+                         const int *rare_list = nullptr, const int *rare_cnt = nullptr, unsigned *err = nullptr,
+                         double *sums = nullptr);
 void fgd_clip_general(int order, FgPairSpace ps, FgCells S, const double *mask, FgCells D,
               double *tmp_area, double *tmp_clon, double *tmp_clat, int *nacc, int *defer_list, int *defer_cnt,
               unsigned long long *stats, unsigned *err, hipStream_t st, const FgRect *rect = nullptr, int *row_cnt = nullptr,
diff --git a/fre-nctools_amd/csrc/xgrid_kernels.hip b/fre-nctools_amd/csrc/xgrid_kernels.hip
--- a/fre-nctools_amd/csrc/xgrid_kernels.hip
+++ b/fre-nctools_amd/csrc/xgrid_kernels.hip
@@ -240,7 +240,8 @@
     }
     else if (n < 0 || n > G_MAXV) {
       atomicOr(err, G_ERRBIT_MAXV);
-      c.nv[s] = 0; c.lon_min[s] = 0; c.lon_max[s] = 0; c.lon_avg[s] = 0; c.area[s] = 0;
+      c.nv[s] = 0; c.lon_avg[s] = 0; c.area[s] = 0;
+      if constexpr (!QUADS_ONLY) { c.lon_min[s] = 0; c.lon_max[s] = 0; }
     } else if constexpr (QUADS_ONLY) {
       double xmin = x[0], xmax = x[0], xs = 0;
 #pragma unroll
@@ -248,7 +249,7 @@
 #pragma unroll
       for (int k = 0; k < 4; k++) xs += x[k];
       xs /= 4;
-      c.lon_min[s] = xmin; c.lon_max[s] = xmax; c.lon_avg[s] = xs;
+      c.lon_avg[s] = xs;
       box[2] = xmin; box[3] = xmax; box[4] = xs;
       c.nv[s] = 4;
       nvert = 4;
@@ -273,35 +274,32 @@
   }
   if (QUADS_ONLY) *rare = listed;
   if (!__syncthreads_or(nvert != 0 || listed) && cull) return 0;
-  const long cnt = (long)min(256, ncells - s0) * 16;
-  double *out = c.verts + (size_t)s0 * 16;
-#pragma unroll
-  for (int q = 0; q < 16; q++) {
+  const long cnt = (long)min(256, ncells - s0) * NLIVE;
+  double *out = QUADS_ONLY ? d_cell_quad(c, s0) : c.verts + (size_t)s0 * 16;
+#pragma unroll
+  for (int q = 0; q < NLIVE; q++) {
     const long e = (long)q * 256 + threadIdx.x;
-    if constexpr (QUADS_ONLY) {
-      const int k = (int)e & 15;
-      if (e < cnt) out[e] = (k & 4) ? 0.0 : vtile[(e >> 4) * VS + ((k >> 3) << 2) + (k & 3)];
-    } else if (e < cnt) out[e] = vtile[(e >> 4) * VS + (e & 15)];
+    if (e < cnt) out[e] = vtile[(e / NLIVE) * VS + (e % NLIVE)];
   }
   return nvert;
 }
 
-__device__ __forceinline__ int d_finish_rare_cell(const FgCells &c, unsigned *err, int s, int lane, double *box)
-{
-  double *v = c.verts + (size_t)s * 16;
+__device__ __forceinline__ int d_finish_rare_cell(const FgCells &c, unsigned *err, int s, int h, int lane, double *box)
+{
+  double *v = d_cell_quad(c, s);
   double x[G_FIXCAP], y[G_FIXCAP];
 #pragma unroll
-  for (int k = 0; k < 4; k++) { x[k] = v[k]; y[k] = v[8 + k]; }
+  for (int k = 0; k < 4; k++) { x[k] = v[k]; y[k] = v[4 + k]; }
   double lmin = y[0], lmax = y[0];
 #pragma unroll
   for (int k = 1; k < 4; k++) { if (y[k] < lmin) lmin = y[k]; if (y[k] > lmax) lmax = y[k]; }
   box[0] = lmin; box[1] = lmax;
   const int n = d_fix_lon(x, y, 4, G_PI);
-  if (n < 0 || n > G_MAXV) {
+  if (n < 0 || n > G_MAXV || (n > 4 && h >= c.wide_cap)) {
     if (lane == 0) {
-      atomicOr(err, G_ERRBIT_MAXV);
-      c.nv[s] = 0; c.lon_min[s] = 0; c.lon_max[s] = 0; c.lon_avg[s] = 0; c.area[s] = 0;
-      for (int k = 0; k < 16; k++) v[k] = 0.0;
+      atomicOr(err, (n < 0 || n > G_MAXV) ? G_ERRBIT_MAXV : G_ERRBIT_WIDECAP);
+      c.nv[s] = 0; c.lon_avg[s] = 0; c.area[s] = 0;
+      for (int k = 0; k < FG_VSTRIDE_QUAD; k++) v[k] = 0.0;
     }
     return 0;
   }
@@ -312,12 +310,20 @@
   box[2] = xmin; box[3] = xmax; box[4] = xs;
   const double area = d_poly_area<1>(x, y, n);
   if (lane == 0) {
-    c.lon_min[s] = xmin; c.lon_max[s] = xmax; c.lon_avg[s] = xs;
+    c.lon_avg[s] = xs;
     c.nv[s] = n;
-    for (int k = 0; k < G_MAXV; k++) {
-      v[k] = (k < n) ? x[k] : 0.0;
-      v[8 + k] = (k < n) ? y[k] : 0.0;
-    }
+    if (n > 4) {
+      double *w = c.wide + (size_t)h * 16;
+      for (int k = 0; k < G_MAXV; k++) {
+        w[k] = (k < n) ? x[k] : 0.0;
+        w[8 + k] = (k < n) ? y[k] : 0.0;
+      }
+      *(int *)v = h;
+    } else
+      for (int k = 0; k < 4; k++) {
+        v[k] = (k < n) ? x[k] : 0.0;
+        v[4 + k] = (k < n) ? y[k] : 0.0;
+      }
     c.area[s] = area;
   }
   return n;
@@ -773,21 +779,33 @@
 
 #define RECT_HDR 8
 #define RECT_EPS 1.e-9
+#define RECT_VERIFY_BLOCKS 8192
 #define RECT_HEAVY 48
 
 __global__ __launch_bounds__(256) void k_rect_tables(const double *lon, const double *lat, int nx, int ny, double *hdr, double *lat_ax,
                                                       double *lon_ax, double *col, double *col_min, double *col_max, double *col_avg, double *row,
                                                       unsigned *bad, unsigned *err, double dst_tlon)
 {
+  const int nbT = (max(nx, ny) + 1 + 255) / 256;
+  const long np = (long)(nx + 1) * (ny + 1);
+  bool b = false;
+  if ((int)blockIdx.x >= nbT) {
+    const long gid = (long)((int)blockIdx.x - nbT) * 256 + threadIdx.x, gsz = (long)((int)gridDim.x - nbT) * 256;
+    const int nxp = nx + 1;
+    const int dj = (int)(gsz / nxp), di = (int)(gsz - (long)dj * nxp);
+    long j = 0; int i = 0;
+    if (gid < np) { j = (long)((unsigned)gid / (unsigned)nxp); i = (int)(gid - j * nxp); }
+    for (long e = gid; e < np; e += gsz) {
+      if (__double_as_longlong(lon[e]) != __double_as_longlong(lon[i]) ||
+          __double_as_longlong(lat[e]) != __double_as_longlong(lat[j * nxp])) b = true;
+      j += dj; i += di;
+      if (i >= nxp) { i -= nxp; j++; }
+    }
+    if (__ballot(b) && (threadIdx.x & 63) == 0) atomicOr(bad, 1u);
+    return;
+  }
   d_load_trig_table();
-  const long np = (long)(nx + 1) * (ny + 1);
-  const long gid = (long)blockIdx.x * 256 + threadIdx.x, gsz = (long)gridDim.x * 256;
-  bool b = false;
-  for (long e = gid; e < np; e += gsz) {
-    const long j = e / (nx + 1); const int i = (int)(e - j * (nx + 1));
-    if (__double_as_longlong(lon[e]) != __double_as_longlong(lon[i]) ||
-        __double_as_longlong(lat[e]) != __double_as_longlong(lat[j * (nx + 1)])) b = true;
-  }
+  const long gid = (long)blockIdx.x * 256 + threadIdx.x;
   if (gid <= ny) {
     const double y = lat[gid * (nx + 1)];
     lat_ax[gid] = y;
@@ -810,7 +828,8 @@
     double x[G_FIXCAP], y[G_FIXCAP];
     x[0] = x0; x[1] = x1; x[2] = x1; x[3] = x0;
     y[0] = 0.0; y[1] = 0.0; y[2] = 0.1; y[3] = 0.1;
-    const int n = d_fix_lon(x, y, 4, dst_tlon);
+    int n = d_fix_lon_quad_fast(x, y, dst_tlon);
+    if (n < 0) n = d_fix_lon(x, y, 4, dst_tlon);
     double *c = col + (size_t)gid * RECT_COLW;
     if (n != 4) { b = true; for (int k = 0; k < RECT_COLW; k++) c[k] = 0.0; col_min[gid] = 0.0; col_max[gid] = 0.0; col_avg[gid] = 0.0; }
     else {
@@ -933,7 +952,8 @@
 __device__ __forceinline__ bool d_rect_wave_candidates(const FgRect &R, const FgPairSpace &ps, bool active, int s, int nsrc, unsigned wave_no,
                                                        double lat_in_min, double lat_in_max, double lon_in_min, double lon_in_max,
                                                        double lon_in_avg, int *pair_beg, int *pair_cnt, int *big_list, int *big_cnt,
-                                                       unsigned *wl )
+                                                       unsigned *wl ,
+                                                       int *n_pairs = nullptr )
 {
   const int lane = threadIdx.x & 63;
   int cnt = 0, nr = 0, nwc = 0, nc = 0;
@@ -968,6 +988,7 @@
     pair_beg[s] = r * ps.regcap + loc0;
     pair_cnt[s] = n_ok;
   }
+  if (n_pairs) *n_pairs = n_ok;
   {
     const bool bigc = n_ok > CP_SMALL;
     const unsigned long long bm = __ballot(bigc);
@@ -1087,7 +1108,6 @@
         if (rare) rare_list[base + __popcll(m & ((1ull << lane) - 1ull))] = s;
       }
     }
-    if (s < nsrc && sums) { sums[s] = 0.0; sums[nsrc + s] = 0.0; sums[2 * (size_t)nsrc + s] = 0.0; }
     if (s < nsrc && src_idx_f) {
       if (order != 2) src_idx_f[s] = s;
       else {
@@ -1098,8 +1118,10 @@
       }
     }
     const bool active = s < nsrc && nv > 0 && (!mask || mask[s] > 0.5);
+    int npair = 0;
     const bool heavy = d_rect_wave_candidates(R, ps, active, s, nsrc, (unsigned)(s >> 6), box[0], box[1], box[2], box[3], box[4], pair_beg, pair_cnt,
-                                              big_list, big_cnt, (unsigned *)(vtile + (threadIdx.x >> 6) * (64 * 9)));
+                                              big_list, big_cnt, (unsigned *)(vtile + (threadIdx.x >> 6) * (64 * 9)), &npair);
+    if (s < nsrc && sums && npair == 0 && !heavy && !rare) { sums[s] = 0.0; sums[nsrc + s] = 0.0; sums[2 * (size_t)nsrc + s] = 0.0; }
     const unsigned long long m = __ballot(heavy);
     if (m) {
       int base = 0;
@@ -1170,9 +1192,29 @@
   v[8] = ya; v[9] = ya; v[10] = yb; v[11] = yb;
 }
 
+__global__ __launch_bounds__(256) void k_quad_materialize(int nsrc, FgCells S, double *lon_min, double *lon_max, double *verts)
+{
+  const int s = blockIdx.x * 256 + threadIdx.x;
+  if (s >= nsrc) return;
+  const int n = min(S.nv[s], G_MAXV);
+  double *o = verts + (size_t)s * 16;
+  double xmin = 0.0, xmax = 0.0;
+  if (n > 0) {
+    const FgVerts v = d_cell_verts(S, s, n);
+    xmin = v.x[0]; xmax = v.x[0];
+    for (int k = 0; k < G_MAXV; k++) {
+      const double x = k < n ? v.x[k] : 0.0, y = k < n ? v.y[k] : 0.0;
+      if (k > 0 && k < n) { if (x < xmin) xmin = x; if (x > xmax) xmax = x; }
+      o[k] = x; o[8 + k] = y;
+    }
+  } else
+    for (int k = 0; k < 16; k++) o[k] = 0.0;
+  lon_min[s] = xmin; lon_max[s] = xmax;
+}
+
 __device__ __forceinline__ void d_rect_cell_candidates(const FgRect &R, const FgPairSpace &ps, int s, int lane, double lat_in_min, double lat_in_max,
                                                        double lon_in_min, double lon_in_max, double lon_in_avg, int *pair_beg, int *pair_cnt,
-                                                       int *big_list, int *big_cnt)
+                                                       int *big_list, int *big_cnt, double *zero_sums = nullptr, int nsrc = 0)
 {
   const RectQuery q = d_rect_query(R, lat_in_min, lat_in_max, lon_in_min, lon_in_max);
   const int nwc = d_rect_ncols(q), nr = q.j1 - q.j0 + 1;
@@ -1205,13 +1247,15 @@
     cbase += __popcll(m);
   }
   if (lane == 0) { pair_beg[s] = wbase; pair_cnt[s] = n_ok; if (n_ok > CP_SMALL) big_list[atomicAdd(big_cnt, 1)] = s; }
+  if (zero_sums && n_ok == 0 && lane < 3) zero_sums[(size_t)lane * nsrc + s] = 0.0;
 }
 
 #define RARE_BLOCKS 64
 template <bool FINISH>
 __global__ __launch_bounds__(64) void k_candidates_rect(int nsrc, int H, FgCells S, const double *mask, FgRect R, FgPairSpace ps,
                                                          int *pair_beg, int *pair_cnt, const int *heavy_list, const int *heavy_cnt,
-                                                         int *big_list, int *big_cnt, const int *rare_list, const int *rare_cnt, unsigned *err)
+                                                         int *big_list, int *big_cnt, const int *rare_list, const int *rare_cnt, unsigned *err,
+                                                         double *sums )
 {
   const int lane = threadIdx.x;
   __shared__ unsigned wl[64 * RECT_WL_WORDS];
@@ -1224,7 +1268,24 @@
     const int nheavy = *heavy_cnt;
     for (int h = hb; h < nheavy; h += H) {
       const int s = heavy_list[h];
-      d_rect_cell_candidates(R, ps, s, lane, S.lat_min[s], S.lat_max[s], S.lon_min[s], S.lon_max[s], S.lon_avg[s], pair_beg, pair_cnt, big_list, big_cnt);
+      double xmin, xmax;
+      if constexpr (FINISH) {
+        const double *q = d_cell_quad(S, s);
+        const int n = S.nv[s];
+        double x[G_MAXV];
+#pragma unroll
+        for (int k = 0; k < G_MAXV; k++) x[k] = k < 4 ? q[k] : 0.0;
+        if (n > 4) {
+          const FgVerts v = d_cell_verts(S, s, n);
+#pragma unroll
+          for (int k = 0; k < G_MAXV; k++) x[k] = v.x[k];
+        }
+        xmin = x[0]; xmax = x[0];
+#pragma unroll
+        for (int k = 1; k < G_MAXV; k++) if (k < n) { if (x[k] < xmin) xmin = x[k]; if (x[k] > xmax) xmax = x[k]; }
+      } else { xmin = S.lon_min[s]; xmax = S.lon_max[s]; }
+      d_rect_cell_candidates(R, ps, s, lane, S.lat_min[s], S.lat_max[s], xmin, xmax, S.lon_avg[s], pair_beg, pair_cnt, big_list, big_cnt,
+                             FINISH ? sums : nullptr, nsrc);
     }
     return;
   }
@@ -1233,10 +1294,18 @@
       const int s = rare_list[h];
       const double mk = mask ? mask[s] : 1.0;
       double b[5] = {0, 0, 0, 0, 0};
-      const int nv = d_finish_rare_cell(S, err, s, lane, b);
-      if (!(nv > 0 && mk > 0.5)) continue;
-      if (d_rect_heavy(R, b[0], b[1], b[2], b[3])) d_rect_cell_candidates(R, ps, s, lane, b[0], b[1], b[2], b[3], b[4], pair_beg, pair_cnt, big_list, big_cnt);
-      else (void)d_rect_wave_candidates<true>(R, ps, lane == 0, s, nsrc, (unsigned)(s >> 6), b[0], b[1], b[2], b[3], b[4], pair_beg, pair_cnt, big_list, big_cnt, wl);
+      const int nv = d_finish_rare_cell(S, err, s, h, lane, b);
+      if (!(nv > 0 && mk > 0.5)) {
+        if (sums && lane < 3) sums[(size_t)lane * nsrc + s] = 0.0;
+        continue;
+      }
+      if (d_rect_heavy(R, b[0], b[1], b[2], b[3])) d_rect_cell_candidates(R, ps, s, lane, b[0], b[1], b[2], b[3], b[4], pair_beg, pair_cnt, big_list, big_cnt, sums, nsrc);
+      else {
+        int npair = 0;
+        (void)d_rect_wave_candidates<true>(R, ps, lane == 0, s, nsrc, (unsigned)(s >> 6), b[0], b[1], b[2], b[3], b[4], pair_beg, pair_cnt, big_list, big_cnt, wl, &npair);
+        npair = __shfl(npair, 0);
+        if (sums && npair == 0 && lane < 3) sums[(size_t)lane * nsrc + s] = 0.0;
+      }
     }
   } else {
     const int bR = (int)blockIdx.x - H;
@@ -1279,18 +1348,24 @@
 #define CLIP_PAD_LDS 0
 #endif
 
-template <bool RECT, int T>
+template <bool RECT, int T, bool QSRC = false>
 __device__ __forceinline__ int d_clip_quad_sh(double2 (*sh_poly)[T], const int tid, const int s, const int d,
                                               const FgCells &S, const FgCells &D, const FgRect &R, unsigned *err)
 {
   constexpr int NV1 = RECT ? CLIP_SLOTS : 4;
-  const double *sv = S.verts + (size_t)s * 16;
   double x1[NV1], y1[NV1], x2[4], y2[4];
   double lon_out_avg;
   int n1 = S.nv[s], n2 = RECT ? 4 : D.nv[d];
   double lon_in_avg = S.lon_avg[s];
-#pragma unroll
-  for (int k = 0; k < NV1; k++) { x1[k] = sv[k]; y1[k] = sv[8 + k]; }
+  if constexpr (QSRC) {
+    const double *sq = d_cell_quad(S, s);
+#pragma unroll
+    for (int k = 0; k < NV1; k++) { x1[k] = k < 4 ? sq[k] : 0.0; y1[k] = k < 4 ? sq[4 + k] : 0.0; }
+  } else {
+    const FgVerts sv = d_cell_verts(S, s, 0);
+#pragma unroll
+    for (int k = 0; k < NV1; k++) { x1[k] = sv.x[k]; y1[k] = sv.y[k]; }
+  }
   if (RECT) {
     const int j = d / R.nx, i = d - j * R.nx;
     const double *c = R.col + (size_t)i * RECT_COLW;
@@ -1299,9 +1374,9 @@
     asm volatile("" : "+v"(ya), "+v"(yb));
     y2[0] = ya; y2[1] = ya; y2[2] = yb; y2[3] = yb;
   } else {
-    const double *dv = D.verts + (size_t)d * 16;
-#pragma unroll
-    for (int k = 0; k < 4; k++) { x2[k] = dv[k]; y2[k] = dv[8 + k]; }
+    const FgVerts dv = d_cell_verts(D, d, 0);
+#pragma unroll
+    for (int k = 0; k < 4; k++) { x2[k] = dv.x[k]; y2[k] = dv.y[k]; }
     lon_out_avg = D.lon_avg[d];
 #pragma unroll
     for (int k = 0; k < 4; k++) asm volatile("" : "+v"(y2[k]));
@@ -1313,6 +1388,13 @@
   for (int k = 0; k < 4; k++) asm volatile("" : "+v"(x2[k]));
   asm volatile("" : "+v"(n1), "+v"(lon_in_avg), "+v"(lon_out_avg));
   if (n1 > NV1 || n2 > 4) return -1;
+  if constexpr (QSRC) {
+    if (n1 > 4) {
+      const FgVerts sv = d_cell_verts(S, s, n1);
+#pragma unroll
+      for (int k = 0; k < NV1; k++) { x1[k] = sv.x[k]; y1[k] = sv.y[k]; }
+    }
+  }
   double shift = 0.0;
   {
     double dx = lon_out_avg - lon_in_avg;
@@ -1404,7 +1486,7 @@
 #define CLIP_COMPACT 0
 #endif
 __device__ __forceinline__ int d_row_slot(int *row_cnt, bool take, int d, int lane);
-template <int ORDER, bool RECT>
+template <int ORDER, bool RECT, bool QSRC = false>
 __global__ __launch_bounds__(CLIP_THREADS) __attribute__((amdgpu_waves_per_eu(CLIP_WAVES, CLIP_WAVES))) void k_clip_quad(FgPairSpace ps, FgCells S, const double *mask, FgCells D, FgRect R,
                                                  double *tmp_area, double *tmp_clon, double *tmp_clat, int *nacc,
                                                  int *defer_list, int *defer_cnt,
@@ -1437,7 +1519,7 @@
   bool defer = false;
   int n_cur = 0;
   if ((unsigned)(p0 + tid) - reg * (unsigned)ps.regcap < min(fill, (unsigned)ps.regcap)) {
-    n_cur = d_clip_quad_sh<RECT, T>(sh_poly, tid, s_in, d_in, S, D, R, err);
+    n_cur = d_clip_quad_sh<RECT, T, QSRC>(sh_poly, tid, s_in, d_in, S, D, R, err);
     if (n_cur < 0) { defer = true; n_cur = 0; }
     else if (n_cur == 0) ps.dst[p0 + tid] = -1;
   }
@@ -1526,7 +1608,7 @@
     const int p = defer_list[q];
     const int s = pair_src[p], d = pair_dst[p];
     const int n1 = S.nv[s], n2 = RECT ? 4 : D.nv[d];
-    const double *sv = S.verts + (size_t)s * 16;
+    const FgVerts sv = d_cell_verts(S, s, n1);
     const double lon_in_avg = S.lon_avg[s];
     double dvx[G_MAXV], dvy[G_MAXV], lon_out_avg;
     if (RECT) {
@@ -1538,9 +1620,9 @@
 #pragma unroll
       for (int k = 4; k < G_MAXV; k++) { dvx[k] = 0.0; dvy[k] = 0.0; }
     } else {
-      const double *dv = D.verts + (size_t)d * 16;
-#pragma unroll
-      for (int k = 0; k < G_MAXV; k++) { dvx[k] = dv[k]; dvy[k] = dv[8 + k]; }
+      const FgVerts dv = d_cell_verts(D, d, n2);
+#pragma unroll
+      for (int k = 0; k < G_MAXV; k++) { dvx[k] = dv.x[k]; dvy[k] = dv.y[k]; }
       lon_out_avg = D.lon_avg[d];
     }
     double shift = 0.0;
@@ -1549,10 +1631,10 @@
       if (dx < -G_PI) shift = G_TPI; else if (dx > G_PI) shift = -G_TPI;
     }
     bool wrap = false;
-    for (int k = 0; k < n1; k++) { double xv = sv[k]; if (xv > G_TPI || xv < 0.0) wrap = true; }
+    for (int k = 0; k < n1; k++) { double xv = sv.x[k]; if (xv > G_TPI || xv < 0.0) wrap = true; }
     for (int k = 0; k < n1; k++) {
-      double xv = sv[k]; if (wrap) xv = d_pimod1(xv);
-      sh_a[k][tid] = make_double2(xv, sv[8 + k]);
+      double xv = sv.x[k]; if (wrap) xv = d_pimod1(xv);
+      sh_a[k][tid] = make_double2(xv, sv.y[k]);
     }
 #pragma unroll
     for (int k = 0; k < G_MAXV; k++)
@@ -1868,8 +1950,8 @@
     if (whole) {
       double x[G_MAXV], y[G_MAXV];
       int n = nv;
-      const double *vp = S.verts + (size_t)s * 16;
-      for (int k = 0; k < G_MAXV; k++) { x[k] = vp[k]; y[k] = vp[8 + k]; }
+      const FgVerts vp = d_cell_verts(S, s, n);
+      for (int k = 0; k < G_MAXV; k++) { x[k] = k < n ? vp.x[k] : 0.0; y[k] = k < n ? vp.y[k] : 0.0; }
       cl = d_poly_ctrlon<1>(x, y, n, S.lon_avg[s]) / ca;
       ct = d_poly_ctrlat<1>(x, y, n) / ca;
     }
@@ -1937,9 +2019,10 @@
   if (np <= 0) return;
   const FgRect R = rect ? *rect : FgRect{};
   const int g = nblk(np, CLIP_THREADS);
-#define FG_LAUNCH_QUAD(O, RC) k_clip_quad<O, RC><<<g, CLIP_THREADS, 0, st>>>(ps, S, mask, D, R, tmp_area, tmp_clon, tmp_clat, nacc, defer_list, defer_cnt, stats, err, row_cnt, tmp_rowpos)
-  if (order == 2) { if (rect) FG_LAUNCH_QUAD(2, true); else FG_LAUNCH_QUAD(2, false); }
-  else            { if (rect) FG_LAUNCH_QUAD(1, true); else FG_LAUNCH_QUAD(1, false); }
+#define FG_LAUNCH_QUAD(O, RC, QS) k_clip_quad<O, RC, QS><<<g, CLIP_THREADS, 0, st>>>(ps, S, mask, D, R, tmp_area, tmp_clon, tmp_clat, nacc, defer_list, defer_cnt, stats, err, row_cnt, tmp_rowpos)
+  const bool qsrc = rect && S.vstride == FG_VSTRIDE_QUAD;
+  if (order == 2) { if (qsrc) FG_LAUNCH_QUAD(2, true, true); else if (rect) FG_LAUNCH_QUAD(2, true, false); else FG_LAUNCH_QUAD(2, false, false); }
+  else            { if (qsrc) FG_LAUNCH_QUAD(1, true, true); else if (rect) FG_LAUNCH_QUAD(1, true, false); else FG_LAUNCH_QUAD(1, false, false); }
 #undef FG_LAUNCH_QUAD
 }
 
@@ -1961,8 +2044,9 @@
                      double *col_min, double *col_max, double *col_avg, double *row, unsigned *bad, unsigned *err, hipStream_t st, double dst_tlon)
 {
   const long np = (long)(nx + 1) * (ny + 1);
-  const int g = (int)std::min<long>(1024, std::max<long>((np + 255) / 256, (std::max(nx, ny) + 1 + 255) / 256));
-  k_rect_tables<<<std::max(g, 1), 256, 0, st>>>(lon, lat, nx, ny, hdr, lat_ax, lon_ax, col, col_min, col_max, col_avg, row, bad, err, dst_tlon);
+  const int nbT = (std::max(nx, ny) + 1 + 255) / 256;
+  const int nbV = (int)std::min<long>(RECT_VERIFY_BLOCKS, std::max<long>((np + 255) / 256, 1));
+  k_rect_tables<<<nbT + nbV, 256, 0, st>>>(lon, lat, nx, ny, hdr, lat_ax, lon_ax, col, col_min, col_max, col_avg, row, bad, err, dst_tlon);
 }
 void fgd_cell_struct2r(const FgTileSet &ts, const FgTile *tiles_in, FgTile *tiles_out, int ntiles, int nsrc, int ndst, FgCells S, double *area_out,
                        FgRect R, const double *mask, int order, int *src_idx_f, double *sums, unsigned *err, hipStream_t st,
@@ -1984,18 +2068,22 @@
 {
   if (ndst > 0) k_rect_materialize<<<nblk(ndst, 256), 256, 0, st>>>(ndst, R, D);
 }
+void fgd_quad_materialize(int nsrc, FgCells S, double *lon_min, double *lon_max, double *verts, hipStream_t st)
+{
+  if (nsrc > 0) k_quad_materialize<<<nblk(nsrc, 256), 256, 0, st>>>(nsrc, S, lon_min, lon_max, verts);
+}
 void fgd_candidates_rect(int nsrc, FgCells S, const double *mask, FgRect R, FgPairSpace ps, int *pair_beg, int *pair_cnt,
                          const int *heavy_list, const int *heavy_cnt, int *big_list, int *big_cnt, hipStream_t st, int listed_only,
-                         const int *rare_list, const int *rare_cnt, unsigned *err)
+                         const int *rare_list, const int *rare_cnt, unsigned *err, double *sums)
 {
   if (nsrc <= 0) return;
   const int nbR = listed_only ? 0 : nblk(nsrc, 64);
   const int H = min(HEAVY_BLOCKS, max(64, nblk(nsrc, 8)));
   const int Hf = max(H - RARE_BLOCKS, RARE_BLOCKS);
   if (listed_only) k_candidates_rect<true><<<Hf + RARE_BLOCKS, 64, 0, st>>>(nsrc, Hf, S, mask, R, ps, pair_beg, pair_cnt, heavy_list, heavy_cnt, big_list, big_cnt,
-                                                          rare_list, rare_cnt, err);
+                                                          rare_list, rare_cnt, err, sums);
   else k_candidates_rect<false><<<nbR + H, 64, 0, st>>>(nsrc, H, S, mask, R, ps, pair_beg, pair_cnt, heavy_list, heavy_cnt, big_list, big_cnt,
-                                                       nullptr, nullptr, nullptr);
+                                                       nullptr, nullptr, nullptr, nullptr);
 }
 
 void fgd_compact(int order, int nsrc, FgPairSpace ps, const FgCompactIo &io, hipStream_t st)
diff --git a/include/fregrid_hip.h b/include/fregrid_hip.h
--- a/include/fregrid_hip.h
+++ b/include/fregrid_hip.h
@@ -153,6 +153,7 @@
 void fg_set_search_cull(int on);
 void fg_set_search_finalize(int on);
 void fg_set_search_rect(int on);
+void fg_set_search_wide_cap(int n);
 void fg_set_search_frame(int coupler);
 void fg_set_apply_ep(int on);
 void fg_set_apply_vec(int v);
```

After: 5.759 billion exchange-cells/s, median of 6. 2.0% higher.
